# lnkloveating/MediQuery-RAG

Measured on AMD Instinct MI355X. Metric: queries/s (embed+top-k, k=5, b=256) over 1M×768 corpus; p50 single-query ms, higher is better.
Workload: dtype f32 (exact 3-way bf16 split, fp32 accumulate; exact fp32 top-k)

## Files before the change

### include/mq.h

```cpp
#ifndef MQ_H
#define MQ_H

#include <stdint.h>

#ifdef __cplusplus
extern "C" {
#endif

#define MQ_OK 0
#define MQ_EINVAL -1
#define MQ_ENOMEM -2
#define MQ_EHIP -3
#define MQ_EIO -4
#define MQ_ESTATE -5

#define MQ_DTYPE_F32 0
#define MQ_DTYPE_BF16 1
#define MQ_DTYPE_F32X6 2
#define MQ_DTYPE_F32_SCREEN 3

#define MQ_GELU_ERF 0
#define MQ_GELU_TANH 1
#define MQ_POOL_CLS 0
#define MQ_POOL_MEAN 1

#define MQ_MAX_K 64

typedef struct mq_index mq_index;
typedef struct mq_encoder mq_encoder;

const char* mq_last_error(void);
const char* mq_version(void);
const char* mq_build_source_hash(void);
int mq_device_count(void);

int mq_index_create(int device, int dim, int64_t capacity, int dtype, mq_index** out);
int mq_index_destroy(mq_index* ix);
int mq_index_size(const mq_index* ix, int64_t* n_rows);
int mq_index_dim(const mq_index* ix, int* dim);
int mq_index_add(mq_index* ix, const float* rows, int64_t n, int rows_on_device, void* stream);
int mq_index_reset(mq_index* ix);
int mq_index_search(mq_index* ix, const float* queries, int64_t nq, int k,
                    float* out_scores, int64_t* out_ids, int io_on_device, void* stream);
int mq_index_select(mq_index* src, const int64_t* rows, int64_t n, mq_index* dst);
int mq_index_get(mq_index* ix, int64_t row0, int64_t n, float* out, int out_on_device, void* stream);
int mq_index_set_precision(mq_index* ix, int dtype);
int mq_index_set_stream_threshold(mq_index* ix, int max_queries);
int mq_index_set_threshold_scan(mq_index* ix, int enabled);
int mq_index_set_int8_screen(mq_index* ix, int enabled);
int mq_index_set_async_screen(mq_index* ix, int enabled);
int mq_index_rescans(const mq_index* ix, int64_t* rescans, int64_t* remerges);
int mq_index_screen_fallbacks(const mq_index* ix, int64_t* to_direct, int64_t* to_split);
int mq_index_screen_skips(const mq_index* ix, int64_t* bf16_skips, int64_t* int8_skips);
int mq_index_data(mq_index* ix, void** device_rows);
int mq_index_set_timing(mq_index* ix, int enabled);
int mq_index_read_timing(mq_index* ix, float* ms, int n);
#define MQ_MASK_SET 0
#define MQ_MASK_AND 1
#define MQ_MASK_OR 2
#define MQ_MASK_CLEAR 3
int mq_mask_eval(const int32_t* codes, int64_t n, const uint8_t* lut, int n_lut, uint32_t* bits, int mode,
                 void* stream);
int mq_mask_eval_bits(const int32_t* codes, int64_t n, const uint64_t* lut_words, int n_lut, uint32_t* bits,
                      int mode, void* stream);
int mq_mask_combine(uint32_t* dst, const uint32_t* src, int64_t n_words, int mode, void* stream);
int mq_index_search_masked(mq_index* ix, const float* query, int k, const uint32_t* bits, float* out_scores,
                           int64_t* out_ids, int io_on_device, void* stream);
int mq_index_search_masked_batch(mq_index* ix, const float* queries, int64_t nq, int k, const uint32_t* bits,
                                 float* out_scores, int64_t* out_ids, int io_on_device, void* stream);
int mq_index_masked_gathers(const mq_index* ix, int64_t* count);
#define MQ_CONTAINS_MAX_BYTES 256
#define MQ_CONTAINS_SPAN_BYTES 16384
int mq_mask_contains(const uint8_t* text, int64_t text_bytes, const int64_t* offsets, int64_t n,
                     const uint8_t* pattern, int pattern_len, int negate, uint32_t* bits, int mode,
                     uint32_t* scratch, void* stream);

#define MQ_MMR_SCORE(fmul, fsub, lambda, s, red) \
  fsub(fmul((lambda), (s)), fmul(fsub(1.0f, (lambda)), (red)))
int mq_index_mmr_select(mq_index* ix, const float* cand_scores, const int64_t* cand_ids, int64_t nq,
                        int fetch_k, int k, float lambda, float* out_scores, int64_t* out_ids,
                        int io_on_device, void* stream);
int mq_index_search_mmr(mq_index* ix, const float* queries, int64_t nq, int k, int fetch_k,
                        float lambda, const uint32_t* bits, float* out_scores, int64_t* out_ids,
                        int io_on_device, void* stream);

int mq_index_save(mq_index* ix, const char* path);
int mq_index_load(mq_index* ix, const char* path);
int mq_index_save_rows(mq_index* ix, const char* path, int64_t row0, int64_t n);
int mq_index_load_append(mq_index* ix, const char* path);

int mq_topk_merge_host(const float* scores, const int64_t* ids, int n_lists, int64_t nq,
                       int k_in, int k_out, float* out_scores, int64_t* out_ids);
int mq_topk_merge_device(const float* scores, const int64_t* ids, int n_lists, int64_t nq,
                         int k_in, int k_out, float* out_scores, int64_t* out_ids, void* stream);

typedef struct mq_bert_config {
  int vocab_size;
  int hidden;
  int layers;
  int heads;
  int ffn;
  int max_positions;
  int type_vocab;
  float ln_eps;
  int gelu;
  int pooling;
} mq_bert_config;

int mq_encoder_create(int device, const mq_bert_config* cfg, mq_encoder** out);
int mq_encoder_destroy(mq_encoder* enc);
int64_t mq_encoder_weight_count(const mq_bert_config* cfg);
int mq_encoder_load_weights(mq_encoder* enc, const float* blob, int64_t n_floats);
int mq_encoder_set_precision(mq_encoder* enc, int dtype);
#define MQ_ENC_STAGES 8
int mq_encoder_set_graphs(mq_encoder* enc, int enabled);
#define MQ_ENC_OPT_ROWS_MAX 0
#define MQ_ENC_OPT_ROWS_SPLITS 1
#define MQ_ENC_OPT_SPLITK_MAX 2
#define MQ_ENC_OPT_LN_ROWS_PER_WAVE 3
#define MQ_ENC_OPT_FUSE_ATTN_OPROJ 4
#define MQ_ENC_OPT_FUSED_LN 5
#define MQ_ENC_OPT_SPLITK_TILES 6
#define MQ_ENC_OPT_LN_ON_LOAD 7
#define MQ_ENC_OPT_RESIDENT_LAYERS 8
#define MQ_ENC_OPT_X6_PRESPLIT 9
#define MQ_ENC_OPT_ROWS_PLANES 10
#define MQ_ENC_OPT_LN_FOLD 11
int mq_encoder_set_option(mq_encoder* enc, int option, int value);
int mq_encoder_get_option(const mq_encoder* enc, int option, int* value);
int mq_encoder_set_timing(mq_encoder* enc, int enabled);
int mq_encoder_read_timing(mq_encoder* enc, float* ms, int n);
int mq_encoder_embed(mq_encoder* enc, const int32_t* ids, const int32_t* mask, int B, int L,
                     float* out, int io_on_device, void* stream);

typedef struct mq_tokenizer mq_tokenizer;
int mq_tokenizer_create_wordpiece(const char* vocab_path, int lower_case, int max_length,
                                  mq_tokenizer** out);
int mq_tokenizer_create_wordpiece_tokens(const char* const* tokens, int n_tokens, int lower_case,
                                         int max_length, mq_tokenizer** out);
int mq_tokenizer_create_char(int vocab_size, int max_length, mq_tokenizer** out);
int mq_tokenizer_destroy(mq_tokenizer* tok);
int mq_tokenizer_encode_batch(mq_tokenizer* tok, const char* const* texts, int n, int pad_to,
                              int32_t* ids, int32_t* mask, int* out_len);

int mq_debug_gemm_f32(const float* A, const float* W, const float* bias, const float* resid,
                      float* out, int M, int N, int K, int epi, int tile, void* stream);
int64_t mq_debug_w3_bytes(int N, int K);
int mq_debug_split_w3(const float* W, int N, int K, void* w3, void* stream);
int mq_debug_gemm_x6p(const float* A, const void* W3, const float* bias, const float* resid,
                      float* out, int M, int N, int K, int epi, int tile, void* stream);
int mq_debug_gemm_x6p_ln(const float* A, const void* W3, const float* bias, const float* resid,
                         float* out, int M, int N, int K, int epi, int tile, const float* stats_in,
                         float* stats_out, const float* g, const float* b, const float* s_fold,
                         float eps, void* stream);
int mq_debug_ln_fold_weight(const float* W, const float* bias, const float* g, const float* b, int N,
                            int K, float* Wg, float* s_out, float* c_out, void* stream);
int mq_debug_attention(const float* qkv, const int* mask, int B, int L, int H, int heads, float scale,
                       int variant, float* ctx, void* stream);
int mq_debug_attn_oproj(const float* qkv, const int* mask, int B, int L, int H, int heads, float scale,
                        const float* Wo, const float* bo, const float* resid, int cls_only, int hg, int qf,
                        int acc, float* out, void* stream);

int mq_debug_int8_screen(mq_index* ix, const float* query, int kc, float* out_scores, int64_t* out_ids,
                         float* stats);

#ifdef __cplusplus
}
#endif
#endif
```

### mediquery-rag_amd/csrc/encoder.hip

```cpp
#include <algorithm>
#include <cmath>
#include <cstdlib>
#include <cstring>
#include <memory>
#include <vector>

#include "common.hpp"
#include "gemm_epi.hpp"
#include "gemm_f32.hpp"
#include "gemm_x6p.hpp"

namespace mq {


struct LnArgs {
  float* stats_out;
  const float* stats_in;
  const float* g;
  const float* b;
  float* xout;
  int ldx;
  int nt;
  float eps;
};

__device__ __forceinline__ float wave_sum(float v) {
#pragma unroll
  for (int off = 32; off > 0; off >>= 1) v += __shfl_xor(v, off);
  return v;
}

#ifndef MQ_LN_DIAG
#define MQ_LN_DIAG 0
#endif
#if MQ_LN_DIAG != 0 && !defined(MQ_MEASUREMENT_BUILD)
#error "MQ_LN_DIAG computes wrong results: only a measurement build (-DMQ_MEASUREMENT_BUILD) may set it"
#endif

template <class T, class Coords>
struct LnInHooks {
  static constexpr int A_LOADS = T::BM * T::F4_PER_ROW / T::THREADS;
  static_assert(T::A_SLOTS && T::THREADS % T::F4_PER_ROW == 0, "A slots: fixed row chunk per thread");
  const LnArgs& ln;
  Coords& coords;
  float2* st;
  int M, nk, S;
  float inv_k;
  FastDiv nkd;
  float2 part[kLnMaxParts];
  floatx4 gg[T::PF], bb[T::PF];
  float2 mr[A_LOADS];
  template <class DC>
  __device__ __forceinline__ void issue(int s, DC) {
    if constexpr (MQ_LN_DIAG == 1) return;
    constexpr int d = DC::value;
    const int sc = s < S ? s : S - 1;
    const int i = nkd.div(sc), kt = sc - i * nk;
    const int k = kt * T::BK + (threadIdx.x % T::F4_PER_ROW) * 4;
    gg[d] = *reinterpret_cast<const floatx4*>(ln.g + k);
    bb[d] = *reinterpret_cast<const floatx4*>(ln.b + k);
    int m0;
    int64_t n0;
    coords(i, m0, n0);
    const float2* src = reinterpret_cast<const float2*>(ln.stats_in) +
                        (int64_t)min(m0 + (int)threadIdx.x % T::BM, M - 1) * kLnMaxParts;
#pragma unroll
    for (int t = 0; t < kLnMaxParts; ++t) part[t] = src[t];
  }
  __device__ __forceinline__ void prepare(int s) {
    if constexpr (MQ_LN_DIAG == 1) return;
    if (s >= S || nkd.mod(s) != 0) return;
#pragma unroll
    for (int t = 0; t < kLnMaxParts; ++t) asm volatile("" : "+v"(part[t].x), "+v"(part[t].y));
    float mean = 0.f;
#pragma unroll
    for (int t = 0; t < kLnMaxParts; ++t) mean += part[t].x;
    mean *= 1.0f / (float)kLnMaxParts;
    float m2 = 0.f;
#pragma unroll
    for (int t = 0; t < kLnMaxParts; ++t) {
      const float dm = part[t].x - mean;
      m2 += part[t].y + (float)kLnPartW * dm * dm;
    }
    const float rstd = 1.0f / sqrtf(m2 * inv_k + ln.eps);
    if (threadIdx.x < T::BM) st[(nkd.div(s) & 1) * T::BM + threadIdx.x] = make_float2(mean, rstd);
  }
  __device__ __forceinline__ void stage_in(int s) {
    if constexpr (MQ_LN_DIAG == 1) return;
    const float2* ms = st + (nkd.div(s < S ? s : S - 1) & 1) * T::BM;
#pragma unroll
    for (int a = 0; a < A_LOADS; ++a) mr[a] = ms[((int)threadIdx.x + a * T::THREADS) / T::F4_PER_ROW];
  }
  template <class DC>
  __device__ __forceinline__ void xform(Stager<T>& sg, int s, DC) {
    if constexpr (MQ_LN_DIAG != 0) return;
    constexpr int d = DC::value;
#pragma unroll
    for (int a = 0; a < A_LOADS; ++a) sg.r[a] = (sg.r[a] - mr[a].x) * mr[a].y * gg[d] + bb[d];
    const int sc = s < S ? s : S - 1;
    const int i = nkd.div(sc), kt = sc - i * nk;
    int m0;
    int64_t n0;
    coords(i, m0, n0);
    if (n0 == 0 && s < S) {
      const int ch = threadIdx.x % T::F4_PER_ROW;
#pragma unroll
      for (int a = 0; a < A_LOADS; ++a) {
        const int r = min(m0 + ((int)threadIdx.x + a * T::THREADS) / T::F4_PER_ROW, M - 1);
        *reinterpret_cast<floatx4*>(ln.xout + (int64_t)r * ln.ldx + kt * T::BK + ch * 4) = sg.r[a];
      }
    }
  }
};

template <class T, int EPI, bool LN_IN = false>
__global__ __launch_bounds__(T::THREADS, T::WG_PER_CU) void gemm_nt_kernel(const float* __restrict__ A, int lda,
                                                         const float* __restrict__ W,
                                                         const float* __restrict__ bias,
                                                         const float* __restrict__ resid, int ldr,
                                                         float* __restrict__ out, int ldo, int M,
                                                         int N, int K, LnArgs ln, int rx, LnFold lf) {
  __shared__ __attribute__((aligned(16))) float lds[2 * T::STAGE_FLOATS];
  __shared__ float2 ln_st[LN_IN ? 2 * T::BM : 1];
  const int lane = threadIdx.x & 63, wave = __builtin_amdgcn_readfirstlane(threadIdx.x >> 6);
  const int wm = wave / T::WAVES_N, wn = wave % T::WAVES_N;
  const int tiles_n = (N + T::BN - 1) / T::BN, tiles_m = (M + T::BM - 1) / T::BM;
  const int G = gridDim.x, per_xcd = G >> 3;
  const int xslot = (blockIdx.x & 7) * per_xcd + (blockIdx.x >> 3);
  Region rg{0, tiles_m, 0, tiles_n};
  int loc = xslot, wstep = G;
  if (rx > 0) {
    rg = region_of(rx, blockIdx.x & 7, tiles_m, tiles_n);
    loc = blockIdx.x >> 3;
    wstep = per_xcd;
  }
  const int rtiles = rg.rm * rg.rn;
  const int n_tiles = loc < rtiles ? (rtiles - loc + wstep - 1) / wstep : 0;
  const FastDiv tnd(rg.rn);
  auto coords = [&](int i, int& m0, int64_t& n0) {
    const int t = i * wstep + loc;
    const int tr = tnd.div(t);
    m0 = (rg.m_lo + tr) * T::BM;
    n0 = (int64_t)(rg.n_lo + t - tr * rg.rn) * T::BN;
  };
  auto epi = [&](int i, floatx16(&acc)[T::TM][T::TN], float*) {
    int m0;
    int64_t n0l;
    coords(i, m0, n0l);
    const int n0 = (int)n0l;
    if constexpr (T::M16) {
      static_assert(EPI != EPI_RESID_STATS, "no LayerNorm partials on the 16x16x32 tiles");
      floatx4 a4[2 * T::TM][2 * T::TN];
#pragma unroll
      for (int m = 0; m < 2 * T::TM; ++m)
#pragma unroll
        for (int n = 0; n < 2 * T::TN; ++n)
#pragma unroll
          for (int e = 0; e < 4; ++e) a4[m][n][e] = acc[m >> 1][n >> 1][4 * (2 * (m & 1) + (n & 1)) + e];
      store_wave_tile16<EPI, 2 * T::TM, 2 * T::TN>(a4, m0 + wm * T::WM, n0 + wn * T::WN, M, N, bias, resid, ldr, out,
                                                   ldo, lane, lf);
      return;
    }
    static_assert(T::M16 || EPI < EPI_RESID_LN_STATS, "the LayerNorm-fold epilogues are on the 16x16 store");
    if constexpr (EPI == EPI_RESID_STATS) {
      static_assert(T::WN == kLnPartW, "stats partials are per kLnPartW-column wave tile");
      const int wr0 = m0 + wm * T::WM, wc0 = n0 + wn * T::WN;
      const int part = wc0 / T::WN;
      float bv[T::TN];
#pragma unroll
      for (int tn = 0; tn < T::TN; ++tn) bv[tn] = bias[wc0 + tn * 32 + (lane & 31)];
      float rv[T::TM][T::TN][16];
      const bool full = m0 + T::BM <= M;
      const __amdgpu_buffer_rsrc_t ro = __builtin_amdgcn_make_buffer_rsrc(
          (void*)(out + (int64_t)wr0 * ldo + wc0), (short)0, 0x7fffffff, 0x00020000);
      const int ol = (4 * (lane >> 5) * ldo + (lane & 31)) * 4;
      if (full) {
        const __amdgpu_buffer_rsrc_t rr = __builtin_amdgcn_make_buffer_rsrc(
            (void*)(resid + (int64_t)wr0 * ldr + wc0), (short)0, 0x7fffffff, 0x00020000);
        const int rl = (4 * (lane >> 5) * ldr + (lane & 31)) * 4;
#pragma unroll
        for (int tm = 0; tm < T::TM; ++tm)
#pragma unroll
          for (int tn = 0; tn < T::TN; ++tn)
#pragma unroll
            for (int e = 0; e < 16; ++e)
              rv[tm][tn][e] = __uint_as_float(__builtin_amdgcn_raw_buffer_load_b32(
                  rr, rl, (acc_row(tm, e, 0) * ldr + tn * 32) * 4, 0));
      } else {
#pragma unroll
        for (int tm = 0; tm < T::TM; ++tm)
#pragma unroll
          for (int tn = 0; tn < T::TN; ++tn)
#pragma unroll
            for (int e = 0; e < 16; ++e) {
              const int row = min(wr0 + acc_row(tm, e, lane), M - 1);
              rv[tm][tn][e] = resid[(int64_t)row * ldr + wc0 + tn * 32 + (lane & 31)];
            }
      }
#pragma unroll
      for (int tm = 0; tm < T::TM; ++tm)
#pragma unroll
        for (int e = 0; e < 16; ++e) {
          const int row = wr0 + acc_row(tm, e, lane);
          float v[T::TN], sum = 0.f;
#pragma unroll
          for (int tn = 0; tn < T::TN; ++tn) {
            v[tn] = acc[tm][tn][e] + bv[tn] + rv[tm][tn][e];
            sum += v[tn];
          }
          if (full) {
#pragma unroll
            for (int tn = 0; tn < T::TN; ++tn)
              __builtin_amdgcn_raw_buffer_store_b32(__float_as_uint(v[tn]), ro, ol, (acc_row(tm, e, 0) * ldo + tn * 32) * 4, 0);
          } else if (row < M) {
#pragma unroll
            for (int tn = 0; tn < T::TN; ++tn) out[(int64_t)row * ldo + wc0 + tn * 32 + (lane & 31)] = v[tn];
          }
#pragma unroll
          for (int off = 16; off > 0; off >>= 1) sum += __shfl_xor(sum, off);
          const float mean = sum * (1.0f / T::WN);
          float m2 = 0.f;
#pragma unroll
          for (int tn = 0; tn < T::TN; ++tn) m2 += (v[tn] - mean) * (v[tn] - mean);
#pragma unroll
          for (int off = 16; off > 0; off >>= 1) m2 += __shfl_xor(m2, off);
          if ((lane & 31) == 0 && row < M)
            reinterpret_cast<float2*>(ln.stats_out)[(int64_t)row * ln.nt + part] = make_float2(mean, m2);
        }
      return;
    }
    if (m0 + T::BM <= M && n0 + T::BN <= N) {
      const int wr0 = m0 + wm * T::WM, wc0 = n0 + wn * T::WN;
      float bv[T::TN];
#pragma unroll
      for (int tn = 0; tn < T::TN; ++tn) bv[tn] = bias[wc0 + tn * 32 + (lane & 31)];
      float rv[T::TM][T::TN][16];
      if constexpr (EPI == EPI_RESID) {
        const __amdgpu_buffer_rsrc_t rr = __builtin_amdgcn_make_buffer_rsrc(
            (void*)(resid + (int64_t)wr0 * ldr + wc0), (short)0, 0x7fffffff, 0x00020000);
        const int rl = (4 * (lane >> 5) * ldr + (lane & 31)) * 4;
#pragma unroll
        for (int tm = 0; tm < T::TM; ++tm)
#pragma unroll
          for (int tn = 0; tn < T::TN; ++tn)
#pragma unroll
            for (int e = 0; e < 16; ++e)
              rv[tm][tn][e] = __uint_as_float(__builtin_amdgcn_raw_buffer_load_b32(
                  rr, rl, (acc_row(tm, e, 0) * ldr + tn * 32) * 4, 0));
      }
      const __amdgpu_buffer_rsrc_t ro = __builtin_amdgcn_make_buffer_rsrc(
          (void*)(out + (int64_t)wr0 * ldo + wc0), (short)0, 0x7fffffff, 0x00020000);
      const int ol = (4 * (lane >> 5) * ldo + (lane & 31)) * 4;
#pragma unroll
      for (int tm = 0; tm < T::TM; ++tm)
#pragma unroll
        for (int tn = 0; tn < T::TN; ++tn)
#pragma unroll
          for (int e = 0; e < 16; ++e) {
            float v = acc[tm][tn][e] + bv[tn];
            if (EPI == EPI_GELU_ERF) v = gelu_erf(v);
            if (EPI == EPI_GELU_TANH) v = gelu_tanh(v);
            if (EPI == EPI_RESID) v += rv[tm][tn][e];
            __builtin_amdgcn_raw_buffer_store_b32(__float_as_uint(v), ro, ol, (acc_row(tm, e, 0) * ldo + tn * 32) * 4, 0);
          }
      return;
    }
#pragma unroll
    for (int tn = 0; tn < T::TN; ++tn) {
      const int col = n0 + wn * T::WN + tn * 32 + (lane & 31);
      if (col >= N) continue;
      const float b = bias[col];
#pragma unroll
      for (int tm = 0; tm < T::TM; ++tm)
#pragma unroll
        for (int e = 0; e < 16; ++e) {
          const int row = m0 + wm * T::WM + acc_row(tm, e, lane);
          if (row >= M) continue;
          float v = acc[tm][tn][e] + b;
          if (EPI == EPI_GELU_ERF) v = gelu_erf(v);
          if (EPI == EPI_GELU_TANH) v = gelu_tanh(v);
          if (EPI == EPI_RESID) v += resid[(int64_t)row * ldr + col];
          out[(int64_t)row * ldo + col] = v;
        }
    }
  };
  if constexpr (LN_IN) {
    LnInHooks<T, decltype(coords)> hk{ln, coords, ln_st, M, K / T::BK, n_tiles * (K / T::BK), 1.0f / (float)K,
                                      FastDiv(K / T::BK)};
    walk_tiles_hooked<T>(lds, n_tiles, TileOperands{A, lda, M, W, K, N, K}, coords, epi, hk);
  } else {
    walk_tiles<T>(lds, n_tiles, TileOperands{A, lda, M, W, K, N, K}, coords, epi);
  }
}

template <class T>
__global__ __launch_bounds__(T::THREADS, 1) void gemm_resid_ln_kernel(
    const float* __restrict__ A, int lda, const float* __restrict__ W, const float* __restrict__ bias,
    const float* resid, const float* __restrict__ lng, const float* __restrict__ lnb, float eps, float* out,
    int M, int K) {
  constexpr int H = T::BN;
  static_assert(T::WAVES_M == 1 && T::TM == 1 && T::BM == 32, "32-row full-width tiles");
  __shared__ __attribute__((aligned(16))) float lds[2 * T::STAGE_FLOATS];
  __shared__ float red[2][T::WAVES_N][32];
  const int lane = threadIdx.x & 63, wave = threadIdx.x >> 6;
  const int total = (M + 31) / 32;
  const int n_tiles = blockIdx.x < total ? (total - blockIdx.x + gridDim.x - 1) / gridDim.x : 0;
  auto coords = [&](int i, int& m0, int64_t& n0) {
    m0 = (blockIdx.x + i * gridDim.x) * 32;
    n0 = 0;
  };
  float bv[T::TN], gv[T::TN], ev[T::TN];
#pragma unroll
  for (int tn = 0; tn < T::TN; ++tn) {
    const int col = wave * T::WN + tn * 32 + (lane & 31);
    bv[tn] = bias[col];
    gv[tn] = lng[col];
    ev[tn] = lnb[col];
  }
  auto epi = [&](int i, floatx16(&acc)[T::TM][T::TN], float*) {
    const int m0 = (blockIdx.x + i * gridDim.x) * 32;
#pragma unroll
    for (int tn = 0; tn < T::TN; ++tn) {
      const int col = wave * T::WN + tn * 32 + (lane & 31);
#pragma unroll
      for (int e = 0; e < 16; ++e) {
        const int row = min(m0 + acc_row(0, e, lane), M - 1);
        acc[0][tn][e] = acc[0][tn][e] + bv[tn] + resid[(int64_t)row * H + col];
      }
    }
    auto row_reduce = [&](int pass, auto&& val) {
      float p[16];
#pragma unroll
      for (int e = 0; e < 16; ++e) {
        float t = 0.f;
#pragma unroll
        for (int tn = 0; tn < T::TN; ++tn) t += val(tn, e);
        p[e] = t;
      }
#pragma unroll
      for (int off = 1; off < 32; off <<= 1)
#pragma unroll
        for (int e = 0; e < 16; ++e) p[e] += __shfl_xor(p[e], off);
      if ((lane & 31) == 0)
#pragma unroll
        for (int e = 0; e < 16; ++e) red[pass][wave][acc_row(0, e, lane)] = p[e];
    };
    row_reduce(0, [&](int tn, int e) { return acc[0][tn][e]; });
    __syncthreads();
    float mean[16];
#pragma unroll
    for (int e = 0; e < 16; ++e) {
      const int rr = acc_row(0, e, lane);
      float t = 0.f;
#pragma unroll
      for (int w = 0; w < T::WAVES_N; ++w) t += red[0][w][rr];
      mean[e] = t * (1.0f / H);
    }
    row_reduce(1, [&](int tn, int e) {
      const float d = acc[0][tn][e] - mean[e];
      return d * d;
    });
    __syncthreads();
#pragma unroll
    for (int e = 0; e < 16; ++e) {
      const int rr = acc_row(0, e, lane);
      float t = 0.f;
#pragma unroll
      for (int w = 0; w < T::WAVES_N; ++w) t += red[1][w][rr];
      const float rstd = 1.0f / sqrtf(t * (1.0f / H) + eps);
      const int row = m0 + rr;
      if (row < M) {
#pragma unroll
        for (int tn = 0; tn < T::TN; ++tn) {
          const int col = wave * T::WN + tn * 32 + (lane & 31);
          out[(int64_t)row * H + col] = (acc[0][tn][e] - mean[e]) * rstd * gv[tn] + ev[tn];
        }
      }
    }
  };
  walk_tiles<T>(lds, n_tiles, TileOperands{A, lda, M, W, K, H, K}, coords, epi);
}

template <class T>
__global__ __launch_bounds__(256, 2) void gemm_splitk_kernel(const float* __restrict__ A, int lda,
                                                             const float* __restrict__ W, int M,
                                                             int N, int K, int S,
                                                             float* __restrict__ slab) {
  __shared__ __attribute__((aligned(16))) float lds[2 * T::STAGE_FLOATS];
  const int lane = threadIdx.x & 63, wave = threadIdx.x >> 6;
  const int wm = wave / T::WAVES_N, wn = wave % T::WAVES_N;
  const int tiles_n = (N + T::BN - 1) / T::BN;
  const int tile = blockIdx.x / S, sidx = blockIdx.x % S;
  const int Kc = K / S;
  const int m0 = (tile / tiles_n) * T::BM;
  const int n0 = (tile % tiles_n) * T::BN;
  auto coords = [&](int, int& mm0, int64_t& nn0) {
    mm0 = m0;
    nn0 = n0;
  };
  float* dst = slab + (int64_t)sidx * M * N;
  auto epi = [&](int, floatx16(&acc)[T::TM][T::TN], float*) {
#pragma unroll
    for (int tn = 0; tn < T::TN; ++tn) {
      const int col = n0 + wn * T::WN + tn * 32 + (lane & 31);
      if (col >= N) continue;
#pragma unroll
      for (int tm = 0; tm < T::TM; ++tm)
#pragma unroll
        for (int e = 0; e < 16; ++e) {
          const int row = m0 + wm * T::WM + acc_row(tm, e, lane);
          if (row < M) dst[(int64_t)row * N + col] = acc[tm][tn][e];
        }
    }
  };
  walk_tiles<T>(lds, 1, TileOperands{A + (int64_t)sidx * Kc, lda, M, W + (int64_t)sidx * Kc, K, N, Kc},
                coords, epi);
}

__device__ __forceinline__ floatx4 sum_slabs(const float* __restrict__ p, int64_t plane, int S) {
  floatx4 v = {-0.f, -0.f, -0.f, -0.f};
  int s = 0;
  for (; s + 8 <= S; s += 8) {
    floatx4 t[8];
#pragma unroll
    for (int u = 0; u < 8; ++u) t[u] = *reinterpret_cast<const floatx4*>(p + (s + u) * plane);
#pragma unroll
    for (int u = 0; u < 8; ++u) v += t[u];
  }
  if (s + 4 <= S) {
    floatx4 t[4];
#pragma unroll
    for (int u = 0; u < 4; ++u) t[u] = *reinterpret_cast<const floatx4*>(p + (s + u) * plane);
#pragma unroll
    for (int u = 0; u < 4; ++u) v += t[u];
    s += 4;
  }
  for (; s < S; ++s) v += *reinterpret_cast<const floatx4*>(p + s * plane);
  return v;
}

template <int EPI>
__global__ __launch_bounds__(256) void splitk_reduce_kernel(const float* __restrict__ slab, int S,
                                                            int M, int N,
                                                            const float* __restrict__ bias,
                                                            const float* __restrict__ resid, int ldr,
                                                            float* __restrict__ out, int ldo) {
  const int64_t i4 = (int64_t)blockIdx.x * 256 + threadIdx.x;
  const int64_t n4 = N / 4;
  if (i4 >= (int64_t)M * n4) return;
  const int row = (int)(i4 / n4), c = (int)(i4 % n4) * 4;
  const int64_t plane = (int64_t)M * N;
  floatx4 v = sum_slabs(slab + (int64_t)row * N + c, plane, S);
  v += *reinterpret_cast<const floatx4*>(bias + c);
#pragma unroll
  for (int j = 0; j < 4; ++j) {
    if (EPI == EPI_GELU_ERF) v[j] = gelu_erf(v[j]);
    if (EPI == EPI_GELU_TANH) v[j] = gelu_tanh(v[j]);
  }
  if (EPI == EPI_RESID) v += *reinterpret_cast<const floatx4*>(resid + (int64_t)row * ldr + c);
  *reinterpret_cast<floatx4*>(out + (int64_t)row * ldo + c) = v;
}

template <int VPL>
__device__ __forceinline__ void ln_row_store(floatx4 (&x)[VPL], const float* __restrict__ g,
                                             const float* __restrict__ b, float eps,
                                             float* __restrict__ dst, int lane) {
  constexpr int H = VPL * 256;
  float s = 0.f;
#pragma unroll
  for (int i = 0; i < VPL; ++i) s += x[i].x + x[i].y + x[i].z + x[i].w;
  const float mean = wave_sum(s) * (1.0f / H);
  float v = 0.f;
#pragma unroll
  for (int i = 0; i < VPL; ++i) {
    x[i] -= mean;
    v += x[i].x * x[i].x + x[i].y * x[i].y + x[i].z * x[i].z + x[i].w * x[i].w;
  }
  const float rstd = 1.0f / sqrtf(wave_sum(v) * (1.0f / H) + eps);
#pragma unroll
  for (int i = 0; i < VPL; ++i) {
    const int c = (i * 64 + lane) * 4;
    const floatx4 gg = *reinterpret_cast<const floatx4*>(g + c);
    const floatx4 bb = *reinterpret_cast<const floatx4*>(b + c);
    *reinterpret_cast<floatx4*>(dst + c) = x[i] * rstd * gg + bb;
  }
}

template <int VPL>
__global__ __launch_bounds__(256) void splitk_reduce_ln_kernel(
    const float* __restrict__ slab, int S, int M, const float* __restrict__ bias,
    const float* resid, int ldr, const float* __restrict__ g, const float* __restrict__ b,
    float eps, float* dst) {
  constexpr int H = VPL * 256;
  __shared__ float part[4];
  const int t = threadIdx.x, lane = t & 63, wave = t >> 6;
  const int row = blockIdx.x;
  const int64_t plane = (int64_t)M * H;
  float x[VPL];
#pragma unroll
  for (int i = 0; i < VPL; ++i) {
    const int c = t + 256 * i;
    const float* p = slab + (int64_t)row * H + c;
    float v = -0.f;
    int sl = 0;
    for (; sl + 8 <= S; sl += 8) {
      float u[8];
#pragma unroll
      for (int j = 0; j < 8; ++j) u[j] = p[(sl + j) * plane];
#pragma unroll
      for (int j = 0; j < 8; ++j) v += u[j];
    }
    if (sl + 4 <= S) {
      float u[4];
#pragma unroll
      for (int j = 0; j < 4; ++j) u[j] = p[(sl + j) * plane];
#pragma unroll
      for (int j = 0; j < 4; ++j) v += u[j];
      sl += 4;
    }
    for (; sl < S; ++sl) v += p[sl * plane];
    x[i] = v + bias[c] + resid[(int64_t)row * ldr + c];
  }
  auto block_sum = [&](float v) {
    v = wave_sum(v);
    if (lane == 0) part[wave] = v;
    __syncthreads();
    const float r = part[0] + part[1] + part[2] + part[3];
    __syncthreads();
    return r;
  };
  float sum = 0.f;
#pragma unroll
  for (int i = 0; i < VPL; ++i) sum += x[i];
  const float mean = block_sum(sum) * (1.0f / H);
  float var = 0.f;
#pragma unroll
  for (int i = 0; i < VPL; ++i) {
    x[i] -= mean;
    var += x[i] * x[i];
  }
  const float rstd = 1.0f / sqrtf(block_sum(var) * (1.0f / H) + eps);
#pragma unroll
  for (int i = 0; i < VPL; ++i) {
    const int c = t + 256 * i;
    dst[(int64_t)row * H + c] = x[i] * rstd * g[c] + b[c];
  }
}

template <int VPL>
__device__ __forceinline__ void ln_row_stats(const floatx4 (&x)[VPL], float eps, float& mean,
                                             float& rstd) {
  constexpr int H = VPL * 256;
  float s = 0.f;
#pragma unroll
  for (int i = 0; i < VPL; ++i) s += x[i].x + x[i].y + x[i].z + x[i].w;
  mean = wave_sum(s) * (1.0f / H);
  float v = 0.f;
#pragma unroll
  for (int i = 0; i < VPL; ++i) {
    const floatx4 d = x[i] - mean;
    v += d.x * d.x + d.y * d.y + d.z * d.z + d.w * d.w;
  }
  rstd = 1.0f / sqrtf(wave_sum(v) * (1.0f / H) + eps);
}

__device__ __forceinline__ float dpp_add(float v, int ctrl_id) {
  int t;
  switch (ctrl_id) {
    case 0: t = __builtin_amdgcn_update_dpp(0, __float_as_int(v), 0xB1, 0xF, 0xF, false); break;
    case 1: t = __builtin_amdgcn_update_dpp(0, __float_as_int(v), 0x4E, 0xF, 0xF, false); break;
    case 2: t = __builtin_amdgcn_update_dpp(0, __float_as_int(v), 0x141, 0xF, 0xF, false); break;
    default: t = __builtin_amdgcn_update_dpp(0, __float_as_int(v), 0x140, 0xF, 0xF, false); break;
  }
  return v + __int_as_float(t);
}
__device__ __forceinline__ float wave_sum_fast(float v) {
  v = dpp_add(v, 0);
  v = dpp_add(v, 1);
  v = dpp_add(v, 2);
  v = dpp_add(v, 3);
  v += __shfl_xor(v, 16);
  v += __shfl_xor(v, 32);
  return v;
}

template <int VPL>
__device__ __forceinline__ void ln_row_stats_fast(const floatx4 (&x)[VPL], float eps, float& mean,
                                                  float& rstd) {
  constexpr int H = VPL * 256;
  float s = 0.f;
#pragma unroll
  for (int i = 0; i < VPL; ++i) s += x[i].x + x[i].y + x[i].z + x[i].w;
  mean = wave_sum_fast(s) * (1.0f / H);
  float v = 0.f;
#pragma unroll
  for (int i = 0; i < VPL; ++i) {
    const floatx4 d = x[i] - mean;
    v += d.x * d.x + d.y * d.y + d.z * d.z + d.w * d.w;
  }
  rstd = 1.0f / sqrtf(wave_sum_fast(v) * (1.0f / H) + eps);
}

#ifndef MQ_ROWS_DBG
#define MQ_ROWS_DBG 0
#endif
#if MQ_ROWS_DBG != 0 && !defined(MQ_MEASUREMENT_BUILD)
#error "MQ_ROWS_DBG computes wrong results: only a measurement build (-DMQ_MEASUREMENT_BUILD) may set it"
#endif
#if defined(MQ_KTRACE) && !defined(MQ_MEASUREMENT_BUILD)
#error "MQ_KTRACE is a measurement build option (-DMQ_MEASUREMENT_BUILD)"
#endif
#ifdef MQ_KTRACE
constexpr int kTraceSlots = 8, kTraceWgs = 1024, kTraceRegions = 4;
__device__ long long mq_ktrace[kTraceRegions * kTraceWgs * kTraceSlots];
#define KTRACE_R(region, slot)                                                                 \
  do {                                                                                        \
    if (threadIdx.x == 0) {                                                                   \
      const int wg_ = blockIdx.x + gridDim.x * (blockIdx.y + gridDim.y * blockIdx.z);           \
      if (wg_ < kTraceWgs) mq_ktrace[((region) * kTraceWgs + wg_) * kTraceSlots + (slot)] = wall_clock64(); \
    }                                                                                         \
  } while (0)
#else
#define KTRACE_R(region, slot) \
  do {                         \
  } while (0)
#endif
#if defined(MQ_ROWS_REPEAT) && !defined(MQ_MEASUREMENT_BUILD)
#error "MQ_ROWS_REPEAT is a measurement build option (-DMQ_MEASUREMENT_BUILD)"
#endif
#ifdef MQ_ROWS_REPEAT
#define ROWS_REP for (int rep_ = 0; rep_ < 2; ++rep_)
#else
#define ROWS_REP
#endif
__device__ __forceinline__ floatx4 load_w(__amdgpu_buffer_rsrc_t w, int byte_off, int nt) {
  return __builtin_bit_cast(floatx4, nt ? __builtin_amdgcn_raw_buffer_load_b128(w, byte_off, 0, 2)
                                        : __builtin_amdgcn_raw_buffer_load_b128(w, byte_off, 0, 0));
}
__device__ __forceinline__ __amdgpu_buffer_rsrc_t w_rsrc(const float* W) {
  return __builtin_amdgcn_make_buffer_rsrc((void*)W, (short)0, 0x7fffffff, 0x00020000);
}
enum RowsFlags { FL_A = 1, FL_O = 2, FL_OT = 4, FL_ACC = 8 };
__device__ __forceinline__ int64_t frag16_offset(int64_t row, int col, int cols) {
  return ((row >> 4) * (cols >> 4) + (col >> 4)) * 256 + ((row & 15) + 16 * ((col & 15) >> 2)) * 4 + (col & 3);
}
__global__ __launch_bounds__(256) void frag16_image_kernel(const float* __restrict__ W, int R, int C,
                                                           floatx4* __restrict__ img) {
  const int64_t idx = (int64_t)blockIdx.x * 256 + threadIdx.x;
  if (idx >= (int64_t)R * C / 4) return;
  const int lane = (int)(idx & 63);
  const int64_t blk = idx >> 6;
  const int cbs = C >> 4;
  const int64_t rb = blk / cbs;
  const int cb = (int)(blk - rb * cbs);
  img[idx] = *reinterpret_cast<const floatx4*>(W + (rb * 16 + (lane & 15)) * C + cb * 16 + 4 * (lane >> 4));
}

constexpr int kRT = 16;
constexpr int kRWaves = 16;
constexpr int kRowsMax = 256;
constexpr int kRowsDefault = 64;

template <int EPI, bool LN_IN, int VPL, int NB, int S_IN, int RT, int FL = 0>
__global__ __launch_bounds__(1024) void rows_gemm_kernel(
    const float* __restrict__ A, int lda, int64_t a_plane, int M, const float* __restrict__ lng,
    const float* __restrict__ lnb, float eps, float* __restrict__ ln_out,
    const float* __restrict__ W, int ldw, const float* __restrict__ bias,
    const float* __restrict__ resid, int ldr, float* __restrict__ out, int ldo, int64_t o_plane,
    const int* __restrict__ ids, int L, int vocab, const float* __restrict__ pos,
    const float* __restrict__ typ, int nt_w, float* __restrict__ zbuf, int64_t zn) {
  static_assert(!(LN_IN && (FL & FL_A)), "a LayerNorm input is read row-major");
  static_assert(!((FL & FL_ACC) && (FL & FL_O)), "accumulated output is row-major");
  if (zbuf) {
    const int64_t nwg = (int64_t)gridDim.x * gridDim.y * gridDim.z;
    const int64_t wg = blockIdx.x + (int64_t)gridDim.x * (blockIdx.y + (int64_t)gridDim.y * blockIdx.z);
    for (int64_t i = wg * 1024 + threadIdx.x; i < zn / 4; i += nwg * 1024)
      reinterpret_cast<floatx4*>(zbuf)[i] = floatx4{0.f, 0.f, 0.f, 0.f};
  }
  constexpr int K = NB * 256;
  constexpr int CH = RT == 1 ? (NB <= 12 ? NB : 8) : (NB <= 6 ? NB : 4);
  static_assert(NB % CH == 0, "the load batch must divide NB");
  static_assert(!LN_IN || NB == VPL, "LayerNorm input needs K == H");
  static_assert(RT >= 1 && RT * kRT * kRT <= 1024, "one epilogue thread per output element");
  constexpr int AS = K + 4;
  __shared__ __attribute__((aligned(16))) float arows[LN_IN ? RT * kRT * AS : 4];
  __shared__ float part[kRWaves][RT][kRT * kRT];
  const int lane = threadIdx.x & 63, wave = threadIdx.x >> 6;
  const int c = lane & 15, kq = lane >> 4;
  const int n0 = blockIdx.x * kRT, r0 = blockIdx.y * kRT * RT;
  const int kb0 = wave * (K / kRWaves);
  const int ks = blockIdx.z;
  const __amdgpu_buffer_rsrc_t wr = w_rsrc(W);
  const int kblk0 = (ks * K + kb0) >> 4;
  const int wo4 = (((n0 >> 4) * (ldw >> 4) + kblk0) * 64 + lane) * 16;

  KTRACE_R(EPI == EPI_BIAS ? 0 : EPI == EPI_RESID ? 2 : 1, 0);
  floatx4 wv[CH], av[RT][CH];
#pragma unroll
  for (int j = 0; j < CH; ++j)
    wv[j] = (MQ_ROWS_DBG & 1) ? floatx4{1e-3f, 1e-3f, 1e-3f, 1e-3f} : load_w(wr, wo4 + 1024 * j, nt_w);
  const int et = threadIdx.x, ert = et / (kRT * kRT), ep = et % (kRT * kRT);
  const bool vt = (FL & FL_OT) && n0 >= 2 * (ldo / 3);
  const int ee = !(FL & FL_O) ? ep
                 : vt ? ((4 * (ep >> 6) + (ep & 3)) * kRT + ((ep >> 2) & 15))
                      : (((ep >> 2) & 15) * kRT + 4 * (ep >> 6) + (ep & 3));
  const int erow = r0 + ert * kRT + ee / kRT, ecol = n0 + ee % kRT;
  float ebias = 0.f, eres = 0.f;
  if (ert < RT && ks == 0 && erow < M) {
    ebias = bias[ecol];
    if (EPI == EPI_RESID) eres = resid[(int64_t)erow * ldr + ecol];
  }
  floatx4 lgv[LN_IN ? VPL : 1], lbv[LN_IN ? VPL : 1];
  if (LN_IN) {
#pragma unroll
    for (int i = 0; i < VPL; ++i) {
      lgv[i] = *reinterpret_cast<const floatx4*>(lng + (i * 64 + lane) * 4);
      lbv[i] = *reinterpret_cast<const floatx4*>(lnb + (i * 64 + lane) * 4);
    }
  }
  if (LN_IN) {
    floatx4 x[RT][VPL];
#pragma unroll
    for (int rt = 0; rt < RT; ++rt) {
      const int rr = min(r0 + rt * kRT + wave, M - 1);
      const float* src = A + (int64_t)rr * lda;
      if constexpr (MQ_ROWS_DBG & 2) {
#pragma unroll
        for (int i = 0; i < VPL; ++i) x[rt][i] = floatx4{0.1f * lane, 0.2f, 0.3f, 0.4f * wave};
      } else if constexpr (S_IN == 0) {
        int id = ids[rr];
        id = id < 0 ? 0 : (id >= vocab ? vocab - 1 : id);
#pragma unroll
        for (int i = 0; i < VPL; ++i) {
          const int cc = (i * 64 + lane) * 4;
          x[rt][i] = *reinterpret_cast<const floatx4*>(A + (int64_t)id * K + cc) +
                     *reinterpret_cast<const floatx4*>(pos + (int64_t)(rr % L) * K + cc) +
                     *reinterpret_cast<const floatx4*>(typ + cc);
        }
      } else {
        floatx4 p[S_IN][VPL];
#pragma unroll
        for (int z = 0; z < S_IN; ++z)
#pragma unroll
          for (int i = 0; i < VPL; ++i)
            p[z][i] = *reinterpret_cast<const floatx4*>(src + z * a_plane + (i * 64 + lane) * 4);
#pragma unroll
        for (int i = 0; i < VPL; ++i) {
          x[rt][i] = p[0][i];
#pragma unroll
          for (int z = 1; z < S_IN; ++z) x[rt][i] += p[z][i];
        }
      }
    }
#pragma unroll
    for (int rt = 0; rt < RT; ++rt) {
      float mu, rs;
      ln_row_stats_fast<VPL>(x[rt], eps, mu, rs);
#pragma unroll
      for (int i = 0; i < VPL; ++i) {
        const int cc = (i * 64 + lane) * 4;
        x[rt][i] = (x[rt][i] - mu) * rs * lgv[i] + lbv[i];
        *reinterpret_cast<floatx4*>(&arows[(rt * kRT + wave) * AS + cc]) = x[rt][i];
      }
    }
    KTRACE_R(EPI == EPI_BIAS ? 0 : EPI == EPI_RESID ? 2 : 1, 1);
    asm volatile("s_waitcnt lgkmcnt(0)" ::: "memory");
    __builtin_amdgcn_s_barrier();
    KTRACE_R(EPI == EPI_BIAS ? 0 : EPI == EPI_RESID ? 2 : 1, 2);
    if (ln_out && ert < RT) {
      const int rr = ert * kRT + ee / kRT, cc = ee % kRT;
      if (r0 + rr < M)
        for (int c0 = blockIdx.x * kRT; c0 < K; c0 += gridDim.x * kRT)
          ln_out[(int64_t)(r0 + rr) * K + c0 + cc] = arows[rr * AS + c0 + cc];
    }
  }

  floatx4 acc[RT];
#pragma unroll
  for (int rt = 0; rt < RT; ++rt) acc[rt] = floatx4{0.f, 0.f, 0.f, 0.f};
#pragma unroll
  for (int b = 0; b < NB; b += CH) {
    if (b > 0) {
#pragma unroll
      for (int j = 0; j < CH; ++j) wv[j] = load_w(wr, wo4 + 1024 * (b + j), nt_w);
    }
#pragma unroll
    for (int rt = 0; rt < RT; ++rt) {
      const float* arow = A + (int64_t)min(r0 + rt * kRT + c, M - 1) * lda + ks * K + kb0 + 4 * kq;
      const floatx4* afr = reinterpret_cast<const floatx4*>(A) +
                           ((int64_t)((r0 >> 4) + rt) * (lda >> 4) + kblk0) * 64 + lane;
#pragma unroll
      for (int j = 0; j < CH; ++j) {
        if (LN_IN)
          av[rt][j] = *reinterpret_cast<const floatx4*>(&arows[(rt * kRT + c) * AS + kb0 + 16 * (b + j) + 4 * kq]);
        else if (MQ_ROWS_DBG & 2)
          av[rt][j] = floatx4{0.1f, 0.2f, 0.3f, 0.4f};
        else if (FL & FL_A)
          av[rt][j] = afr[(b + j) * 64];
        else
          av[rt][j] = *reinterpret_cast<const floatx4*>(arow + 16 * (b + j));
      }
    }
#pragma unroll
    for (int j = 0; j < CH; ++j) {
#pragma unroll
      for (int t = 0; t < 4; ++t) {
#pragma unroll
        for (int rt = 0; rt < RT; ++rt) {
          if (MQ_ROWS_DBG & 4)
            acc[rt][t] += av[rt][j][t] * wv[j][t];
          else
            acc[rt] = __builtin_amdgcn_mfma_f32_16x16x4f32(av[rt][j][t], wv[j][t], acc[rt], 0, 0, 0);
        }
      }
    }
  }
  KTRACE_R(EPI == EPI_BIAS ? 0 : EPI == EPI_RESID ? 2 : 1, 3);
#pragma unroll
  for (int rt = 0; rt < RT; ++rt)
#pragma unroll
    for (int j = 0; j < 4; ++j) part[wave][rt][(4 * kq + j) * kRT + c] = acc[rt][j];
  __syncthreads();
  KTRACE_R(EPI == EPI_BIAS ? 0 : EPI == EPI_RESID ? 2 : 1, 4);
  if (ert >= RT) return;
  float v = part[0][ert][ee];
#pragma unroll
  for (int w = 1; w < kRWaves; ++w) v += part[w][ert][ee];
  if (erow >= M) return;
  if (ks == 0) {
    v += ebias;
    if (EPI == EPI_GELU_ERF) v = gelu_erf(v);
    if (EPI == EPI_GELU_TANH) v = gelu_tanh(v);
    if (EPI == EPI_RESID) v += eres;
  }
  if (FL & FL_O)
    out[ks * o_plane + (((int64_t)((r0 >> 4) + ert) * (ldo >> 4) + blockIdx.x) << 8) + ep] = v;
  else if (FL & FL_ACC)
    (void)atomicAdd(out + (int64_t)erow * ldo + ecol, v);
  else
    out[ks * o_plane + (int64_t)erow * ldo + ecol] = v;
  KTRACE_R(EPI == EPI_BIAS ? 0 : EPI == EPI_RESID ? 2 : 1, 5);
}

template <int VPL>
__global__ __launch_bounds__(256) void embed_ln_kernel(
    const int* __restrict__ ids, int M, int L, int vocab, const float* __restrict__ word,
    const float* __restrict__ pos, const float* __restrict__ typ, const float* __restrict__ g,
    const float* __restrict__ b, float eps, float* __restrict__ out) {
  constexpr int H = VPL * 256;
  const int lane = threadIdx.x & 63;
  const int row = blockIdx.x * 4 + (threadIdx.x >> 6);
  if (row >= M) return;
  int id = ids[row];
  id = id < 0 ? 0 : (id >= vocab ? vocab - 1 : id);
  const int p = row % L;
  floatx4 x[VPL];
#pragma unroll
  for (int i = 0; i < VPL; ++i) {
    const int c = (i * 64 + lane) * 4;
    x[i] = *reinterpret_cast<const floatx4*>(word + (int64_t)id * H + c) +
           *reinterpret_cast<const floatx4*>(pos + (int64_t)p * H + c) +
           *reinterpret_cast<const floatx4*>(typ + c);
  }
  ln_row_store<VPL>(x, g, b, eps, out + (int64_t)row * H, lane);
}

template <int VPL, int RPW>
__global__ __launch_bounds__(256) void ln_kernel(const float* __restrict__ src, int M,
                                                 const float* __restrict__ g,
                                                 const float* __restrict__ b, float eps,
                                                 float* __restrict__ dst) {
  constexpr int H = VPL * 256;
  const int lane = threadIdx.x & 63;
  const int row0 = (blockIdx.x * 4 + (threadIdx.x >> 6)) * RPW;
  if (row0 >= M) return;
  floatx4 x[RPW][VPL];
#pragma unroll
  for (int r = 0; r < RPW; ++r)
#pragma unroll
    for (int i = 0; i < VPL; ++i)
      x[r][i] = *reinterpret_cast<const floatx4*>(src + (int64_t)min(row0 + r, M - 1) * H + (i * 64 + lane) * 4);
  float s[RPW], v[RPW];
#pragma unroll
  for (int r = 0; r < RPW; ++r) {
    s[r] = 0.f;
#pragma unroll
    for (int i = 0; i < VPL; ++i) s[r] += x[r][i].x + x[r][i].y + x[r][i].z + x[r][i].w;
  }
#pragma unroll
  for (int off = 32; off > 0; off >>= 1)
#pragma unroll
    for (int r = 0; r < RPW; ++r) s[r] += __shfl_xor(s[r], off);
#pragma unroll
  for (int r = 0; r < RPW; ++r) {
    const float mean = s[r] * (1.0f / H);
    v[r] = 0.f;
#pragma unroll
    for (int i = 0; i < VPL; ++i) {
      x[r][i] -= mean;
      v[r] += x[r][i].x * x[r][i].x + x[r][i].y * x[r][i].y + x[r][i].z * x[r][i].z + x[r][i].w * x[r][i].w;
    }
  }
#pragma unroll
  for (int off = 32; off > 0; off >>= 1)
#pragma unroll
    for (int r = 0; r < RPW; ++r) v[r] += __shfl_xor(v[r], off);
#pragma unroll
  for (int r = 0; r < RPW; ++r) {
    if (row0 + r >= M) break;
    const float rstd = 1.0f / sqrtf(v[r] * (1.0f / H) + eps);
#pragma unroll
    for (int i = 0; i < VPL; ++i) {
      const int c = (i * 64 + lane) * 4;
      const floatx4 gg = *reinterpret_cast<const floatx4*>(g + c);
      const floatx4 bb = *reinterpret_cast<const floatx4*>(b + c);
      *reinterpret_cast<floatx4*>(dst + (int64_t)(row0 + r) * H + c) = x[r][i] * rstd * gg + bb;
    }
  }
}

template <int VPL>
__global__ __launch_bounds__(256) void ln_rows_inplace_kernel(float* x, int rows, int64_t stride,
                                                              const float* __restrict__ g,
                                                              const float* __restrict__ b, float eps) {
  const int lane = threadIdx.x & 63;
  const int row = blockIdx.x * 4 + (threadIdx.x >> 6);
  if (row >= rows) return;
  float* xr = x + (int64_t)row * stride;
  floatx4 v[VPL];
#pragma unroll
  for (int i = 0; i < VPL; ++i) v[i] = *reinterpret_cast<const floatx4*>(xr + (i * 64 + lane) * 4);
  ln_row_store<VPL>(v, g, b, eps, xr, lane);
}

constexpr int kDh = 64;

template <int NS, int HB = 1>
__global__ __launch_bounds__(64 * NS * HB, NS == 1 && HB == 1 ? 3 : 1) void attention_kernel(const float* __restrict__ qkv,
                                                            const int* __restrict__ mask, int L,
                                                            int H, int heads, int q_tiles,
                                                            float scale, float* __restrict__ ctx) {
  constexpr int kSt = kDh + 4;
  static_assert(HB == 1 || NS == 1, "heads per block or key splits");
  __shared__ __attribute__((aligned(16))) float tiles[NS * HB][32 * kSt];
  __shared__ float wmax[NS > 1 ? NS : 1][32], wsum[NS > 1 ? NS : 1][32];
  const int wv = NS > 1 ? __builtin_amdgcn_readfirstlane(threadIdx.x >> 6) : 0;
  const int hw = HB > 1 ? __builtin_amdgcn_readfirstlane(threadIdx.x >> 6) : 0;
  float* tile = tiles[NS > 1 ? wv : hw];
  float(*obuf)[kDh + 1] = reinterpret_cast<float(*)[kDh + 1]>(tile);
  const int lane = threadIdx.x & 63, r = lane & 31, hh = lane >> 5;
  const int hgroups = heads / HB;
  const int qt = blockIdx.x % q_tiles, h = ((blockIdx.x / q_tiles) % hgroups) * HB + hw;
  const int bseq = blockIdx.x / (q_tiles * hgroups);
  const int q0 = qt * 32;
  const int64_t row0 = (int64_t)bseq * L;
  const int ld = 3 * H;
  auto stage = [&](int row_base, int col) {
#pragma unroll
    for (int i = 0; i < 8; ++i) {
      const int rr = 4 * i + (lane >> 4);
      const float* src = qkv + (row0 + min(row_base + rr, L - 1)) * ld + col + (lane & 15) * 4;
      *reinterpret_cast<floatx4*>(&tile[rr * kSt + (lane & 15) * 4]) = *reinterpret_cast<const floatx4*>(src);
    }
  };

  float qf[32];
  stage(q0, h * kDh);
#pragma unroll
  for (int i = 0; i < 8; ++i) {
    const floatx4 v = *reinterpret_cast<const floatx4*>(&tile[r * kSt + hh * 32 + 4 * i]) * scale;
    qf[4 * i] = v.x;
    qf[4 * i + 1] = v.y;
    qf[4 * i + 2] = v.z;
    qf[4 * i + 3] = v.w;
  }
  float m_run = -INFINITY, l_run = 0.f;
  floatx16 o0, o1;
#pragma unroll
  for (int e = 0; e < 16; ++e) o0[e] = o1[e] = 0.f;

  for (int k0 = wv * 32; k0 < L; k0 += 32 * NS) {
    const int kr = min(k0 + r, L - 1);
    const bool kvalid = (k0 + r < L) && mask[row0 + kr] != 0;
    const unsigned long long kbits = __ballot(kvalid);
    float kf[32];
    stage(k0, H + h * kDh);
#pragma unroll
    for (int i = 0; i < 8; ++i) {
      const floatx4 v = *reinterpret_cast<const floatx4*>(&tile[r * kSt + hh * 32 + 4 * i]);
      kf[4 * i] = v.x;
      kf[4 * i + 1] = v.y;
      kf[4 * i + 2] = v.z;
      kf[4 * i + 3] = v.w;
    }
    floatx16 st;
#pragma unroll
    for (int e = 0; e < 16; ++e) st[e] = 0.f;
#pragma unroll
    for (int sidx = 0; sidx < 32; ++sidx) st = __builtin_amdgcn_mfma_f32_32x32x2f32(kf[sidx], qf[sidx], st, 0, 0, 0);

    float tmax = -INFINITY;
#pragma unroll
    for (int e = 0; e < 16; ++e) {
      const int key = (e & 3) + 8 * (e >> 2) + 4 * hh;
      st[e] = ((kbits >> key) & 1ull) ? st[e] : -INFINITY;
      tmax = fmaxf(tmax, st[e]);
    }
    tmax = fmaxf(tmax, __shfl_xor(tmax, 32));
    const float m_new = fmaxf(m_run, tmax);
    const float alpha = (m_new == -INFINITY) ? 1.f : expf(m_run - m_new);
    float psum = 0.f;
#pragma unroll
    for (int e = 0; e < 16; ++e) {
      st[e] = (st[e] == -INFINITY) ? 0.f : expf(st[e] - m_new);
      psum += st[e];
    }
    psum += __shfl_xor(psum, 32);
    l_run = l_run * alpha + psum;
    m_run = m_new;
    o0 *= alpha;
    o1 *= alpha;
    const float* vbase = qkv + row0 * ld + 2 * H + h * kDh + r;
#pragma unroll
    for (int sidx = 0; sidx < 16; ++sidx) {
      const int key = min(k0 + (sidx & 3) + 8 * (sidx >> 2) + 4 * hh, L - 1);
      const float v0 = vbase[(int64_t)key * ld];
      const float v1 = vbase[(int64_t)key * ld + 32];
      o0 = __builtin_amdgcn_mfma_f32_32x32x2f32(v0, st[sidx], o0, 0, 0, 0);
      o1 = __builtin_amdgcn_mfma_f32_32x32x2f32(v1, st[sidx], o1, 0, 0, 0);
    }
  }
  const int nrows = min(32, L - q0);
  if constexpr (NS == 1) {
    const float inv = l_run > 0.f ? 1.0f / l_run : 0.f;
#pragma unroll
    for (int e = 0; e < 16; ++e) {
      const int d = (e & 3) + 8 * (e >> 2) + 4 * hh;
      obuf[r][d] = o0[e] * inv;
      obuf[r][d + 32] = o1[e] * inv;
    }
    __syncthreads();
    for (int q = 0; q < nrows; ++q) ctx[(row0 + q0 + q) * H + h * kDh + lane] = obuf[q][lane];
  } else {
    if (hh == 0) wmax[wv][r] = m_run;
    __syncthreads();
    float m = -INFINITY;
#pragma unroll
    for (int w = 0; w < NS; ++w) m = fmaxf(m, wmax[w][r]);
    const float sc = m_run == -INFINITY ? 0.f : expf(m_run - m);
    if (hh == 0) wsum[wv][r] = l_run * sc;
#pragma unroll
    for (int e = 0; e < 16; ++e) {
      const int d = (e & 3) + 8 * (e >> 2) + 4 * hh;
      obuf[r][d] = o0[e] * sc;
      obuf[r][d + 32] = o1[e] * sc;
    }
    __syncthreads();
    for (int i = threadIdx.x; i < 32 * kDh; i += 64 * NS) {
      const int q = i / kDh, d = i % kDh;
      if (q >= nrows) break;
      float o = 0.f, l = 0.f;
#pragma unroll
      for (int w = 0; w < NS; ++w) {
        o += reinterpret_cast<const float(*)[kDh + 1]>(tiles[w])[q][d];
        l += wsum[w][q];
      }
      ctx[(row0 + q0 + q) * H + h * kDh + d] = l > 0.f ? o * (1.0f / l) : 0.f;
    }
  }
}

void launch_attention(int B, int L, int heads, int qt, int H, float scale, const float* qkv,
                      const int* mask, float* ctx, hipStream_t s) {
  const int triples = B * heads * qt, key_tiles = (L + 31) / 32;
  const dim3 grid(triples);
  if (key_tiles == 1 && heads == 12 && triples >= 12 * 256)
    hipLaunchKernelGGL((attention_kernel<1, 12>), dim3(B * qt), dim3(768), 0, s, qkv, mask, L, H, heads, qt, scale,
                       ctx);
  else if (key_tiles >= 8 && triples <= 256)
    hipLaunchKernelGGL(attention_kernel<8>, grid, dim3(512), 0, s, qkv, mask, L, H, heads, qt, scale, ctx);
  else if (key_tiles >= 4 && triples <= 512)
    hipLaunchKernelGGL(attention_kernel<4>, grid, dim3(256), 0, s, qkv, mask, L, H, heads, qt, scale, ctx);
  else if (key_tiles >= 2 && triples <= 1024)
    hipLaunchKernelGGL(attention_kernel<2>, grid, dim3(128), 0, s, qkv, mask, L, H, heads, qt, scale, ctx);
  else
    hipLaunchKernelGGL(attention_kernel<1>, grid, dim3(64), 0, s, qkv, mask, L, H, heads, qt, scale, ctx);
}

__global__ __launch_bounds__(512) void attention_rows_kernel(const float* __restrict__ qkv,
                                                             const int* __restrict__ mask, int L,
                                                             int H, int heads, int q_tiles,
                                                             float scale, float* __restrict__ ctx) {
  __shared__ float smax[2][4][16], ssum[2][4][16];
  __shared__ float opart[2][4][16][kDh + 1];
  const int lane = threadIdx.x & 63, w = threadIdx.x >> 6;
  const int kw = w >> 1, qh = w & 1;
  const int c = lane & 15, g = lane >> 4;
  const int qt = blockIdx.x % q_tiles, h = (blockIdx.x / q_tiles) % heads;
  const int bseq = blockIdx.x / (q_tiles * heads);
  const int64_t row0 = (int64_t)bseq * L;
  const int ld = 3 * H;
  const int q = qt * 32 + qh * 16 + c;
  const int key = kw * 16 + c;

  floatx4 qf[4], kf[4];
  {
    const float* qs = qkv + (row0 + min(q, L - 1)) * ld + h * kDh + 4 * g;
    const float* ks = qkv + (row0 + min(key, L - 1)) * ld + H + h * kDh + 4 * g;
#pragma unroll
    for (int s = 0; s < 4; ++s) {
      qf[s] = *reinterpret_cast<const floatx4*>(qs + 16 * s) * scale;
      kf[s] = *reinterpret_cast<const floatx4*>(ks + 16 * s);
    }
  }
  float vf[4][4];
  {
    const float* vs = qkv + row0 * ld + 2 * H + h * kDh + c;
#pragma unroll
    for (int t = 0; t < 4; ++t) {
      const int kk = min(kw * 16 + 4 * g + t, L - 1);
#pragma unroll
      for (int db = 0; db < 4; ++db) vf[db][t] = vs[(int64_t)kk * ld + 16 * db];
    }
  }
  const bool kvalid = key < L && mask[row0 + min(key, L - 1)] != 0;
  const unsigned kbits = (unsigned)(__ballot(kvalid) & 0xFFFFull);

  floatx4 s0 = {0.f, 0.f, 0.f, 0.f}, s1 = {0.f, 0.f, 0.f, 0.f};
#pragma unroll
  for (int s = 0; s < 2; ++s)
#pragma unroll
    for (int t = 0; t < 4; ++t) {
      s0 = __builtin_amdgcn_mfma_f32_16x16x4f32(kf[s][t], qf[s][t], s0, 0, 0, 0);
      s1 = __builtin_amdgcn_mfma_f32_16x16x4f32(kf[s + 2][t], qf[s + 2][t], s1, 0, 0, 0);
    }
  floatx4 st = s0 + s1;
  float mx = -INFINITY;
#pragma unroll
  for (int j = 0; j < 4; ++j) {
    st[j] = ((kbits >> (4 * g + j)) & 1u) ? st[j] : -INFINITY;
    mx = fmaxf(mx, st[j]);
  }
  mx = fmaxf(mx, __shfl_xor(mx, 16));
  mx = fmaxf(mx, __shfl_xor(mx, 32));
  if (g == 0) smax[qh][kw][c] = mx;
  __syncthreads();
  const float m = fmaxf(fmaxf(smax[qh][0][c], smax[qh][1][c]), fmaxf(smax[qh][2][c], smax[qh][3][c]));
  float ls = 0.f;
#pragma unroll
  for (int j = 0; j < 4; ++j) {
    st[j] = (st[j] == -INFINITY) ? 0.f : expf(st[j] - m);
    ls += st[j];
  }
  ls += __shfl_xor(ls, 16);
  ls += __shfl_xor(ls, 32);
  if (g == 0) ssum[qh][kw][c] = ls;
  floatx4 o[4];
#pragma unroll
  for (int db = 0; db < 4; ++db) {
    o[db] = floatx4{0.f, 0.f, 0.f, 0.f};
#pragma unroll
    for (int t = 0; t < 4; ++t) o[db] = __builtin_amdgcn_mfma_f32_16x16x4f32(vf[db][t], st[t], o[db], 0, 0, 0);
  }
#pragma unroll
  for (int db = 0; db < 4; ++db)
#pragma unroll
    for (int j = 0; j < 4; ++j) opart[qh][kw][c][16 * db + 4 * g + j] = o[db][j];
  __syncthreads();
#pragma unroll
  for (int e = 0; e < 4; ++e) {
    const int idx = e * 512 + (int)threadIdx.x;
    const int q32 = idx >> 6, d = idx & 63;
    const int qq = q32 >> 4, qc = q32 & 15;
    const float v = ((opart[qq][0][qc][d] + opart[qq][1][qc][d]) + opart[qq][2][qc][d]) + opart[qq][3][qc][d];
    const float l = ((ssum[qq][0][qc] + ssum[qq][1][qc]) + ssum[qq][2][qc]) + ssum[qq][3][qc];
    const int qrow = qt * 32 + q32;
    if (qrow < L) ctx[(row0 + qrow) * H + h * kDh + d] = v * (l > 0.f ? 1.0f / l : 0.f);
  }
}

constexpr int kOpCols = 32;

template <int HG, int NKB, bool QF = false, bool ACC = false>
__global__ __launch_bounds__(512) void attn_oproj_rows_kernel(
    const float* __restrict__ qkv, const int* __restrict__ mask, int L, int H, int rps, int qtiles,
    float scale, const float* __restrict__ Wo, const float* __restrict__ bo,
    const float* __restrict__ resid, int ldr, float* __restrict__ out, int64_t o_plane, int nt_w) {
  constexpr int KG = HG * kDh;
  constexpr int CS = KG + 4;
  constexpr int KQ = KG / 4;
  constexpr int NJ = KQ / 16;
  __shared__ __attribute__((aligned(16))) float ctx[16 * CS];
  __shared__ float part[8][256];
  const int lane = threadIdx.x & 63, w = threadIdx.x >> 6;
  const int c = lane & 15, g = lane >> 4;
  const int b = blockIdx.y / qtiles, q0 = (blockIdx.y % qtiles) * 16;
  const int grp = blockIdx.z, h0 = grp * HG;
  const int n0 = blockIdx.x * kOpCols;
  const int64_t srow0 = (int64_t)b * L;
  const int ld = 3 * H;

  KTRACE_R(3, 0);
  const int cb = w & 1, kqr = w >> 1;
  floatx4 wv[NJ];
  {
    const __amdgpu_buffer_rsrc_t wr = w_rsrc(Wo);
    const int wo4 = ((((n0 >> 4) + cb) * (H >> 4) + ((h0 * kDh + kqr * KQ) >> 4)) * 64 + lane) * 16;
#pragma unroll
    for (int j = 0; j < NJ; ++j) wv[j] = load_w(wr, wo4 + 1024 * j, nt_w);
  }
  const int et = threadIdx.x, ecb = et >> 8, erow_t = (et & 255) >> 4, ecol = n0 + ecb * 16 + (et & 15);
  const int qrow = q0 + erow_t;
  const int64_t orow = (int64_t)b * rps + qrow;
  float ebias = 0.f, eres = 0.f;
  if (grp == 0 && qrow < rps) {
    ebias = bo[ecol];
    eres = resid[orow * ldr + ecol];
  }

  if (w < HG) {
    const int h = h0 + w;
    const int qpos = rps == 1 ? 0 : min(q0 + c, L - 1);
    floatx4 qf[4], kf[NKB][4];
    float vf[NKB][4][4];
    if constexpr (QF) {
      const floatx4* f4 = reinterpret_cast<const floatx4*>(qkv);
      const int cbs = ld >> 4;
      const int64_t rb0 = srow0 >> 4;
      auto blk = [&](int64_t rb, int cb) { return f4 + (rb * cbs + cb) * 64 + lane; };
#pragma unroll
      for (int sI = 0; sI < 4; ++sI) qf[sI] = *blk(rb0 + (q0 >> 4), ((h * kDh) >> 4) + sI);
#pragma unroll
      for (int kb = 0; kb < NKB; ++kb)
#pragma unroll
        for (int sI = 0; sI < 4; ++sI) kf[kb][sI] = *blk(rb0 + kb, ((H + h * kDh) >> 4) + sI);
#pragma unroll
      for (int kb = 0; kb < NKB; ++kb)
#pragma unroll
        for (int db = 0; db < 4; ++db) {
          const floatx4 v = *blk(rb0 + kb, ((2 * H + h * kDh) >> 4) + db);
#pragma unroll
          for (int t = 0; t < 4; ++t) vf[kb][db][t] = v[t];
        }
    } else {
      const float* qs = qkv + (srow0 + qpos) * ld + h * kDh + 4 * g;
#pragma unroll
      for (int sI = 0; sI < 4; ++sI) qf[sI] = *reinterpret_cast<const floatx4*>(qs + 16 * sI);
#pragma unroll
      for (int kb = 0; kb < NKB; ++kb) {
        const float* ks = qkv + (srow0 + min(kb * 16 + c, L - 1)) * ld + H + h * kDh + 4 * g;
#pragma unroll
        for (int sI = 0; sI < 4; ++sI) kf[kb][sI] = *reinterpret_cast<const floatx4*>(ks + 16 * sI);
      }
      const float* vs = qkv + srow0 * ld + 2 * H + h * kDh + c;
#pragma unroll
      for (int kb = 0; kb < NKB; ++kb)
#pragma unroll
        for (int t = 0; t < 4; ++t) {
          const int64_t kk = min(kb * 16 + 4 * g + t, L - 1);
#pragma unroll
          for (int db = 0; db < 4; ++db) vf[kb][db][t] = vs[kk * ld + 16 * db];
        }
    }
    const bool kval = lane < L && mask[srow0 + min(lane, L - 1)] != 0;
    const unsigned long long kbits = __ballot(kval);
#pragma unroll
    for (int sI = 0; sI < 4; ++sI) qf[sI] *= scale;
    KTRACE_R(3, 1);
    floatx4 st[NKB];
#pragma unroll
    for (int kb = 0; kb < NKB; ++kb) {
      floatx4 a0 = {0.f, 0.f, 0.f, 0.f}, a1 = {0.f, 0.f, 0.f, 0.f};
#pragma unroll
      for (int t = 0; t < 4; ++t) {
        a0 = __builtin_amdgcn_mfma_f32_16x16x4f32(kf[kb][0][t], qf[0][t], a0, 0, 0, 0);
        a1 = __builtin_amdgcn_mfma_f32_16x16x4f32(kf[kb][2][t], qf[2][t], a1, 0, 0, 0);
      }
#pragma unroll
      for (int t = 0; t < 4; ++t) {
        a0 = __builtin_amdgcn_mfma_f32_16x16x4f32(kf[kb][1][t], qf[1][t], a0, 0, 0, 0);
        a1 = __builtin_amdgcn_mfma_f32_16x16x4f32(kf[kb][3][t], qf[3][t], a1, 0, 0, 0);
      }
      st[kb] = a0 + a1;
    }
    float mx = -INFINITY;
#pragma unroll
    for (int kb = 0; kb < NKB; ++kb)
#pragma unroll
      for (int j = 0; j < 4; ++j) {
        const int key = kb * 16 + 4 * g + j;
        st[kb][j] = ((kbits >> key) & 1ull) ? st[kb][j] : -INFINITY;
        mx = fmaxf(mx, st[kb][j]);
      }
    mx = fmaxf(mx, __shfl_xor(mx, 16));
    mx = fmaxf(mx, __shfl_xor(mx, 32));
    float ls = 0.f;
#pragma unroll
    for (int kb = 0; kb < NKB; ++kb)
#pragma unroll
      for (int j = 0; j < 4; ++j) {
        st[kb][j] = (st[kb][j] == -INFINITY) ? 0.f : expf(st[kb][j] - mx);
        ls += st[kb][j];
      }
    ls += __shfl_xor(ls, 16);
    ls += __shfl_xor(ls, 32);
    const float inv = ls > 0.f ? 1.0f / ls : 0.f;
    floatx4 o[4];
#pragma unroll
    for (int db = 0; db < 4; ++db) {
      o[db] = floatx4{0.f, 0.f, 0.f, 0.f};
#pragma unroll
      for (int kb = 0; kb < NKB; ++kb)
#pragma unroll
        for (int t = 0; t < 4; ++t) o[db] = __builtin_amdgcn_mfma_f32_16x16x4f32(vf[kb][db][t], st[kb][t], o[db], 0, 0, 0);
    }
#pragma unroll
    for (int db = 0; db < 4; ++db)
#pragma unroll
      for (int j = 0; j < 4; ++j) ctx[c * CS + w * kDh + 16 * db + 4 * g + j] = o[db][j] * inv;
    KTRACE_R(3, 2);
  }
  __syncthreads();
  KTRACE_R(3, 3);
  floatx4 acc2[2] = {{0.f, 0.f, 0.f, 0.f}, {0.f, 0.f, 0.f, 0.f}};
#pragma unroll
  for (int j = 0; j < NJ; ++j) {
    const floatx4 av = *reinterpret_cast<const floatx4*>(&ctx[c * CS + kqr * KQ + 16 * j + 4 * g]);
#pragma unroll
    for (int t = 0; t < 4; ++t) acc2[j & 1] = __builtin_amdgcn_mfma_f32_16x16x4f32(av[t], wv[j][t], acc2[j & 1], 0, 0, 0);
  }
  const floatx4 acc = acc2[0] + acc2[1];
  KTRACE_R(3, 4);
#pragma unroll
  for (int j = 0; j < 4; ++j) part[w][(4 * g + j) * 16 + c] = acc[j];
  __syncthreads();
  KTRACE_R(3, 5);
  const int e = et & 255;
  float v = part[ecb][e];
#pragma unroll
  for (int q = 1; q < 4; ++q) v += part[ecb + 2 * q][e];
  if (qrow >= rps) return;
  if (grp == 0) v = (v + ebias) + eres;
  if (ACC)
    (void)atomicAdd(out + orow * H + ecol, v);
  else
    out[grp * o_plane + orow * H + ecol] = v;
  KTRACE_R(3, 6);
}

template <int VPL>
__global__ __launch_bounds__(256) void pool_kernel(const float* __restrict__ hs,
                                                   const int* __restrict__ mask, int B, int L,
                                                   int pooling, float* __restrict__ out) {
  constexpr int H = VPL * 256;
  const int lane = threadIdx.x & 63;
  const int b = blockIdx.x * 4 + (threadIdx.x >> 6);
  if (b >= B) return;
  floatx4 x[VPL];
  if (pooling == MQ_POOL_MEAN) {
    float cnt = 0.f;
#pragma unroll
    for (int i = 0; i < VPL; ++i) x[i] = floatx4{0.f, 0.f, 0.f, 0.f};
    for (int r = 0; r < L; ++r) {
      if (!mask[(int64_t)b * L + r]) continue;
      cnt += 1.f;
#pragma unroll
      for (int i = 0; i < VPL; ++i)
        x[i] += *reinterpret_cast<const floatx4*>(hs + ((int64_t)b * L + r) * H + (i * 64 + lane) * 4);
    }
    const float inv = 1.0f / fmaxf(cnt, 1.f);
#pragma unroll
    for (int i = 0; i < VPL; ++i) x[i] *= inv;
  } else {
#pragma unroll
    for (int i = 0; i < VPL; ++i)
      x[i] = *reinterpret_cast<const floatx4*>(hs + (int64_t)b * L * H + (i * 64 + lane) * 4);
  }
  float ss = 0.f;
#pragma unroll
  for (int i = 0; i < VPL; ++i) ss += x[i].x * x[i].x + x[i].y * x[i].y + x[i].z * x[i].z + x[i].w * x[i].w;
  const float inv = 1.0f / fmaxf(sqrtf(wave_sum(ss)), 1e-12f);
#pragma unroll
  for (int i = 0; i < VPL; ++i)
    *reinterpret_cast<floatx4*>(out + (int64_t)b * H + (i * 64 + lane) * 4) = x[i] * inv;
}

template <int VPL>
__global__ __launch_bounds__(256) void ln_pool_kernel(const float* __restrict__ hs, int planes,
                                                      int64_t plane, const int* __restrict__ mask,
                                                      int B, int L, int rows, int pooling,
                                                      const float* __restrict__ g,
                                                      const float* __restrict__ be, float eps,
                                                      float* __restrict__ out) {
  constexpr int H = VPL * 256;
  const int lane = threadIdx.x & 63;
  const int b = blockIdx.x * 4 + (threadIdx.x >> 6);
  if (b >= B) return;
  auto ln_row = [&](const float* src, floatx4 (&x)[VPL]) {
#pragma unroll
    for (int i = 0; i < VPL; ++i) x[i] = *reinterpret_cast<const floatx4*>(src + (i * 64 + lane) * 4);
    for (int z = 1; z < planes; ++z)
#pragma unroll
      for (int i = 0; i < VPL; ++i) x[i] += *reinterpret_cast<const floatx4*>(src + z * plane + (i * 64 + lane) * 4);
    float mu, rs;
    ln_row_stats<VPL>(x, eps, mu, rs);
#pragma unroll
    for (int i = 0; i < VPL; ++i) {
      const int c = (i * 64 + lane) * 4;
      x[i] = (x[i] - mu) * rs * *reinterpret_cast<const floatx4*>(g + c) +
             *reinterpret_cast<const floatx4*>(be + c);
    }
  };
  floatx4 x[VPL];
  if (pooling == MQ_POOL_MEAN) {
    float cnt = 0.f;
#pragma unroll
    for (int i = 0; i < VPL; ++i) x[i] = floatx4{0.f, 0.f, 0.f, 0.f};
    for (int r = 0; r < L; ++r) {
      if (!mask[(int64_t)b * L + r]) continue;
      cnt += 1.f;
      floatx4 y[VPL];
      ln_row(hs + ((int64_t)b * rows + r) * H, y);
#pragma unroll
      for (int i = 0; i < VPL; ++i) x[i] += y[i];
    }
    const float inv = 1.0f / fmaxf(cnt, 1.f);
#pragma unroll
    for (int i = 0; i < VPL; ++i) x[i] *= inv;
  } else {
    ln_row(hs + (int64_t)b * rows * H, x);
  }
  float ss = 0.f;
#pragma unroll
  for (int i = 0; i < VPL; ++i) ss += x[i].x * x[i].x + x[i].y * x[i].y + x[i].z * x[i].z + x[i].w * x[i].w;
  const float inv = 1.0f / fmaxf(sqrtf(wave_sum(ss)), 1e-12f);
#pragma unroll
  for (int i = 0; i < VPL; ++i)
    *reinterpret_cast<floatx4*>(out + (int64_t)b * H + (i * 64 + lane) * 4) = x[i] * inv;
}

}

using namespace mq;

namespace {

struct Buf {
  float* p = nullptr;
  size_t n = 0;
  int ensure(size_t need) {
    if (need <= n) return MQ_OK;
    if (p) (void)hipFree(p);
    p = nullptr;
    n = 0;
    if (hipMalloc((void**)&p, need * sizeof(float)) != hipSuccess)
      MQ_FAIL(MQ_ENOMEM, "hipMalloc(%zu floats) failed", need);
    n = need;
    return MQ_OK;
  }
  void release() {
    if (p) (void)hipFree(p);
    p = nullptr;
    n = 0;
  }
};

struct LayerW {
  const float *wqkv, *bqkv, *wo, *bo, *ln1g, *ln1b, *w1, *b1, *w2, *b2, *ln2g, *ln2b;
  const unsigned char *wqkv3 = nullptr, *wo3 = nullptr, *w13 = nullptr, *w23 = nullptr;
  const float *wqkvf = nullptr, *wof = nullptr, *w1f = nullptr, *w2f = nullptr;
  const unsigned char *w1g3 = nullptr, *wqkvg3 = nullptr;
  const float *w1gf = nullptr, *wqkvgf = nullptr;
  const float *w1s = nullptr, *w1c = nullptr, *wqkvs = nullptr, *wqkvc = nullptr;
};

int64_t weight_count(const mq_bert_config& c) {
  const int64_t H = c.hidden, F = c.ffn;
  const int64_t per_layer = 3 * H * H + 3 * H + H * H + H + 2 * H + F * H + F + H * F + H + 2 * H;
  return ((int64_t)c.vocab_size + c.max_positions + c.type_vocab) * H + 2 * H + c.layers * per_layer;
}

}


namespace {

struct GemmArgs {
  float* slab;
  size_t slab_floats;
  const float* A;
  int lda;
  const float* W;
  const float* bias;
  const float* resid;
  int ldr;
  float* out;
  int ldo;
  int M, N, K;
  int nt = 0;
  const void* W3 = nullptr;
  LnFold lf{};
};

template <class T, int EPI, bool LN_IN = false>
void launch_gemm_t(const GemmArgs& g, int num_cus, hipStream_t s, const LnArgs& ln = LnArgs{}) {
  const int tiles = ((g.M + T::BM - 1) / T::BM) * ((g.N + T::BN - 1) / T::BN);
  const int grid = (std::min(tiles, T::WG_PER_CU * num_cus) + 7) / 8 * 8;
  const int tiles_m = (g.M + T::BM - 1) / T::BM, tiles_n = (g.N + T::BN - 1) / T::BN;
  const int rx = region_pick_rx(tiles_m, tiles_n, (double)T::BM * g.K * 4, (double)T::BN * g.K * 4, grid);
  hipLaunchKernelGGL((gemm_nt_kernel<T, EPI, LN_IN>), dim3(grid), dim3(T::THREADS), 0, s, g.A, g.lda, g.W,
                     g.bias, g.resid, g.ldr, g.out, g.ldo, g.M, g.N, g.K, ln, rx, g.lf);
}

using GemmBig = F32Tile<2, 2, 2, 2>;
using GemmT96 = F32Tile<4, 1, 1, 3>;
using GemmMid = F32Tile<2, 2, 2, 1>;
using GemmSmall = F32Tile<1, 4, 1, 1>;

using X6Big = F32Tile<2, 2, 2, 2, true, 2, false, 0, false, true>;
using X6T96 = F32Tile<4, 1, 1, 3, true, 2, false, 0, false, true>;
using X6Mid = F32Tile<2, 2, 2, 1, true, 2, false, 0, false, true>;
using X6W192 = F32Tile<4, 2, 1, 3, true, 2, false, 0, false, true>;

template <int EPI>
void launch_gemm_tile(const GemmArgs& g, int tile, int num_cus, hipStream_t s) {
  switch (tile) {
    case 0: launch_gemm_t<GemmBig, EPI>(g, num_cus, s); return;
    case 1: launch_gemm_t<GemmT96, EPI>(g, num_cus, s); return;
    case 2: launch_gemm_t<GemmMid, EPI>(g, num_cus, s); return;
    case 5: launch_gemm_t<X6Big, EPI>(g, num_cus, s); return;
    case 6: launch_gemm_t<X6T96, EPI>(g, num_cus, s); return;
    case 7: launch_gemm_t<X6Mid, EPI>(g, num_cus, s); return;
    case 8: launch_gemm_t<F32Tile<4, 2, 1, 3>, EPI>(g, num_cus, s); return;
    case 9: launch_gemm_t<X6W192, EPI>(g, num_cus, s); return;
    default: launch_gemm_t<GemmSmall, EPI>(g, num_cus, s); return;
  }
}

int splitk_factor(const GemmArgs& g, int num_cus, int cap = 16, int tiles_max = 0) {
  if (!g.slab || g.N % 4 != 0) return 0;
  const int64_t tiles = (int64_t)((g.M + 31) / 32) * ((g.N + 127) / 128);
  const int64_t slots = 2 * (int64_t)num_cus;
  if (tiles > (tiles_max > 0 ? tiles_max : num_cus) || g.M > 256) return 0;
  const int slices = g.K / kBK;
  int best = 1;
  for (int s = 1; s <= slices && s <= cap; ++s)
    if (slices % s == 0 && tiles * s <= slots && (size_t)s * g.M * g.N <= g.slab_floats) best = s;
  return best >= 2 ? best : 0;
}

void launch_splitk_gemm(const GemmArgs& g, int S, hipStream_t s) {
  auto go = [&](auto tile) {
    using T = decltype(tile);
    const int tiles = ((g.M + T::BM - 1) / T::BM) * ((g.N + T::BN - 1) / T::BN);
    hipLaunchKernelGGL((gemm_splitk_kernel<T>), dim3(tiles * S), dim3(256), 0, s, g.A, g.lda, g.W, g.M, g.N, g.K,
                       S, g.slab);
  };
  if (g.nt)
    go(F32Tile<1, 4, 1, 1, false, 2, false, 0, true>{});
  else
    go(F32Tile<1, 4, 1, 1>{});
}

template <int EPI>
void launch_splitk(const GemmArgs& g, int S, hipStream_t s) {
  launch_splitk_gemm(g, S, s);
  const int64_t n4 = (int64_t)g.M * g.N / 4;
  hipLaunchKernelGGL((splitk_reduce_kernel<EPI>), dim3((unsigned)((n4 + 255) / 256)), dim3(256), 0,
                     s, g.slab, S, g.M, g.N, g.bias, g.resid, g.ldr, g.out, g.ldo);
}

int x6_tile_pick(const GemmArgs& g, int num_cus) {
  const int bns[3] = {128, 96, 64};
  const double effs[3] = {1.0, 0.96, 0.9};
  const int64_t slots = 2 * (int64_t)num_cus;
  int best = 0;
  double best_cost = 1e300;
  for (int i = 0; i < 3; ++i) {
    const int64_t tiles = (int64_t)((g.M + 127) / 128) * ((g.N + bns[i] - 1) / bns[i]);
    const double cost = (double)((tiles + slots - 1) / slots) * 128 * bns[i] / effs[i];
    if (cost < best_cost) {
      best_cost = cost;
      best = i;
    }
  }
  return best;
}

template <int EPI>
void launch_gemm_fold(const GemmArgs& g, int num_cus, hipStream_t s) {
  if (g.W3) {
    X6pArgs a{g.A, g.lda, g.W3, g.bias, g.resid, g.ldr, g.out, g.ldo, g.M, g.N, g.K};
    a.lf = g.lf;
    launch_gemm_x6p(a, EPI, -1, num_cus, s);
    return;
  }
  if constexpr (EPI == EPI_RESID_LN_STATS) {
    launch_gemm_t<X6T96, EPI>(g, num_cus, s);
  } else {
    switch (x6_tile_pick(g, num_cus)) {
      case 0: launch_gemm_t<X6Big, EPI>(g, num_cus, s); return;
      case 1: launch_gemm_t<X6T96, EPI>(g, num_cus, s); return;
      default: launch_gemm_t<X6Mid, EPI>(g, num_cus, s); return;
    }
  }
}

template <int EPI>
void launch_gemm(const GemmArgs& g, int num_cus, hipStream_t s, bool x6 = false, int splitk_cap = 16,
                 int splitk_tiles = 0) {
  const int S = splitk_factor(g, num_cus, splitk_cap, splitk_tiles);
  if (S) {
    launch_splitk<EPI>(g, S, s);
    return;
  }
  if (x6 && (int64_t)((g.M + 127) / 128) * ((g.N + 191) / 192) < num_cus) x6 = false;
  if (x6 && g.W3) {
    launch_gemm_x6p(X6pArgs{g.A, g.lda, g.W3, g.bias, g.resid, g.ldr, g.out, g.ldo, g.M, g.N, g.K}, EPI, -1, num_cus,
                    s);
    return;
  }
  if (x6) {
    launch_gemm_tile<EPI>(g, 5 + x6_tile_pick(g, num_cus), num_cus, s);
    return;
  }
  struct Cand {
    int bm, bn;
    double eff;
  };
  const Cand cands[4] = {{128, 128, 1.0}, {128, 96, 0.96}, {128, 64, 0.9}, {32, 128, 0.55}};
  const int64_t slots = 2 * (int64_t)num_cus;
  int best = 0;
  double best_cost = 1e300;
  for (int i = 0; i < 4; ++i) {
    const int64_t tiles = (int64_t)((g.M + cands[i].bm - 1) / cands[i].bm) * ((g.N + cands[i].bn - 1) / cands[i].bn);
    const int64_t rounds = (tiles + slots - 1) / slots;
    const double cost = (double)rounds * cands[i].bm * cands[i].bn / cands[i].eff;
    if (cost < best_cost) {
      best_cost = cost;
      best = i;
    }
  }
  launch_gemm_tile<EPI>(g, best, num_cus, s);
}

void launch_gemm_stats(const GemmArgs& g, const LnArgs& ln, int num_cus, hipStream_t s) {
  launch_gemm_t<GemmT96, EPI_RESID_STATS>(g, num_cus, s, ln);
}

template <int EPI>
void launch_gemm_ln_in(const GemmArgs& g, const LnArgs& ln, int num_cus, hipStream_t s) {
  const int64_t slots = 2 * (int64_t)num_cus;
  auto cost = [&](int bn, double eff) {
    const int64_t tiles = (int64_t)((g.M + 127) / 128) * ((g.N + bn - 1) / bn);
    return (double)((tiles + slots - 1) / slots) * 128 * bn / eff;
  };
  if (cost(128, 1.0) <= cost(96, 0.96))
    launch_gemm_t<GemmBig, EPI, true>(g, num_cus, s, ln);
  else
    launch_gemm_t<GemmT96, EPI, true>(g, num_cus, s, ln);
}

#ifndef MQ_LN_FOLD_DEFAULT
#define MQ_LN_FOLD_DEFAULT 1
#endif
constexpr bool kLnFoldDefault = MQ_LN_FOLD_DEFAULT != 0;

enum Stage { ST_EMBED = 0, ST_QKV, ST_ATTN, ST_OPROJ, ST_LN, ST_FFN_UP, ST_FFN_DOWN, ST_POOL, ST_N };


}

struct mq_encoder {
  int device = 0;
  PinBuf pin;
  mq_bert_config cfg{};
  int precision = MQ_DTYPE_F32;
  bool loaded = false;
  Buf weights;
  const float *word = nullptr, *pos = nullptr, *typ = nullptr, *eg = nullptr, *eb = nullptr;
  std::vector<LayerW> layers;
  Buf x, y, qkv, ctx, ffn, io_out, slab;
  Buf w3;
  Buf wfrag;
  int* io_ids = nullptr;
  int* io_mask = nullptr;
  size_t io_tokens = 0;
  Timeline tl;
  int num_cus = 256;
  struct Graph {
    int B = 0, L = 0, precision = 0;
    std::vector<const void*> bufs;
    hipGraphExec_t exec = nullptr;
    uint64_t last_use = 0;
  };
  std::vector<Graph> graphs;
  bool fuse_attn_oproj = true;
  int rows_max = kRowsDefault;
  int rows_splits = 0;
  int splitk_max = 16;
  int splitk_tiles = 0;
  int ln_rows_per_wave = 4;
  bool fused_ln = false;
  int resident_layers = 8;
  bool ln_on_load = false;
  Buf lnst;
  bool x6_presplit = true;
  bool ln_fold = kLnFoldDefault;
  Buf wfold3, wfoldf, sfold;
  bool rows_planes = false;
  bool use_graphs = false;
  uint64_t graph_clock = 0;
  hipStream_t cap_stream = nullptr;
  std::mutex mu;
};

namespace {

int build_w3(mq_encoder* e) {
  if (e->precision != MQ_DTYPE_F32X6 || !e->loaded || e->layers.empty() || e->layers[0].wqkv3) return MQ_OK;
  const mq_bert_config& c = e->cfg;
  const int H = c.hidden, F = c.ffn;
  const size_t per = w3_bytes(3 * H, H) + w3_bytes(H, H) + w3_bytes(F, H) + w3_bytes(H, F);
  DeviceGuard dg(e->device);
  int rc = e->w3.ensure((per * e->layers.size() + 3) / 4);
  if (rc) return rc;
  unsigned char* p = reinterpret_cast<unsigned char*>(e->w3.p);
  for (LayerW& w : e->layers) {
    auto one = [&](const float* W, int n, int k, const unsigned char*& dst) {
      launch_split_w3(W, n, k, p, nullptr);
      dst = p;
      p += w3_bytes(n, k);
    };
    one(w.wqkv, 3 * H, H, w.wqkv3);
    one(w.wo, H, H, w.wo3);
    one(w.w1, F, H, w.w13);
    one(w.w2, H, F, w.w23);
  }
  MQ_HIP(hipGetLastError());
  MQ_HIP(hipStreamSynchronize(nullptr));
  return MQ_OK;
}

int build_fold(mq_encoder* e) {
  const mq_bert_config& c = e->cfg;
  const int H = c.hidden, F = c.ffn;
  if (!e->ln_fold || e->precision != MQ_DTYPE_F32X6 || !e->loaded || e->layers.empty() ||
      H != kLnPartW * kLnMaxParts || F % 32 != 0)
    return MQ_OK;
  const bool img = e->x6_presplit;
  if (img ? e->layers[0].w1g3 != nullptr : e->layers[0].w1gf != nullptr) return MQ_OK;
  const size_t nl = e->layers.size();
  DeviceGuard dg(e->device);
  int rc = e->sfold.ensure(nl * 2 * ((size_t)F + 3 * H));
  if (rc) return rc;
  Buf tmp;
  if (img) {
    rc = e->wfold3.ensure((nl * w3_bytes(F, H) + (nl - 1) * w3_bytes(3 * H, H) + 3) / 4);
    if (!rc) rc = tmp.ensure((size_t)std::max(F, 3 * H) * H);
  } else {
    rc = e->wfoldf.ensure((nl * (size_t)F + (nl - 1) * (size_t)3 * H) * H);
  }
  if (rc) return rc;
  unsigned char* p3 = reinterpret_cast<unsigned char*>(e->wfold3.p);
  float* pf = e->wfoldf.p;
  float* ps = e->sfold.p;
  const LayerW* prev = nullptr;
  for (LayerW& w : e->layers) {
    auto one = [&](const float* W, const float* bias, const float* g, const float* b, int n, const unsigned char*& d3,
                   const float*& df, const float*& ds, const float*& dc) {
      float* wg = img ? tmp.p : pf;
      launch_ln_fold_weight(W, bias, g, b, n, H, wg, ps, ps + n, nullptr);
      ds = ps;
      dc = ps + n;
      ps += 2 * n;
      if (img) {
        launch_split_w3(wg, n, H, p3, nullptr);
        d3 = p3;
        p3 += w3_bytes(n, H);
      } else {
        df = pf;
        pf += (size_t)n * H;
      }
    };
    one(w.w1, w.b1, w.ln1g, w.ln1b, F, w.w1g3, w.w1gf, w.w1s, w.w1c);
    if (prev) one(w.wqkv, w.bqkv, prev->ln2g, prev->ln2b, 3 * H, w.wqkvg3, w.wqkvgf, w.wqkvs, w.wqkvc);
    prev = &w;
  }
  const hipError_t e1 = hipGetLastError(), e2 = hipStreamSynchronize(nullptr);
  tmp.release();
  MQ_HIP(e1);
  MQ_HIP(e2);
  return MQ_OK;
}

int build_frag16(mq_encoder* e) {
  const mq_bert_config& c = e->cfg;
  const int64_t H = c.hidden, F = c.ffn;
  const int64_t per = 3 * H * H + H * H + F * H + H * F;
  DeviceGuard dg(e->device);
  int rc = e->wfrag.ensure((size_t)(per * (int64_t)e->layers.size()));
  if (rc) return rc;
  float* p = e->wfrag.p;
  for (LayerW& w : e->layers) {
    auto one = [&](const float* W, int64_t r, int64_t k, const float*& dst) {
      const int64_t n4 = r * k / 4;
      hipLaunchKernelGGL(frag16_image_kernel, dim3((unsigned)((n4 + 255) / 256)), dim3(256), 0, nullptr, W, (int)r,
                         (int)k, reinterpret_cast<floatx4*>(p));
      dst = p;
      p += r * k;
    };
    one(w.wqkv, 3 * H, H, w.wqkvf);
    one(w.wo, H, H, w.wof);
    one(w.w1, F, H, w.w1f);
    one(w.w2, H, F, w.w2f);
  }
  MQ_HIP(hipGetLastError());
  MQ_HIP(hipStreamSynchronize(nullptr));
  return MQ_OK;
}

template <int EPI>
void gemm(mq_encoder* e, const GemmArgs& g, int stage, hipStream_t s) {
  e->tl.mark(s, stage);
  GemmArgs a = g;
  if (!e->x6_presplit) a.W3 = nullptr;
  launch_gemm<EPI>(a, e->num_cus, s, e->precision == MQ_DTYPE_F32X6, e->splitk_max, e->splitk_tiles);
}

template <int VPL>
void gemm_resid_ln(mq_encoder* e, const GemmArgs& g, const float* lng, const float* lnb, float* x,
                   int stage, hipStream_t s) {
  const int H = VPL * 256;
  const unsigned rb = (unsigned)((g.M + 3) / 4);
  const int S = splitk_factor(g, e->num_cus, e->splitk_max, e->splitk_tiles);
  if constexpr (VPL <= 3) {
    if (!S && e->fused_ln && e->precision == MQ_DTYPE_F32 && g.ldr == H && g.N == H && g.resid == x) {
      using T = F32Tile<1, 8, 1, VPL, false, 2, false, 16>;
      e->tl.mark(s, stage);
      const int tiles = (g.M + 31) / 32;
      hipLaunchKernelGGL((gemm_resid_ln_kernel<T>), dim3(std::min(tiles, e->num_cus)), dim3(T::THREADS), 0, s,
                         g.A, g.lda, g.W, g.bias, g.resid, lng, lnb, e->cfg.ln_eps, x, g.M, g.K);
      return;
    }
  }
  if (S && g.ldr == H && g.N == H) {
    e->tl.mark(s, stage);
    launch_splitk_gemm(g, S, s);
    e->tl.mark(s, ST_LN);
    hipLaunchKernelGGL((splitk_reduce_ln_kernel<VPL>), dim3((unsigned)g.M), dim3(256), 0, s, g.slab, S,
                       g.M, g.bias, g.resid, g.ldr, lng, lnb, e->cfg.ln_eps, x);
    return;
  }
  gemm<EPI_RESID>(e, g, stage, s);
  e->tl.mark(s, ST_LN);
  const int rpw = e->ln_rows_per_wave;
  if (rpw == 4)
    hipLaunchKernelGGL((ln_kernel<VPL, 4>), dim3((unsigned)((g.M + 15) / 16)), dim3(256), 0, s, g.out, g.M, lng,
                       lnb, e->cfg.ln_eps, x);
  else if (rpw == 1)
    hipLaunchKernelGGL((ln_kernel<VPL, 1>), dim3(rb), dim3(256), 0, s, g.out, g.M, lng, lnb, e->cfg.ln_eps, x);
  else
    hipLaunchKernelGGL((ln_kernel<VPL, 2>), dim3((unsigned)((g.M + 7) / 8)), dim3(256), 0, s, g.out, g.M, lng,
                       lnb, e->cfg.ln_eps, x);
}

template <int VPL>
int forward_vpl(mq_encoder* e, const int* ids, const int* mask, int B, int L, float* out,
                hipStream_t s) {
  const mq_bert_config& c = e->cfg;
  const int M = B * L, H = c.hidden, F = c.ffn;
  const unsigned row_blocks = (unsigned)((M + 3) / 4);
  const float scale = 1.0f / sqrtf((float)(H / c.heads));
  const int q_tiles = (L + 31) / 32;
  e->tl.mark(s, ST_EMBED);
  hipLaunchKernelGGL((embed_ln_kernel<VPL>), dim3(row_blocks), dim3(256), 0, s, ids, M, L,
                     c.vocab_size, e->word, e->pos, e->typ, e->eg, e->eb, c.ln_eps, e->x.p);
  const int nt = H / kLnPartW;
  const bool lnl = e->ln_on_load && !e->fused_ln && e->precision == MQ_DTYPE_F32 && M > 256 &&
                   H == kLnPartW * kLnMaxParts && e->lnst.n >= (size_t)4 * M * nt;
  float* st1 = e->lnst.p;
  float* st2 = lnl ? e->lnst.p + (size_t)2 * M * nt : nullptr;
  bool y_pending = false;
  const LayerW* prev = nullptr;
  const LayerW w0 = e->layers.empty() ? LayerW{} : e->layers[0];
  const bool fold = e->ln_fold && e->precision == MQ_DTYPE_F32X6 && M > 256 && H == kLnPartW * kLnMaxParts &&
                    F % 32 == 0 && (int64_t)((M + 127) / 128) * ((H + 191) / 192) >= e->num_cus &&
                    e->lnst.n >= (size_t)4 * M * nt && (e->x6_presplit ? w0.w1g3 != nullptr : w0.w1gf != nullptr);
  float* fst1 = e->lnst.p;
  float* fst2 = e->lnst.p + (size_t)2 * M * nt;
  bool raw = false;
  auto fold_gemm = [&](auto epi, GemmArgs g, int stage) {
    e->tl.mark(s, stage);
    if (!e->x6_presplit) g.W3 = nullptr;
    g.lf.eps = c.ln_eps;
    launch_gemm_fold<decltype(epi)::value>(g, e->num_cus, s);
  };
  auto ln_args = [&](const float* stats, const float* g, const float* b) {
    LnArgs a{};
    a.stats_in = stats;
    a.g = g;
    a.b = b;
    a.xout = e->x.p;
    a.ldx = H;
    a.nt = nt;
    a.eps = c.ln_eps;
    return a;
  };
  auto stats_out = [&](float* stats) {
    LnArgs a{};
    a.stats_out = stats;
    a.nt = nt;
    return a;
  };
  for (size_t li = 0; li < e->layers.size(); ++li) {
    const LayerW& w = e->layers[li];
    const bool cls_only = c.pooling == MQ_POOL_CLS && li + 1 == e->layers.size();
    const int rows = cls_only ? B : M;
    const int stride = cls_only ? L * H : H;
    const float* qkv_in = y_pending ? e->y.p : e->x.p;
    const int lnt = M <= 256 && (int)li >= e->resident_layers ? 1 : 0;
    const bool fold_layer = fold && !(cls_only && L > 1);
    auto qkv_fold = [&](GemmArgs g, int row0) {
      g.W = w.wqkvgf ? w.wqkvgf + (int64_t)row0 * H : nullptr;
      g.W3 = w.wqkvg3 ? w.wqkvg3 + w3_row_offset(row0, H) : nullptr;
      g.bias = w.wqkvc + row0;
      g.lf.s = w.wqkvs + row0;
      g.lf.stats_in = fst2;
      fold_gemm(IC<EPI_BIAS_LNFOLD>{}, g, ST_QKV);
    };
    auto qkv_gemm = [&](GemmArgs g) {
      g.nt = lnt;
      if (raw) {
        qkv_fold(g, (int)(g.W - w.wqkv) / H);
      } else if (y_pending) {
        e->tl.mark(s, ST_QKV);
        launch_gemm_ln_in<EPI_BIAS>(g, ln_args(st2, prev->ln2g, prev->ln2b), e->num_cus, s);
      } else {
        gemm<EPI_BIAS>(e, g, ST_QKV, s);
      }
    };
    if (cls_only && L > 1) {
      GemmArgs kv{e->slab.p, e->slab.n, qkv_in, H, w.wqkv + (int64_t)H * H, w.bqkv + H, nullptr, 0, e->qkv.p + H,
                  3 * H, M, 2 * H, H};
      if (w.wqkv3) kv.W3 = w.wqkv3 + w3_row_offset(H, H);
      qkv_gemm(kv);
      if (raw) {
        e->tl.mark(s, ST_LN);
        hipLaunchKernelGGL((ln_rows_inplace_kernel<VPL>), dim3((unsigned)((B + 3) / 4)), dim3(256), 0, s, e->x.p, B,
                           (int64_t)L * H, prev->ln2g, prev->ln2b, c.ln_eps);
      }
      GemmArgs q{e->slab.p, e->slab.n, e->x.p, L * H, w.wqkv, w.bqkv, nullptr, 0, e->qkv.p, L * 3 * H, B, H, H, lnt};
      q.W3 = w.wqkv3;
      gemm<EPI_BIAS>(e, q, ST_QKV, s);
    } else {
      GemmArgs qkv{e->slab.p, e->slab.n, qkv_in, H, w.wqkv, w.bqkv, nullptr, 0, e->qkv.p, 3 * H, M, 3 * H, H};
      qkv.W3 = w.wqkv3;
      qkv_gemm(qkv);
    }
    y_pending = false;
    const bool resid_raw = raw && fold_layer;
    raw = false;
    e->tl.mark(s, ST_ATTN);
    const int qt = cls_only ? 1 : q_tiles;
    launch_attention(B, L, c.heads, qt, H, scale, e->qkv.p, mask, e->ctx.p, s);
    const bool lnl_layer = lnl && !cls_only;
    GemmArgs oproj{e->slab.p, e->slab.n, e->ctx.p, stride, w.wo, w.bo, e->x.p, stride, e->y.p, H, rows, H, H, lnt};
    oproj.W3 = w.wo3;
    if (fold_layer) {
      oproj.lf.stats_out = fst1;
      if (resid_raw) {
        oproj.lf.stats_in = fst2;
        oproj.lf.g = prev->ln2g;
        oproj.lf.b = prev->ln2b;
      }
      fold_gemm(IC<EPI_RESID_LN_STATS>{}, oproj, ST_OPROJ);
    } else if (lnl_layer) {
      e->tl.mark(s, ST_OPROJ);
      launch_gemm_stats(oproj, stats_out(st1), e->num_cus, s);
    } else {
      gemm_resid_ln<VPL>(e, oproj, w.ln1g, w.ln1b, e->x.p, ST_OPROJ, s);
    }
    GemmArgs up{e->slab.p, e->slab.n, lnl_layer ? e->y.p : e->x.p, H, w.w1, w.b1, nullptr, 0, e->ffn.p, F,
                rows, F, H, lnt};
    up.W3 = w.w13;
    if (fold_layer) {
      up.A = e->y.p;
      up.W = w.w1gf;
      up.W3 = w.w1g3;
      up.bias = w.w1c;
      up.lf.s = w.w1s;
      up.lf.stats_in = fst1;
      if (c.gelu == MQ_GELU_TANH)
        fold_gemm(IC<EPI_GELU_TANH_LNFOLD>{}, up, ST_FFN_UP);
      else
        fold_gemm(IC<EPI_GELU_ERF_LNFOLD>{}, up, ST_FFN_UP);
    } else if (lnl_layer) {
      e->tl.mark(s, ST_FFN_UP);
      if (c.gelu == MQ_GELU_TANH)
        launch_gemm_ln_in<EPI_GELU_TANH>(up, ln_args(st1, w.ln1g, w.ln1b), e->num_cus, s);
      else
        launch_gemm_ln_in<EPI_GELU_ERF>(up, ln_args(st1, w.ln1g, w.ln1b), e->num_cus, s);
    } else if (c.gelu == MQ_GELU_TANH) {
      gemm<EPI_GELU_TANH>(e, up, ST_FFN_UP, s);
    } else {
      gemm<EPI_GELU_ERF>(e, up, ST_FFN_UP, s);
    }
    GemmArgs down{e->slab.p, e->slab.n, e->ffn.p, F, w.w2, w.b2, e->x.p, H, e->y.p, H, rows, H, F, lnt};
    down.W3 = w.w23;
    if (fold_layer) {
      const bool last = li + 1 == e->layers.size();
      down.resid = e->y.p;
      down.lf.stats_in = fst1;
      down.lf.g = w.ln1g;
      down.lf.b = w.ln1b;
      down.lf.stats_out = fst2;
      down.out = last ? e->ctx.p : e->x.p;
      fold_gemm(IC<EPI_RESID_LN_STATS>{}, down, ST_FFN_DOWN);
      if (last) {
        e->tl.mark(s, ST_LN);
        hipLaunchKernelGGL((ln_kernel<VPL, 4>), dim3((unsigned)((M + 15) / 16)), dim3(256), 0, s, e->ctx.p, M, w.ln2g,
                           w.ln2b, c.ln_eps, e->x.p);
      } else {
        raw = true;
      }
    } else if (lnl_layer && li + 1 < e->layers.size()) {
      e->tl.mark(s, ST_FFN_DOWN);
      launch_gemm_stats(down, stats_out(st2), e->num_cus, s);
      y_pending = true;
    } else {
      gemm_resid_ln<VPL>(e, down, w.ln2g, w.ln2b, e->x.p, ST_FFN_DOWN, s);
    }
    prev = &w;
  }
  e->tl.mark(s, ST_POOL);
  const bool pruned = c.pooling == MQ_POOL_CLS;
  hipLaunchKernelGGL((pool_kernel<VPL>), dim3((B + 3) / 4), dim3(256), 0, s, e->x.p, mask, B,
                     pruned ? 1 : L, c.pooling, out);
  e->tl.close(s);
  MQ_HIP(hipGetLastError());
  return MQ_OK;
}

struct RowsArgs {
  const float* A;
  int lda;
  int64_t a_plane;
  const float* W;
  int ldw;
  const float* bias;
  const float* resid;
  int ldr;
  float* out;
  int ldo;
  int64_t o_plane;
  int M, N, K;
  int splits;
  const int* ids = nullptr;
  int L = 1, vocab = 0;
  const float* pos = nullptr;
  const float* typ = nullptr;
  int nt_w = 0;
  float* zbuf = nullptr;
  int64_t zn = 0;
};

template <int EPI, bool LN_IN, int VPL, int NB, int S_IN, int RT, int FL>
void launch_rows_rt(const RowsArgs& g, const float* lng, const float* lnb, float eps, float* ln_out,
                    hipStream_t s) {
  hipLaunchKernelGGL((rows_gemm_kernel<EPI, LN_IN, VPL, NB, S_IN, RT, FL>),
                     dim3(g.N / kRT, (g.M + kRT * RT - 1) / (kRT * RT), g.splits), dim3(64 * kRWaves), 0, s,
                     g.A, g.lda, g.a_plane, g.M, lng, lnb, eps, ln_out, g.W, g.ldw, g.bias, g.resid, g.ldr,
                     g.out, g.ldo, g.o_plane, g.ids, g.L, g.vocab, g.pos, g.typ, g.nt_w, g.zbuf, g.zn);
}

template <int EPI, bool LN_IN, int VPL, int NB, int S_IN, int FL = 0>
void launch_rows_nb(const RowsArgs& g, const float* lng, const float* lnb, float eps, float* ln_out,
                    hipStream_t s) {
  constexpr bool two_fit = LN_IN && (size_t)(2 * kRT * (NB * 256 + 4) + kRWaves * 2 * kRT * kRT) * 4 <= 160 * 1024;
  if constexpr (two_fit) {
    if (g.M > kRT) {
      launch_rows_rt<EPI, LN_IN, VPL, NB, S_IN, 2, FL>(g, lng, lnb, eps, ln_out, s);
      return;
    }
  }
  launch_rows_rt<EPI, LN_IN, VPL, NB, S_IN, 1, FL>(g, lng, lnb, eps, ln_out, s);
}

bool rows_nb_ok(int nb) { return nb >= 1 && (nb <= 4 || nb == 6 || nb == 8 || nb == 12 || nb == 16); }

int rows_splits(int K, int forced = 0) {
  const int nb = K / 256;
  if (forced >= 1 && forced <= 4 && nb % forced == 0 && rows_nb_ok(nb / forced)) return forced;
  for (int sp = 1; sp <= 4; ++sp)
    if (nb % sp == 0 && nb / sp <= 6 && rows_nb_ok(nb / sp)) return sp;
  return 1;
}

template <int EPI, int NB, int FL>
void launch_rows_plain(const RowsArgs& g, hipStream_t s) {
  launch_rows_nb<EPI, false, 1, NB, 1, FL>(g, nullptr, nullptr, 0.f, nullptr, s);
}

template <int EPI, int FL = 0>
void launch_rows(const RowsArgs& g, hipStream_t s) {
  switch (g.K / g.splits / 256) {
    case 1: launch_rows_plain<EPI, 1, FL>(g, s); return;
    case 2: launch_rows_plain<EPI, 2, FL>(g, s); return;
    case 3: launch_rows_plain<EPI, 3, FL>(g, s); return;
    case 4: launch_rows_plain<EPI, 4, FL>(g, s); return;
    case 6: launch_rows_plain<EPI, 6, FL>(g, s); return;
    case 8: launch_rows_plain<EPI, 8, FL>(g, s); return;
    case 12: launch_rows_plain<EPI, 12, FL>(g, s); return;
    default: launch_rows_plain<EPI, 16, FL>(g, s); return;
  }
}

template <int EPI, int VPL, int FL = 0>
void launch_rows_ln(const RowsArgs& g, int s_in, const float* lng, const float* lnb, float eps,
                    float* ln_out, hipStream_t s) {
  switch (s_in) {
    case 0: launch_rows_nb<EPI, true, VPL, VPL, 0, FL>(g, lng, lnb, eps, ln_out, s); return;
    case 1: launch_rows_nb<EPI, true, VPL, VPL, 1, FL>(g, lng, lnb, eps, ln_out, s); return;
    case 2: launch_rows_nb<EPI, true, VPL, VPL, 2, FL>(g, lng, lnb, eps, ln_out, s); return;
    case 3: launch_rows_nb<EPI, true, VPL, VPL, 3, FL>(g, lng, lnb, eps, ln_out, s); return;
    default: launch_rows_nb<EPI, true, VPL, VPL, 4, FL>(g, lng, lnb, eps, ln_out, s); return;
  }
}

template <int HG, bool QF, bool ACC>
void launch_attn_oproj_hg(int nkb, dim3 grid, hipStream_t s, const float* qkv, const int* mask, int L, int H,
                          int rps, int qtiles, float scale, const float* wo, const float* bo, const float* resid,
                          int ldr, float* out, int64_t o_plane, int nt_w) {
  auto go = [&](auto kern) {
    hipLaunchKernelGGL(kern, grid, dim3(512), 0, s, qkv, mask, L, H, rps, qtiles, scale, wo, bo, resid, ldr, out,
                       o_plane, nt_w);
  };
  switch (nkb) {
    case 1: go(attn_oproj_rows_kernel<HG, 1, QF, ACC>); break;
    case 2: go(attn_oproj_rows_kernel<HG, 2, QF, ACC>); break;
    case 3: go(attn_oproj_rows_kernel<HG, 3, QF, ACC>); break;
    default: go(attn_oproj_rows_kernel<HG, 4, QF, ACC>); break;
  }
}

void launch_attn_oproj(int hg, bool qf, bool acc, int nkb, dim3 grid, hipStream_t s, const float* qkv,
                       const int* mask, int L, int H, int rps, int qtiles, float scale, const float* wo,
                       const float* bo, const float* resid, int ldr, float* out, int64_t o_plane, int nt_w) {
  auto go = [&](auto hgc, auto qfc, auto accc) {
    launch_attn_oproj_hg<decltype(hgc)::value, decltype(qfc)::value, decltype(accc)::value>(
        nkb, grid, s, qkv, mask, L, H, rps, qtiles, scale, wo, bo, resid, ldr, out, o_plane, nt_w);
  };
  if (hg == 6) {
    if (qf && acc) go(IC<6>{}, std::true_type{}, std::true_type{});
    else if (qf) go(IC<6>{}, std::true_type{}, std::false_type{});
    else if (acc) go(IC<6>{}, std::false_type{}, std::true_type{});
    else go(IC<6>{}, std::false_type{}, std::false_type{});
  } else {
    if (qf && acc) go(IC<4>{}, std::true_type{}, std::true_type{});
    else if (qf) go(IC<4>{}, std::true_type{}, std::false_type{});
    else if (acc) go(IC<4>{}, std::false_type{}, std::true_type{});
    else go(IC<4>{}, std::false_type{}, std::false_type{});
  }
}

int oproj_heads_per_plane(const mq_encoder* e, int L) {
  const mq_bert_config& c = e->cfg;
  if (!e->fuse_attn_oproj || L > 64 || c.hidden != c.heads * kDh || c.hidden % kOpCols) return 0;
  return c.heads % 6 == 0 ? 6 : c.heads % 4 == 0 ? 4 : 0;
}

template <int VPL>
int forward_rows(mq_encoder* e, const int* ids, const int* mask, int B, int L, float* out,
                 hipStream_t s) {
  const mq_bert_config& c = e->cfg;
  const int M = B * L, H = c.hidden, F = c.ffn;
  const float eps = c.ln_eps;
  const float scale = 1.0f / sqrtf((float)(H / c.heads));
  const int q_tiles = (L + 31) / 32;
  const int dsplit = rows_splits(F, e->rows_splits);
  const int hg = oproj_heads_per_plane(e, L);
  const bool qf = hg != 0 && L % 16 == 0 && (3 * H) % 48 == 0;
  const bool dacc = dsplit == 2 && !e->rows_planes;
  const bool yacc = hg != 0 && c.heads / hg == 2 && !e->rows_planes;
  int prev_rows = M;
  for (size_t li = 0; li < e->layers.size(); ++li) {
    const LayerW& w = e->layers[li];
    const bool cls_only = c.pooling == MQ_POOL_CLS && li + 1 == e->layers.size();
    const int rows = cls_only ? B : M;
    const int stride = cls_only ? L * H : H;
    const int nt = (int)li >= e->resident_layers ? 1 : 0;
    e->tl.mark(s, ST_QKV);
    RowsArgs qkv{e->slab.p, H, (int64_t)prev_rows * H, w.wqkvf, H, w.bqkv, nullptr, 0, e->qkv.p, 3 * H, 0, M, 3 * H, H, 1};
    qkv.nt_w = nt;
    if (li == 0) {
      qkv.A = e->word;
      qkv.a_plane = 0;
      qkv.ids = ids;
      qkv.L = L;
      qkv.vocab = c.vocab_size;
      qkv.pos = e->pos;
      qkv.typ = e->typ;
    }
    const LayerW* pl = li ? &e->layers[li - 1] : nullptr;
    const float* lg = pl ? pl->ln2g : e->eg;
    const float* lb = pl ? pl->ln2b : e->eb;
    const int s_in = pl ? (dacc ? 1 : dsplit) : 0;
    if (yacc) {
      qkv.zbuf = e->y.p;
      qkv.zn = (int64_t)rows * H;
    }
    if (qf)
      ROWS_REP launch_rows_ln<EPI_BIAS, VPL, FL_O | FL_OT>(qkv, s_in, lg, lb, eps, e->x.p, s);
    else
      ROWS_REP launch_rows_ln<EPI_BIAS, VPL>(qkv, s_in, lg, lb, eps, e->x.p, s);
    const int qt = cls_only ? 1 : q_tiles;
    int y_planes = 1;
    if (hg) {
      e->tl.mark(s, ST_OPROJ);
      const int rps = cls_only ? 1 : L, qtiles = (rps + 15) / 16;
      y_planes = c.heads / hg;
      const dim3 grid(H / kOpCols, B * qtiles, y_planes);
      if (yacc) y_planes = 1;
      ROWS_REP launch_attn_oproj(hg, qf, yacc, (L + 15) / 16, grid, s, e->qkv.p, mask, L, H, rps, qtiles, scale, w.wof, w.bo, e->x.p,
                                 stride, e->y.p, (int64_t)rows * H, nt);
    } else {
      e->tl.mark(s, ST_ATTN);
      if (L <= 64)
        hipLaunchKernelGGL(attention_rows_kernel, dim3(B * c.heads * qt), dim3(512), 0, s, e->qkv.p, mask, L,
                           H, c.heads, qt, scale, e->ctx.p);
      else
        launch_attention(B, L, c.heads, qt, H, scale, e->qkv.p, mask, e->ctx.p, s);
      e->tl.mark(s, ST_OPROJ);
      RowsArgs oproj{e->ctx.p, stride, 0, w.wof, H, w.bo, e->x.p, stride, e->y.p, H, 0, rows, H, H, 1};
      oproj.nt_w = nt;
      launch_rows<EPI_RESID>(oproj, s);
    }
    e->tl.mark(s, ST_FFN_UP);
    RowsArgs up{e->y.p, H, (int64_t)rows * H, w.w1f, H, w.b1, nullptr, 0, e->ffn.p, F, 0, rows, F, H, 1};
    up.nt_w = nt;
    if (dacc) {
      up.zbuf = e->slab.p;
      up.zn = (int64_t)rows * H;
    }
    if (c.gelu == MQ_GELU_TANH)
      ROWS_REP launch_rows_ln<EPI_GELU_TANH, VPL, FL_O>(up, y_planes, w.ln1g, w.ln1b, eps, e->x.p, s);
    else
      ROWS_REP launch_rows_ln<EPI_GELU_ERF, VPL, FL_O>(up, y_planes, w.ln1g, w.ln1b, eps, e->x.p, s);
    e->tl.mark(s, ST_FFN_DOWN);
    RowsArgs down{e->ffn.p, F, 0, w.w2f, F, w.b2, e->x.p, H, e->slab.p, H, (int64_t)rows * H, rows, H, F, dsplit};
    down.nt_w = nt;
    if (dacc)
      ROWS_REP launch_rows<EPI_RESID, FL_A | FL_ACC>(down, s);
    else
      ROWS_REP launch_rows<EPI_RESID, FL_A>(down, s);
    prev_rows = rows;
  }
  e->tl.mark(s, ST_POOL);
  const LayerW& last = e->layers.back();
  const int pool_rows = c.pooling == MQ_POOL_CLS ? 1 : L;
  hipLaunchKernelGGL((ln_pool_kernel<VPL>), dim3((unsigned)((B + 3) / 4)), dim3(256), 0, s, e->slab.p, dacc ? 1 : dsplit,
                     (int64_t)prev_rows * H, mask, B, L, pool_rows, c.pooling, last.ln2g, last.ln2b, eps, out);
  e->tl.close(s);
  MQ_HIP(hipGetLastError());
  return MQ_OK;
}

bool use_rows_path(const mq_encoder* e, int B, int L) {
  const mq_bert_config& c = e->cfg;
  const int sp = rows_splits(c.ffn, e->rows_splits);
  return (int64_t)B * L <= e->rows_max && !e->layers.empty() && c.ffn % 256 == 0 &&
         rows_nb_ok(c.ffn / 256 / sp) && (size_t)sp * B * L * c.hidden <= e->slab.n &&
         e->layers[0].wqkvf != nullptr;
}

}

namespace {

int forward(mq_encoder* e, const int* ids, const int* mask, int B, int L, float* out,
            hipStream_t s) {
  const bool rows = use_rows_path(e, B, L);
  switch (e->cfg.hidden) {
    case 256: return rows ? forward_rows<1>(e, ids, mask, B, L, out, s) : forward_vpl<1>(e, ids, mask, B, L, out, s);
    case 512: return rows ? forward_rows<2>(e, ids, mask, B, L, out, s) : forward_vpl<2>(e, ids, mask, B, L, out, s);
    case 768: return rows ? forward_rows<3>(e, ids, mask, B, L, out, s) : forward_vpl<3>(e, ids, mask, B, L, out, s);
    default: return rows ? forward_rows<4>(e, ids, mask, B, L, out, s) : forward_vpl<4>(e, ids, mask, B, L, out, s);
  }
}

constexpr size_t kMaxGraphs = 6;

int launch_graph(mq_encoder* e, int B, int L, hipStream_t s) {
  const std::vector<const void*> bufs = {e->weights.p, e->x.p,   e->y.p,      e->qkv.p,
                                         e->ctx.p,     e->ffn.p, e->slab.p,   e->io_out.p,
                                         e->io_ids,    e->io_mask,  e->w3.p,   e->wfrag.p};
  mq_encoder::Graph* hit = nullptr;
  for (auto& g : e->graphs)
    if (g.B == B && g.L == L && g.precision == e->precision && g.bufs == bufs) hit = &g;
  if (!hit) {
    if (!e->cap_stream) MQ_HIP(hipStreamCreateWithFlags(&e->cap_stream, hipStreamNonBlocking));
    for (size_t i = 0; i < e->graphs.size();) {
      if (e->graphs[i].bufs != bufs) {
        (void)hipGraphExecDestroy(e->graphs[i].exec);
        e->graphs.erase(e->graphs.begin() + i);
      } else {
        ++i;
      }
    }
    if (e->graphs.size() >= kMaxGraphs) {
      auto lru = std::min_element(e->graphs.begin(), e->graphs.end(),
                                  [](const auto& a, const auto& b) { return a.last_use < b.last_use; });
      (void)hipGraphExecDestroy(lru->exec);
      e->graphs.erase(lru);
    }
    hipGraph_t graph = nullptr;
    MQ_HIP(hipStreamBeginCapture(e->cap_stream, hipStreamCaptureModeThreadLocal));
    const int rc = forward(e, e->io_ids, e->io_mask, B, L, e->io_out.p, e->cap_stream);
    const hipError_t end = hipStreamEndCapture(e->cap_stream, &graph);
    if (rc) {
      if (graph) (void)hipGraphDestroy(graph);
      return rc;
    }
    if (end != hipSuccess) MQ_FAIL(MQ_EHIP, "graph capture failed: %s", hipGetErrorString(end));
    mq_encoder::Graph g;
    g.B = B;
    g.L = L;
    g.precision = e->precision;
    g.bufs = bufs;
    const hipError_t inst = hipGraphInstantiate(&g.exec, graph, nullptr, nullptr, 0);
    (void)hipGraphDestroy(graph);
    if (inst != hipSuccess) MQ_FAIL(MQ_EHIP, "graph instantiate failed: %s", hipGetErrorString(inst));
    e->graphs.push_back(g);
    hit = &e->graphs.back();
  }
  hit->last_use = ++e->graph_clock;
  MQ_HIP(hipGraphLaunch(hit->exec, s));
  return MQ_OK;
}

__global__ __launch_bounds__(256) void frag16_qkv_image_kernel(const float* __restrict__ qkv, int rows, int H,
                                                               float* __restrict__ img) {
  const int ld = 3 * H;
  const int64_t idx = (int64_t)blockIdx.x * 256 + threadIdx.x;
  if (idx >= (int64_t)rows * ld) return;
  const int64_t row = idx / ld;
  const int col = (int)(idx - row * ld);
  const bool vt = col >= 2 * H;
  const int64_t irow = vt ? ((row & ~(int64_t)15) | (col & 15)) : row;
  const int icol = vt ? ((col & ~15) | (int)(row & 15)) : col;
  img[frag16_offset(irow, icol, ld)] = qkv[idx];
}

}

extern "C" {

int64_t mq_encoder_weight_count(const mq_bert_config* cfg) {
  if (!cfg) return -1;
  return weight_count(*cfg);
}

int mq_encoder_create(int device, const mq_bert_config* cfg, mq_encoder** out) {
  clear_error();
  MQ_CHECK_ARG(out && cfg, "NULL argument");
  *out = nullptr;
  const mq_bert_config& c = *cfg;
  MQ_CHECK_ARG(c.hidden == 256 || c.hidden == 512 || c.hidden == 768 || c.hidden == 1024,
               "hidden must be 256/512/768/1024 (got %d)", c.hidden);
  MQ_CHECK_ARG(c.heads > 0 && c.hidden / c.heads == kDh && c.hidden % c.heads == 0,
               "head dim must be %d (hidden %d, heads %d)", kDh, c.hidden, c.heads);
  MQ_CHECK_ARG(c.ffn > 0 && c.ffn % kBK == 0, "ffn must be a positive multiple of %d", kBK);
  MQ_CHECK_ARG(c.layers >= 1 && c.vocab_size > 0 && c.max_positions > 0 && c.type_vocab > 0,
               "bad config");
  MQ_CHECK_ARG(c.gelu == MQ_GELU_ERF || c.gelu == MQ_GELU_TANH, "bad gelu variant");
  MQ_CHECK_ARG(c.pooling == MQ_POOL_CLS || c.pooling == MQ_POOL_MEAN, "bad pooling");
  DeviceGuard dg(device);
  if (!dg.ok) MQ_FAIL(MQ_EHIP, "hipSetDevice(%d) failed", device);
  auto e = std::make_unique<mq_encoder>();
  e->device = device;
  e->cfg = c;
  int cus = 0;
  if (hipDeviceGetAttribute(&cus, hipDeviceAttributeMultiprocessorCount, device) == hipSuccess &&
      cus > 0)
    e->num_cus = cus;
  *out = e.release();
  return MQ_OK;
}

int mq_encoder_destroy(mq_encoder* e) {
  clear_error();
  if (!e) return MQ_OK;
  {
    DeviceGuard dg(e->device);
    for (Buf* b : {&e->weights, &e->x, &e->y, &e->qkv, &e->ctx, &e->ffn, &e->io_out, &e->slab, &e->w3, &e->wfrag,
                   &e->lnst})
      b->release();
    if (e->io_ids) (void)hipFree(e->io_ids);
    if (e->io_mask) (void)hipFree(e->io_mask);
    e->pin.release();
    for (auto& g : e->graphs) (void)hipGraphExecDestroy(g.exec);
    if (e->cap_stream) (void)hipStreamDestroy(e->cap_stream);
  }
  delete e;
  return MQ_OK;
}

int mq_encoder_load_weights(mq_encoder* e, const float* blob, int64_t n_floats) {
  clear_error();
  MQ_CHECK_ARG(e && blob, "NULL argument");
  const mq_bert_config& c = e->cfg;
  const int64_t need = weight_count(c);
  MQ_CHECK_ARG(n_floats == need, "weight blob has %lld floats, config needs %lld",
               (long long)n_floats, (long long)need);
  std::lock_guard<std::mutex> lk(e->mu);
  DeviceGuard dg(e->device);
  int rc = e->weights.ensure((size_t)need);
  if (rc) return rc;
  MQ_HIP(hipMemcpy(e->weights.p, blob, (size_t)need * 4, hipMemcpyHostToDevice));
  const int64_t H = c.hidden, F = c.ffn;
  const float* p = e->weights.p;
  auto take = [&](int64_t n) {
    const float* r = p;
    p += n;
    return r;
  };
  e->word = take((int64_t)c.vocab_size * H);
  e->pos = take((int64_t)c.max_positions * H);
  e->typ = take((int64_t)c.type_vocab * H);
  e->eg = take(H);
  e->eb = take(H);
  e->layers.clear();
  for (int l = 0; l < c.layers; ++l) {
    LayerW w;
    w.wqkv = take(3 * H * H);
    w.bqkv = take(3 * H);
    w.wo = take(H * H);
    w.bo = take(H);
    w.ln1g = take(H);
    w.ln1b = take(H);
    w.w1 = take(F * H);
    w.b1 = take(F);
    w.w2 = take(H * F);
    w.b2 = take(H);
    w.ln2g = take(H);
    w.ln2b = take(H);
    e->layers.push_back(w);
  }
  e->loaded = true;
  if (H % 16 == 0 && F % 16 == 0) {
    rc = build_frag16(e);
    if (rc) return rc;
  }
  return build_w3(e);
}

int mq_encoder_set_precision(mq_encoder* e, int dtype) {
  clear_error();
  MQ_CHECK_ARG(e, "NULL encoder");
  MQ_CHECK_ARG(dtype == MQ_DTYPE_F32 || dtype == MQ_DTYPE_F32X6,
               "encoder precision must be MQ_DTYPE_F32 or MQ_DTYPE_F32X6 (got %d)", dtype);
  std::lock_guard<std::mutex> lk(e->mu);
  e->precision = dtype;
  return build_w3(e);
}

int mq_debug_gemm_f32(const float* A, const float* W, const float* bias, const float* resid,
                      float* out, int M, int N, int K, int epi, int tile, void* stream) {
  clear_error();
  MQ_CHECK_ARG(A && W && bias && out && (epi != EPI_RESID || resid), "NULL buffer");
  MQ_CHECK_ARG(M > 0 && N > 0 && K > 0 && K % kBK == 0, "bad shape M=%d N=%d K=%d", M, N, K);
  MQ_CHECK_ARG(epi >= 0 && epi <= 3 && tile >= 0 && tile <= 9, "bad epi/tile");
  int dev = 0, cus = 256;
  (void)hipGetDevice(&dev);
  (void)hipDeviceGetAttribute(&cus, hipDeviceAttributeMultiprocessorCount, dev);
  GemmArgs g{nullptr, 0, A, K, W, bias, resid, N, out, N, M, N, K};
  hipStream_t s = (hipStream_t)stream;
  if (tile == 4) {
    MQ_CHECK_ARG(N % 4 == 0, "split-K needs N %% 4 == 0");
    const int slices = K / kBK;
    int S = 1;
    for (int c = 2; c <= slices && c <= 64; ++c)
      if (slices % c == 0) S = c;
    float* slab = nullptr;
    if (hipMalloc((void**)&slab, (size_t)S * M * N * 4) != hipSuccess)
      MQ_FAIL(MQ_ENOMEM, "slab allocation failed");
    g.slab = slab;
    g.slab_floats = (size_t)S * M * N;
    switch (epi) {
      case EPI_BIAS: launch_splitk<EPI_BIAS>(g, S, s); break;
      case EPI_GELU_ERF: launch_splitk<EPI_GELU_ERF>(g, S, s); break;
      case EPI_GELU_TANH: launch_splitk<EPI_GELU_TANH>(g, S, s); break;
      default: launch_splitk<EPI_RESID>(g, S, s); break;
    }
    const hipError_t err = hipStreamSynchronize(s);
    (void)hipFree(slab);
    if (err != hipSuccess) MQ_FAIL(MQ_EHIP, "split-K GEMM failed: %s", hipGetErrorString(err));
    return MQ_OK;
  }
  switch (epi) {
    case EPI_BIAS: launch_gemm_tile<EPI_BIAS>(g, tile, cus, s); break;
    case EPI_GELU_ERF: launch_gemm_tile<EPI_GELU_ERF>(g, tile, cus, s); break;
    case EPI_GELU_TANH: launch_gemm_tile<EPI_GELU_TANH>(g, tile, cus, s); break;
    default: launch_gemm_tile<EPI_RESID>(g, tile, cus, s); break;
  }
  MQ_HIP(hipGetLastError());
  return MQ_OK;
}

int mq_debug_attention(const float* qkv, const int* mask, int B, int L, int H, int heads, float scale,
                       int variant, float* ctx, void* stream) {
  clear_error();
  MQ_CHECK_ARG(qkv && mask && ctx, "NULL buffer");
  MQ_CHECK_ARG(B > 0 && L > 0 && heads > 0 && H == heads * kDh, "bad shape B=%d L=%d H=%d heads=%d", B, L, H, heads);
  hipStream_t s = (hipStream_t)stream;
  const int qt = (L + 31) / 32;
  const dim3 grid(B * heads * qt);
  switch (variant) {
    case -1: launch_attention(B, L, heads, qt, H, scale, qkv, mask, ctx, s); break;
    case 1: hipLaunchKernelGGL(attention_kernel<1>, grid, dim3(64), 0, s, qkv, mask, L, H, heads, qt, scale, ctx); break;
    case 2: hipLaunchKernelGGL(attention_kernel<2>, grid, dim3(128), 0, s, qkv, mask, L, H, heads, qt, scale, ctx); break;
    case 4: hipLaunchKernelGGL(attention_kernel<4>, grid, dim3(256), 0, s, qkv, mask, L, H, heads, qt, scale, ctx); break;
    case 8: hipLaunchKernelGGL(attention_kernel<8>, grid, dim3(512), 0, s, qkv, mask, L, H, heads, qt, scale, ctx); break;
    case 12:
      MQ_CHECK_ARG(heads == 12 && L <= 32, "variant 12 needs heads == 12 and L <= 32 (heads %d, L %d)", heads, L);
      hipLaunchKernelGGL((attention_kernel<1, 12>), dim3(B * qt), dim3(768), 0, s, qkv, mask, L, H, heads, qt, scale,
                         ctx);
      break;
    case 16:
      MQ_CHECK_ARG(L <= 64, "variant 16 (attention_rows_kernel) needs L <= 64 (got %d)", L);
      hipLaunchKernelGGL(attention_rows_kernel, grid, dim3(512), 0, s, qkv, mask, L, H, heads, qt, scale, ctx);
      break;
    default: MQ_FAIL(MQ_EINVAL, "bad attention variant %d", variant);
  }
  MQ_HIP(hipGetLastError());
  return MQ_OK;
}

int mq_debug_attn_oproj(const float* qkv, const int* mask, int B, int L, int H, int heads, float scale,
                        const float* Wo, const float* bo, const float* resid, int cls_only, int hg, int qf,
                        int acc, float* out, void* stream) {
  clear_error();
  MQ_CHECK_ARG(qkv && mask && Wo && bo && resid && out, "NULL buffer");
  MQ_CHECK_ARG(B > 0 && L > 0 && heads > 0 && H == heads * kDh, "bad shape B=%d L=%d H=%d heads=%d", B, L, H, heads);
  MQ_CHECK_ARG((hg == 4 || hg == 6) && heads % hg == 0, "hg must be 4 or 6 and divide heads (hg %d, heads %d)", hg,
               heads);
  MQ_CHECK_ARG(L <= 64, "the fused kernel holds L <= 64 keys (got %d)", L);
  MQ_CHECK_ARG(!qf || L % 16 == 0, "qf needs L %% 16 == 0 (got %d)", L);
  const int planes = heads / hg;
  MQ_CHECK_ARG(!acc || planes == 2, "acc needs two head groups (got %d)", planes);
  hipStream_t s = (hipStream_t)stream;
  const int M = B * L, rows = cls_only ? B : M;
  float* scratch = nullptr;
  const size_t wo_floats = (size_t)H * H, qkv_floats = qf ? (size_t)M * 3 * H : 0;
  if (hipMalloc((void**)&scratch, (wo_floats + qkv_floats) * 4) != hipSuccess)
    MQ_FAIL(MQ_ENOMEM, "operand image allocation failed");
  hipLaunchKernelGGL(frag16_image_kernel, dim3((unsigned)((wo_floats / 4 + 255) / 256)), dim3(256), 0, s, Wo, H, H,
                     reinterpret_cast<floatx4*>(scratch));
  const float* qkv_in = qkv;
  if (qf) {
    float* img = scratch + wo_floats;
    hipLaunchKernelGGL(frag16_qkv_image_kernel, dim3((unsigned)((qkv_floats + 255) / 256)), dim3(256), 0, s, qkv, M,
                       H, img);
    qkv_in = img;
  }
  hipError_t err = hipSuccess;
  if (acc) err = hipMemsetAsync(out, 0, (size_t)rows * H * 4, s);
  if (err == hipSuccess) {
    const int rps = cls_only ? 1 : L, qtiles = (rps + 15) / 16;
    const dim3 grid(H / kOpCols, B * qtiles, planes);
    launch_attn_oproj(hg, qf != 0, acc != 0, (L + 15) / 16, grid, s, qkv_in, mask, L, H, rps, qtiles, scale, scratch,
                      bo, resid, cls_only ? L * H : H, out, (int64_t)rows * H, 0);
    err = hipGetLastError();
  }
  const hipError_t serr = hipStreamSynchronize(s);
  (void)hipFree(scratch);
  if (err == hipSuccess) err = serr;
  if (err != hipSuccess) MQ_FAIL(MQ_EHIP, "fused attention + output projection failed: %s", hipGetErrorString(err));
  return MQ_OK;
}

int mq_encoder_set_graphs(mq_encoder* e, int enabled) {
  clear_error();
  MQ_CHECK_ARG(e, "NULL encoder");
  std::lock_guard<std::mutex> lk(e->mu);
  e->use_graphs = enabled != 0;
  return MQ_OK;
}

int mq_encoder_set_option(mq_encoder* e, int option, int value) {
  clear_error();
  MQ_CHECK_ARG(e, "NULL encoder");
  std::lock_guard<std::mutex> lk(e->mu);
  switch (option) {
    case MQ_ENC_OPT_ROWS_MAX:
      MQ_CHECK_ARG(value >= 0 && value <= kRowsMax, "rows_max must be in [0, %d] (got %d)", kRowsMax, value);
      e->rows_max = value;
      break;
    case MQ_ENC_OPT_ROWS_SPLITS:
      MQ_CHECK_ARG(value >= 0 && value <= 4, "rows_splits must be in [0, 4] (got %d)", value);
      e->rows_splits = value;
      break;
    case MQ_ENC_OPT_SPLITK_MAX:
      MQ_CHECK_ARG(value >= 2 && value <= 64, "splitk_max must be in [2, 64] (got %d)", value);
      e->splitk_max = value;
      break;
    case MQ_ENC_OPT_LN_ROWS_PER_WAVE:
      MQ_CHECK_ARG(value == 1 || value == 2 || value == 4, "ln_rows_per_wave must be 1, 2 or 4 (got %d)", value);
      e->ln_rows_per_wave = value;
      break;
    case MQ_ENC_OPT_FUSE_ATTN_OPROJ:
      MQ_CHECK_ARG(value == 0 || value == 1, "fuse_attn_oproj must be 0 or 1 (got %d)", value);
      e->fuse_attn_oproj = value != 0;
      break;
    case MQ_ENC_OPT_FUSED_LN:
      MQ_CHECK_ARG(value == 0 || value == 1, "fused_ln must be 0 or 1 (got %d)", value);
      e->fused_ln = value != 0;
      break;
    case MQ_ENC_OPT_RESIDENT_LAYERS:
      MQ_CHECK_ARG(value >= 0 && value <= 1024, "resident_layers must be in [0, 1024] (got %d)", value);
      e->resident_layers = value;
      break;
    case MQ_ENC_OPT_LN_ON_LOAD:
      MQ_CHECK_ARG(value == 0 || value == 1, "ln_on_load must be 0 or 1 (got %d)", value);
      e->ln_on_load = value != 0;
      break;
    case MQ_ENC_OPT_SPLITK_TILES:
      MQ_CHECK_ARG(value >= 0 && value <= 4096, "splitk_tiles must be in [0, 4096] (got %d)", value);
      e->splitk_tiles = value;
      break;
    case MQ_ENC_OPT_X6_PRESPLIT:
      MQ_CHECK_ARG(value == 0 || value == 1, "x6_presplit must be 0 or 1 (got %d)", value);
      e->x6_presplit = value != 0;
      break;
    case MQ_ENC_OPT_ROWS_PLANES:
      MQ_CHECK_ARG(value == 0 || value == 1, "rows_planes must be 0 or 1 (got %d)", value);
      e->rows_planes = value != 0;
      break;
    case MQ_ENC_OPT_LN_FOLD:
      MQ_CHECK_ARG(value == 0 || value == 1, "ln_fold must be 0 or 1 (got %d)", value);
      e->ln_fold = value != 0;
      break;
    default:
      MQ_FAIL(MQ_EINVAL, "unknown encoder option %d", option);
  }
  for (auto& g : e->graphs) (void)hipGraphExecDestroy(g.exec);
  e->graphs.clear();
  return MQ_OK;
}

int mq_encoder_get_option(const mq_encoder* e, int option, int* value) {
  clear_error();
  MQ_CHECK_ARG(e && value, "NULL argument");
  switch (option) {
    case MQ_ENC_OPT_ROWS_MAX: *value = e->rows_max; break;
    case MQ_ENC_OPT_ROWS_SPLITS: *value = e->rows_splits; break;
    case MQ_ENC_OPT_SPLITK_MAX: *value = e->splitk_max; break;
    case MQ_ENC_OPT_LN_ROWS_PER_WAVE: *value = e->ln_rows_per_wave; break;
    case MQ_ENC_OPT_FUSE_ATTN_OPROJ: *value = e->fuse_attn_oproj ? 1 : 0; break;
    case MQ_ENC_OPT_FUSED_LN: *value = e->fused_ln ? 1 : 0; break;
    case MQ_ENC_OPT_LN_ON_LOAD: *value = e->ln_on_load ? 1 : 0; break;
    case MQ_ENC_OPT_RESIDENT_LAYERS: *value = e->resident_layers; break;
    case MQ_ENC_OPT_SPLITK_TILES: *value = e->splitk_tiles; break;
    case MQ_ENC_OPT_X6_PRESPLIT: *value = e->x6_presplit ? 1 : 0; break;
    case MQ_ENC_OPT_ROWS_PLANES: *value = e->rows_planes ? 1 : 0; break;
    case MQ_ENC_OPT_LN_FOLD: *value = e->ln_fold ? 1 : 0; break;
    default: MQ_FAIL(MQ_EINVAL, "unknown encoder option %d", option);
  }
  return MQ_OK;
}

int mq_encoder_set_timing(mq_encoder* e, int enabled) {
  clear_error();
  MQ_CHECK_ARG(e, "NULL encoder");
  std::lock_guard<std::mutex> lk(e->mu);
  DeviceGuard dg(e->device);
  e->tl.drain();
  e->tl.on = enabled != 0;
  return MQ_OK;
}

int mq_encoder_read_timing(mq_encoder* e, float* ms, int n) {
  clear_error();
  MQ_CHECK_ARG(e && ms && n >= 0, "bad argument");
  std::lock_guard<std::mutex> lk(e->mu);
  DeviceGuard dg(e->device);
  e->tl.read(ms, n);
  return MQ_OK;
}

int mq_encoder_embed(mq_encoder* e, const int32_t* ids, const int32_t* mask, int B, int L,
                     float* out, int io_on_device, void* stream) {
  clear_error();
  MQ_CHECK_ARG(e, "NULL encoder");
  MQ_CHECK_ARG(B >= 0 && L >= 1, "bad shape B=%d L=%d", B, L);
  MQ_CHECK_ARG(L <= e->cfg.max_positions, "L=%d exceeds max_positions %d", L, e->cfg.max_positions);
  if (B == 0) return MQ_OK;
  MQ_CHECK_ARG(ids && mask && out, "NULL buffer");
  MQ_CHECK_ARG((int64_t)B * L < (1ll << 31) / 4096, "batch too large");
  if (!e->loaded) MQ_FAIL(MQ_ESTATE, "encoder weights not loaded");
  std::lock_guard<std::mutex> lk(e->mu);
  DeviceGuard dg(e->device);
  hipStream_t s = (hipStream_t)stream;
  const mq_bert_config& c = e->cfg;
  const size_t M = (size_t)B * L;
  if (e->tl.used > 4096) e->tl.drain();
  int rc = MQ_OK;
  rc = e->slab.ensure((size_t)2 * e->num_cus * 32 * 128);
  if (rc) return rc;
  rc = build_fold(e);
  if (rc) return rc;
  const size_t ln_parts = (e->ln_on_load || e->ln_fold) && M > 256 ? (size_t)4 * M * std::max(1, c.hidden / kLnPartW) : 0;
  for (auto bn : {std::make_pair(&e->x, M * c.hidden), std::make_pair(&e->y, (M <= (size_t)kRowsMax ? 4 : 1) * M * c.hidden),
                  std::make_pair(&e->ctx, M * c.hidden), std::make_pair(&e->qkv, M * 3 * c.hidden),
                  std::make_pair(&e->ffn, (M + 15) / 16 * 16 * c.ffn), std::make_pair(&e->lnst, ln_parts)}) {
    rc = bn.first->ensure(bn.second);
    if (rc) return rc;
  }
  const bool graph = e->use_graphs && !e->tl.on;
  const int* dids = ids;
  const int* dmask = mask;
  float* dout = out;
  if (!io_on_device || graph) {
    if (e->io_tokens < M) {
      if (e->io_ids) (void)hipFree(e->io_ids);
      if (e->io_mask) (void)hipFree(e->io_mask);
      e->io_ids = e->io_mask = nullptr;
      e->io_tokens = 0;
      if (hipMalloc((void**)&e->io_ids, M * 4) != hipSuccess ||
          hipMalloc((void**)&e->io_mask, M * 4) != hipSuccess)
        MQ_FAIL(MQ_ENOMEM, "hipMalloc(io) failed");
      e->io_tokens = M;
    }
    rc = e->io_out.ensure((size_t)B * c.hidden);
    if (rc) return rc;
    const hipMemcpyKind kind = io_on_device ? hipMemcpyDeviceToDevice : hipMemcpyHostToDevice;
    if (!io_on_device && M * 8 + (size_t)B * c.hidden * 4 <= (1u << 20)) {
      rc = e->pin.ensure(M * 8 + (size_t)B * c.hidden * 4);
      if (rc) return rc;
      memcpy(e->pin.as<unsigned char>(), ids, M * 4);
      memcpy(e->pin.as<unsigned char>() + M * 4, mask, M * 4);
      MQ_HIP(hipMemcpyAsync(e->io_ids, e->pin.p, M * 4, kind, s));
      MQ_HIP(hipMemcpyAsync(e->io_mask, e->pin.as<unsigned char>() + M * 4, M * 4, kind, s));
    } else {
      MQ_HIP(hipMemcpyAsync(e->io_ids, ids, M * 4, kind, s));
      MQ_HIP(hipMemcpyAsync(e->io_mask, mask, M * 4, kind, s));
    }
    dids = e->io_ids;
    dmask = e->io_mask;
    dout = e->io_out.p;
  }
  if (graph) {
    rc = launch_graph(e, B, L, s);
  } else {
    rc = forward(e, dids, dmask, B, L, dout, s);
  }
  if (rc) return rc;
  if (io_on_device && dout != out)
    MQ_HIP(hipMemcpyAsync(out, dout, (size_t)B * c.hidden * 4, hipMemcpyDeviceToDevice, s));
  if (!io_on_device) {
    const size_t ob = (size_t)B * c.hidden * 4;
    if (M * 8 + ob <= (1u << 20)) {
      unsigned char* hp = e->pin.as<unsigned char>() + M * 8;
      MQ_HIP(hipMemcpyAsync(hp, dout, ob, hipMemcpyDeviceToHost, s));
      MQ_HIP(hipStreamSynchronize(s));
      memcpy(out, hp, ob);
    } else {
      MQ_HIP(hipMemcpyAsync(out, dout, ob, hipMemcpyDeviceToHost, s));
      MQ_HIP(hipStreamSynchronize(s));
    }
  }
  return MQ_OK;
}

#ifdef MQ_KTRACE
int mq_debug_ktrace_read(long long* out, int n) {
  const int total = kTraceRegions * kTraceWgs * kTraceSlots;
  if (!out || n < total) return MQ_EINVAL;
  if (hipMemcpyFromSymbol(out, HIP_SYMBOL(mq_ktrace), total * sizeof(long long)) != hipSuccess) return MQ_EHIP;
  std::vector<long long> zero(total, 0);
  if (hipMemcpyToSymbol(HIP_SYMBOL(mq_ktrace), zero.data(), total * sizeof(long long)) != hipSuccess) return MQ_EHIP;
  return MQ_OK;
}
#endif

}
```

### mediquery-rag_amd/mediquery_hip/_lib.py

```python
import ctypes
import hashlib
import os

try:
    import torch
except Exception:
    torch = None

LIB_PATH = os.environ.get("MQ_LIB_PATH") or os.path.join(os.path.dirname(os.path.abspath(__file__)),
                                                          "libmqhip.so")

MQ_OK = 0
MQ_DTYPE_F32, MQ_DTYPE_BF16, MQ_DTYPE_F32X6, MQ_DTYPE_F32_SCREEN = 0, 1, 2, 3
MQ_GELU_ERF, MQ_GELU_TANH = 0, 1
MQ_POOL_CLS, MQ_POOL_MEAN = 0, 1
MQ_MAX_K = 64
MQ_MASK_SET, MQ_MASK_AND, MQ_MASK_OR, MQ_MASK_CLEAR = 0, 1, 2, 3
MQ_CONTAINS_MAX_BYTES = 256
MQ_CONTAINS_SPAN_BYTES = 16384
MQ_ENC_OPT_ROWS_MAX, MQ_ENC_OPT_ROWS_SPLITS, MQ_ENC_OPT_SPLITK_MAX = 0, 1, 2
MQ_ENC_OPT_LN_ROWS_PER_WAVE, MQ_ENC_OPT_FUSE_ATTN_OPROJ, MQ_ENC_OPT_FUSED_LN = 3, 4, 5
MQ_ENC_OPT_SPLITK_TILES, MQ_ENC_OPT_LN_ON_LOAD, MQ_ENC_OPT_RESIDENT_LAYERS = 6, 7, 8
MQ_ENC_OPT_X6_PRESPLIT = 9
MQ_ENC_OPT_ROWS_PLANES = 10
MQ_ENC_OPT_LN_FOLD = 11


class MQError(RuntimeError):

    def __init__(self, fn, code, msg):
        super().__init__("%s failed (status %d): %s" % (fn, code, msg))
        self.code = code


class BertConfigC(ctypes.Structure):
    _fields_ = [("vocab_size", ctypes.c_int), ("hidden", ctypes.c_int), ("layers", ctypes.c_int),
                ("heads", ctypes.c_int), ("ffn", ctypes.c_int), ("max_positions", ctypes.c_int),
                ("type_vocab", ctypes.c_int), ("ln_eps", ctypes.c_float), ("gelu", ctypes.c_int),
                ("pooling", ctypes.c_int)]

    @classmethod
    def from_config(cls, cfg):
        return cls(cfg.vocab_size, cfg.hidden, cfg.layers, cfg.heads, cfg.ffn, cfg.max_positions,
                   cfg.type_vocab, cfg.ln_eps, cfg.gelu, cfg.pooling)


_P = ctypes.c_void_p
_I = ctypes.c_int
_I64 = ctypes.c_int64
_PP = ctypes.POINTER(ctypes.c_void_p)

SIGNATURES = {
    "mq_last_error": (ctypes.c_char_p, []),
    "mq_version": (ctypes.c_char_p, []),
    "mq_build_source_hash": (ctypes.c_char_p, []),
    "mq_device_count": (_I, []),
    "mq_index_create": (_I, [_I, _I, _I64, _I, _PP]),
    "mq_index_destroy": (_I, [_P]),
    "mq_index_size": (_I, [_P, ctypes.POINTER(_I64)]),
    "mq_index_dim": (_I, [_P, ctypes.POINTER(_I)]),
    "mq_index_add": (_I, [_P, _P, _I64, _I, _P]),
    "mq_index_reset": (_I, [_P]),
    "mq_index_search": (_I, [_P, _P, _I64, _I, _P, _P, _I, _P]),
    "mq_index_get": (_I, [_P, _I64, _I64, _P, _I, _P]),
    "mq_index_select": (_I, [_P, _P, _I64, _P]),
    "mq_index_data": (_I, [_P, _PP]),
    "mq_index_set_precision": (_I, [_P, _I]),
    "mq_index_set_stream_threshold": (_I, [_P, _I]),
    "mq_index_set_threshold_scan": (_I, [_P, _I]),
    "mq_index_set_int8_screen": (_I, [_P, _I]),
    "mq_index_set_async_screen": (_I, [_P, _I]),
    "mq_index_rescans": (_I, [_P, _P, _P]),
    "mq_index_screen_fallbacks": (_I, [_P, _P, _P]),
    "mq_index_screen_skips": (_I, [_P, _P, _P]),
    "mq_index_set_timing": (_I, [_P, _I]),
    "mq_index_read_timing": (_I, [_P, _P, _I]),
    "mq_index_save": (_I, [_P, ctypes.c_char_p]),
    "mq_index_load": (_I, [_P, ctypes.c_char_p]),
    "mq_index_save_rows": (_I, [_P, ctypes.c_char_p, ctypes.c_int64, ctypes.c_int64]),
    "mq_index_load_append": (_I, [_P, ctypes.c_char_p]),
    "mq_mask_eval": (_I, [_P, _I64, _P, _I, _P, _I, _P]),
    "mq_mask_eval_bits": (_I, [_P, _I64, _P, _I, _P, _I, _P]),
    "mq_mask_combine": (_I, [_P, _P, _I64, _I, _P]),
    "mq_mask_contains": (_I, [_P, _I64, _P, _I64, _P, _I, _I, _P, _I, _P, _P]),
    "mq_index_search_masked": (_I, [_P, _P, _I, _P, _P, _P, _I, _P]),
    "mq_index_search_masked_batch": (_I, [_P, _P, _I64, _I, _P, _P, _P, _I, _P]),
    "mq_index_masked_gathers": (_I, [_P, ctypes.POINTER(_I64)]),
    "mq_index_mmr_select": (_I, [_P, _P, _P, _I64, _I, _I, ctypes.c_float, _P, _P, _I, _P]),
    "mq_index_search_mmr": (_I, [_P, _P, _I64, _I, _I, ctypes.c_float, _P, _P, _P, _I, _P]),
    "mq_topk_merge_host": (_I, [_P, _P, _I, _I64, _I, _I, _P, _P]),
    "mq_topk_merge_device": (_I, [_P, _P, _I, _I64, _I, _I, _P, _P, _P]),
    "mq_encoder_create": (_I, [_I, ctypes.POINTER(BertConfigC), _PP]),
    "mq_encoder_destroy": (_I, [_P]),
    "mq_encoder_weight_count": (_I64, [ctypes.POINTER(BertConfigC)]),
    "mq_encoder_load_weights": (_I, [_P, _P, _I64]),
    "mq_encoder_set_precision": (_I, [_P, _I]),
    "mq_encoder_set_graphs": (_I, [_P, _I]),
    "mq_encoder_set_option": (_I, [_P, _I, _I]),
    "mq_encoder_get_option": (_I, [_P, _I, ctypes.POINTER(ctypes.c_int)]),
    "mq_encoder_set_timing": (_I, [_P, _I]),
    "mq_encoder_read_timing": (_I, [_P, _P, _I]),
    "mq_encoder_embed": (_I, [_P, _P, _P, _I, _I, _P, _I, _P]),
    "mq_tokenizer_create_wordpiece": (_I, [ctypes.c_char_p, _I, _I, _PP]),
    "mq_tokenizer_create_wordpiece_tokens": (_I, [ctypes.POINTER(ctypes.c_char_p), _I, _I, _I, _PP]),
    "mq_tokenizer_create_char": (_I, [_I, _I, _PP]),
    "mq_tokenizer_destroy": (_I, [_P]),
    "mq_tokenizer_encode_batch": (_I, [_P, ctypes.POINTER(ctypes.c_char_p), _I, _I, _P, _P,
                                       ctypes.POINTER(_I)]),
    "mq_debug_gemm_f32": (_I, [_P, _P, _P, _P, _P, _I, _I, _I, _I, _I, _P]),
    "mq_debug_w3_bytes": (_I64, [_I, _I]),
    "mq_debug_split_w3": (_I, [_P, _I, _I, _P, _P]),
    "mq_debug_gemm_x6p": (_I, [_P, _P, _P, _P, _P, _I, _I, _I, _I, _I, _P]),
    "mq_debug_gemm_x6p_ln": (_I, [_P, _P, _P, _P, _P, _I, _I, _I, _I, _I, _P, _P, _P, _P, _P, ctypes.c_float, _P]),
    "mq_debug_ln_fold_weight": (_I, [_P, _P, _P, _P, _I, _I, _P, _P, _P, _P]),
    "mq_debug_attention": (_I, [_P, _P, _I, _I, _I, _I, ctypes.c_float, _I, _P, _P]),
    "mq_debug_attn_oproj": (_I, [_P, _P, _I, _I, _I, _I, ctypes.c_float, _P, _P, _P, _I, _I, _I, _I, _P, _P]),
    "mq_debug_int8_screen":(_I, [_P, _P, _I, _P, _P, _P]),
}

_lib = None


def lib():
    global _lib
    if _lib is None:
        if not os.path.exists(LIB_PATH):
            raise ImportError("libmqhip.so not found at %s - build it with "
                              "`make -C mediquery-rag_amd/csrc` or __graft_entry__.build()" % LIB_PATH)
        h = ctypes.CDLL(LIB_PATH)
        allow_missing = os.environ.get("MQ_LIB_ALLOW_MISSING") == "1"
        for name, (res, args) in SIGNATURES.items():
            if allow_missing and not hasattr(h, name):
                continue
            fn = getattr(h, name)
            fn.restype = res
            fn.argtypes = args
        _lib = h
    return _lib


def check(fn_name, rc):
    if rc != MQ_OK:
        raise MQError(fn_name, rc, lib().mq_last_error().decode("utf-8", "replace"))
    return rc


def call(fn_name, *args):
    return check(fn_name, getattr(lib(), fn_name)(*args))


CSRC = os.path.join(os.path.dirname(os.path.dirname(os.path.abspath(__file__))), "csrc")
_STAMPED_EXT = (".hip", ".cpp", ".hpp", ".inc")


def tree_source_hash(csrc=CSRC):
    names = sorted(f for f in os.listdir(csrc) if f.endswith(_STAMPED_EXT))
    paths = [os.path.join(csrc, f) for f in names]
    paths += [os.path.join(csrc, "Makefile"), os.path.join(csrc, "..", "..", "include", "mq.h")]
    h = hashlib.sha256()
    for p in paths:
        with open(p, "rb") as f:
            h.update(f.read())
    return h.hexdigest()[:16]


def built_source_hash():
    return lib().mq_build_source_hash().decode()


def check_build_fresh():
    if not os.path.isdir(CSRC):
        return
    built, tree = built_source_hash(), tree_source_hash()
    if built != tree:
        raise ImportError("libmqhip.so at %s was built from sources %s, the tree holds %s: "
                          "rebuild with `make -C mediquery-rag_amd/csrc`" % (LIB_PATH, built, tree))


def device_count():
    return lib().mq_device_count()


def ptr(a):
    if a is None:
        return None
    if isinstance(a, int):
        return ctypes.c_void_p(a)
    if hasattr(a, "data_ptr"):
        return ctypes.c_void_p(a.data_ptr())
    return ctypes.c_void_p(a.ctypes.data)


class device_scope:

    def __init__(self, device):
        self._ctx = None
        if device is not None and torch is not None and torch.cuda.is_available():
            self._ctx = torch.cuda.device(int(device))

    def __enter__(self):
        if self._ctx is not None:
            self._ctx.__enter__()
        return self

    def __exit__(self, *exc):
        if self._ctx is not None:
            return self._ctx.__exit__(*exc)
        return False


def stream_handle(stream=None):
    if stream is None:
        if torch is None or not torch.cuda.is_available():
            return None
        stream = torch.cuda.current_stream()
    if isinstance(stream, int):
        return ctypes.c_void_p(stream)
    return ctypes.c_void_p(stream.cuda_stream)
```

### mediquery-rag_amd/mediquery_hip/native.py

```python
import ctypes

import numpy as np

from . import _lib
from .config import BertConfig
from .weights import state_dict_to_blob, synthetic_state_dict


class FlatIndex:

    def __init__(self, dim=768, capacity=0, device=0, dtype=_lib.MQ_DTYPE_F32):
        h = ctypes.c_void_p()
        _lib.call("mq_index_create", device, dim, capacity, dtype, ctypes.byref(h))
        self._h = h
        self.dim = dim
        self.device = device

    def close(self):
        h, self._h = getattr(self, "_h", None), None
        if h:
            try:
                _lib.lib().mq_index_destroy(h)
            except Exception:
                pass

    __del__ = close

    def __len__(self):
        n = ctypes.c_int64()
        _lib.call("mq_index_size", self._h, ctypes.byref(n))
        return n.value

    def add(self, rows):
        rows = np.ascontiguousarray(rows, dtype=np.float32).reshape(-1, self.dim)
        _lib.call("mq_index_add", self._h, _lib.ptr(rows), rows.shape[0], 0, None)

    def add_device(self, rows, stream=None):
        assert rows.is_cuda and rows.dtype.is_floating_point and rows.is_contiguous()
        _lib.call("mq_index_add", self._h, _lib.ptr(rows), rows.shape[0], 1,
                  _lib.stream_handle(stream))

    def reset(self):
        _lib.call("mq_index_reset", self._h)

    def search(self, queries, k):
        q = np.ascontiguousarray(queries, dtype=np.float32).reshape(-1, self.dim)
        scores = np.empty((q.shape[0], k), dtype=np.float32)
        ids = np.empty((q.shape[0], k), dtype=np.int64)
        _lib.call("mq_index_search", self._h, _lib.ptr(q), q.shape[0], k, _lib.ptr(scores),
                  _lib.ptr(ids), 0, None)
        return scores, ids

    def search_device(self, queries, k, out_scores, out_ids, stream=None):
        _lib.call("mq_index_search", self._h, _lib.ptr(queries), queries.shape[0], k,
                  _lib.ptr(out_scores), _lib.ptr(out_ids), 1, _lib.stream_handle(stream))

    def get(self, row0=0, n=None):
        n = len(self) - row0 if n is None else n
        out = np.empty((n, self.dim), dtype=np.float32)
        _lib.call("mq_index_get", self._h, row0, n, _lib.ptr(out), 0, None)
        return out

    def select(self, rows, out=None):
        rows = np.ascontiguousarray(rows, dtype=np.int64).reshape(-1)
        out = FlatIndex(dim=self.dim, device=self.device) if out is None else out
        _lib.call("mq_index_select", self._h, _lib.ptr(rows), rows.size, out._h)
        return out

    def data_ptr(self):
        p = ctypes.c_void_p()
        _lib.call("mq_index_data", self._h, ctypes.byref(p))
        return p.value

    STAGES = ("flat_search_kernel", "merge_kernel")

    def set_precision(self, dtype):
        _lib.call("mq_index_set_precision", self._h, dtype)

    def set_stream_threshold(self, max_queries):
        _lib.call("mq_index_set_stream_threshold", self._h, int(max_queries))

    def set_threshold_scan(self, enabled=True):
        _lib.call("mq_index_set_threshold_scan", self._h, int(bool(enabled)))

    def set_int8_screen(self, enabled=True):
        _lib.call("mq_index_set_int8_screen", self._h, int(bool(enabled)))

    def set_async_screen(self, enabled=True):
        _lib.call("mq_index_set_async_screen", self._h, int(bool(enabled)))

    @property
    def rescans(self):
        n = ctypes.c_int64()
        _lib.call("mq_index_rescans", self._h, ctypes.byref(n), None)
        return n.value

    @property
    def remerges(self):
        n = ctypes.c_int64()
        _lib.call("mq_index_rescans", self._h, None, ctypes.byref(n))
        return n.value

    @property
    def screen_fallbacks(self):
        n = ctypes.c_int64()
        _lib.call("mq_index_screen_fallbacks", self._h, ctypes.byref(n), None)
        return n.value

    @property
    def screen_passdowns(self):
        n = ctypes.c_int64()
        _lib.call("mq_index_screen_fallbacks", self._h, None, ctypes.byref(n))
        return n.value

    @property
    def screen_skips(self):
        n = ctypes.c_int64()
        _lib.call("mq_index_screen_skips", self._h, ctypes.byref(n), None)
        return n.value

    @property
    def int8_skips(self):
        n = ctypes.c_int64()
        _lib.call("mq_index_screen_skips", self._h, None, ctypes.byref(n))
        return n.value

    def set_timing(self, enabled=True):
        _lib.call("mq_index_set_timing", self._h, int(bool(enabled)))

    def read_timing(self):
        ms = np.zeros(len(self.STAGES), dtype=np.float32)
        _lib.call("mq_index_read_timing", self._h, _lib.ptr(ms), len(ms))
        return dict(zip(self.STAGES, ms.tolist()))

    def save(self, path):
        _lib.call("mq_index_save", self._h, str(path).encode())

    def load(self, path):
        _lib.call("mq_index_load", self._h, str(path).encode())

    def _check_bits(self, bits):
        check_mask_words(bits, len(self), self.device)

    def search_masked(self, queries, k, bits):
        q = np.ascontiguousarray(queries, dtype=np.float32).reshape(-1, self.dim)
        self._check_bits(bits)
        scores = np.empty((q.shape[0], k), dtype=np.float32)
        ids = np.empty((q.shape[0], k), dtype=np.int64)
        with _lib.device_scope(self.device):
            _lib.call("mq_index_search_masked_batch", self._h, _lib.ptr(q), q.shape[0], k, _lib.ptr(bits),
                      _lib.ptr(scores), _lib.ptr(ids), 0, _lib.stream_handle(None))
        return scores, ids

    def mmr_select(self, cand_scores, cand_ids, k, lambda_mult=0.5):
        s = np.ascontiguousarray(cand_scores, dtype=np.float32)
        i = np.ascontiguousarray(cand_ids, dtype=np.int64)
        s = s.reshape(1, -1) if s.ndim == 1 else s
        i = i.reshape(s.shape)
        scores = np.empty((s.shape[0], k), dtype=np.float32)
        ids = np.empty((s.shape[0], k), dtype=np.int64)
        with _lib.device_scope(self.device):
            _lib.call("mq_index_mmr_select", self._h, _lib.ptr(s), _lib.ptr(i), s.shape[0], s.shape[1], k,
                      float(lambda_mult), _lib.ptr(scores), _lib.ptr(ids), 0, _lib.stream_handle(None))
        return scores, ids

    def mmr_select_device(self, cand_scores, cand_ids, k, lambda_mult, out_scores, out_ids, stream=None):
        _lib.call("mq_index_mmr_select", self._h, _lib.ptr(cand_scores), _lib.ptr(cand_ids),
                  cand_scores.shape[0], cand_scores.shape[1], k, float(lambda_mult), _lib.ptr(out_scores),
                  _lib.ptr(out_ids), 1, _lib.stream_handle(stream))

    def search_mmr(self, queries, k, fetch_k, lambda_mult=0.5, bits=None):
        q = np.ascontiguousarray(queries, dtype=np.float32).reshape(-1, self.dim)
        if bits is not None:
            self._check_bits(bits)
        scores = np.empty((q.shape[0], k), dtype=np.float32)
        ids = np.empty((q.shape[0], k), dtype=np.int64)
        with _lib.device_scope(self.device):
            _lib.call("mq_index_search_mmr", self._h, _lib.ptr(q), q.shape[0], k, fetch_k, float(lambda_mult),
                      _lib.ptr(bits), _lib.ptr(scores), _lib.ptr(ids), 0, _lib.stream_handle(None))
        return scores, ids

    @property
    def masked_gathers(self):
        n = ctypes.c_int64()
        _lib.call("mq_index_masked_gathers", self._h, ctypes.byref(n))
        return n.value

    def save_rows(self, path, row0, n):
        _lib.call("mq_index_save_rows", self._h, str(path).encode(), int(row0), int(n))

    def load_append(self, path):
        _lib.call("mq_index_load_append", self._h, str(path).encode())


def merge_topk_host(scores, ids, k_out):
    scores = np.ascontiguousarray(scores, dtype=np.float32)
    ids = np.ascontiguousarray(ids, dtype=np.int64)
    n_lists, nq, k_in = scores.shape
    os_ = np.empty((nq, k_out), dtype=np.float32)
    oi = np.empty((nq, k_out), dtype=np.int64)
    _lib.call("mq_topk_merge_host", _lib.ptr(scores), _lib.ptr(ids), n_lists, nq, k_in, k_out,
              _lib.ptr(os_), _lib.ptr(oi))
    return os_, oi


def merge_topk_device(scores, ids, k_out, out_scores, out_ids, stream=None):
    n_lists, nq, k_in = scores.shape
    _lib.call("mq_topk_merge_device", _lib.ptr(scores), _lib.ptr(ids), n_lists, nq, k_in, k_out,
              _lib.ptr(out_scores), _lib.ptr(out_ids), _lib.stream_handle(stream))


class Encoder:

    def __init__(self, cfg: BertConfig, weights=None, seed=0, device=0):
        self.cfg = cfg
        self.device = device
        self._ccfg = _lib.BertConfigC.from_config(cfg)
        h = ctypes.c_void_p()
        _lib.call("mq_encoder_create", device, ctypes.byref(self._ccfg), ctypes.byref(h))
        self._h = h
        sd = weights if weights is not None else synthetic_state_dict(cfg, seed)
        blob = state_dict_to_blob(cfg, sd)
        n = _lib.lib().mq_encoder_weight_count(ctypes.byref(self._ccfg))
        if n != blob.size:
            raise ValueError("weight blob %d floats, library expects %d" % (blob.size, n))
        _lib.call("mq_encoder_load_weights", self._h, _lib.ptr(blob), blob.size)

    def close(self):
        h, self._h = getattr(self, "_h", None), None
        if h:
            try:
                _lib.lib().mq_encoder_destroy(h)
            except Exception:
                pass

    __del__ = close

    STAGES = ("embed_ln", "qkv_gemm", "attention", "out_proj_gemm", "layernorm", "ffn_up_gemm",
              "ffn_down_gemm", "pool")

    def set_timing(self, enabled=True):
        _lib.call("mq_encoder_set_timing", self._h, int(bool(enabled)))

    def read_timing(self):
        ms = np.zeros(len(self.STAGES), dtype=np.float32)
        _lib.call("mq_encoder_read_timing", self._h, _lib.ptr(ms), len(ms))
        return dict(zip(self.STAGES, ms.tolist()))

    def set_precision(self, dtype):
        _lib.call("mq_encoder_set_precision", self._h, dtype)

    def set_graphs(self, enabled=True):
        _lib.call("mq_encoder_set_graphs", self._h, int(bool(enabled)))

    OPTIONS = {"rows_max": _lib.MQ_ENC_OPT_ROWS_MAX, "rows_splits": _lib.MQ_ENC_OPT_ROWS_SPLITS,
               "splitk_max": _lib.MQ_ENC_OPT_SPLITK_MAX, "ln_rows_per_wave": _lib.MQ_ENC_OPT_LN_ROWS_PER_WAVE,
               "fuse_attn_oproj": _lib.MQ_ENC_OPT_FUSE_ATTN_OPROJ, "fused_ln": _lib.MQ_ENC_OPT_FUSED_LN,
               "splitk_tiles": _lib.MQ_ENC_OPT_SPLITK_TILES, "ln_on_load": _lib.MQ_ENC_OPT_LN_ON_LOAD,
               "resident_layers": _lib.MQ_ENC_OPT_RESIDENT_LAYERS, "x6_presplit": _lib.MQ_ENC_OPT_X6_PRESPLIT,
               "rows_planes": _lib.MQ_ENC_OPT_ROWS_PLANES, "ln_fold": _lib.MQ_ENC_OPT_LN_FOLD}

    def set_option(self, name, value):
        _lib.call("mq_encoder_set_option", self._h, self.OPTIONS[name], int(value))

    def get_option(self, name):
        v = ctypes.c_int()
        _lib.call("mq_encoder_get_option", self._h, self.OPTIONS[name], ctypes.byref(v))
        return v.value

    def embed(self, ids, mask):
        ids = np.ascontiguousarray(ids, dtype=np.int32)
        mask = np.ascontiguousarray(mask, dtype=np.int32)
        B, L = ids.shape
        out = np.empty((B, self.cfg.hidden), dtype=np.float32)
        _lib.call("mq_encoder_embed", self._h, _lib.ptr(ids), _lib.ptr(mask), B, L, _lib.ptr(out),
                  0, None)
        return out

    def embed_device(self, ids, mask, out, stream=None):
        B, L = ids.shape
        _lib.call("mq_encoder_embed", self._h, _lib.ptr(ids), _lib.ptr(mask), B, L, _lib.ptr(out),
                  1, _lib.stream_handle(stream))


def check_mask_words(bits, n, device=None):
    if not (getattr(bits, "is_cuda", False) and bits.element_size() == 4 and bits.is_contiguous()
            and bits.numel() >= (int(n) + 31) // 32):
        raise ValueError("bits must be a contiguous 32-bit device tensor of >= ceil(n / 32) = %d words"
                         % ((int(n) + 31) // 32))
    if device is not None and bits.device.index != int(device):
        raise ValueError("bits lives on cuda:%s, the index on cuda:%d" % (bits.device.index, int(device)))


def _check_codes(codes, bits):
    import torch
    if not (getattr(codes, "is_cuda", False) and codes.dtype == torch.int32 and codes.is_contiguous()):
        raise ValueError("codes must be a contiguous int32 device tensor")
    check_mask_words(bits, codes.numel(), codes.device.index)


def mask_eval(codes, lut, bits, mode, stream=None):
    import torch
    _check_codes(codes, bits)
    if not (getattr(lut, "is_cuda", False) and lut.dtype == torch.uint8 and lut.is_contiguous()
            and lut.device == codes.device and lut.numel() >= 1):
        raise ValueError("lut must be a non-empty contiguous uint8 tensor on the codes' device")
    with _lib.device_scope(codes.device.index):
        _lib.call("mq_mask_eval", _lib.ptr(codes), codes.numel(), _lib.ptr(lut), lut.numel(), _lib.ptr(bits),
                  mode, _lib.stream_handle(stream))


def mask_eval_bits(codes, lut, bits, mode, stream=None):
    _check_codes(codes, bits)
    lut = np.asarray(lut).astype(bool)
    if not 1 <= lut.size <= 256:
        raise ValueError("a by-value table holds 1..256 entries (got %d)" % lut.size)
    words = np.zeros(4, dtype=np.uint64)
    for i in np.flatnonzero(lut).tolist():
        words[i >> 6] |= np.uint64(1 << (i & 63))
    with _lib.device_scope(codes.device.index):
        _lib.call("mq_mask_eval_bits", _lib.ptr(codes), codes.numel(), _lib.ptr(words), len(lut), _lib.ptr(bits),
                  mode, _lib.stream_handle(stream))


def mask_contains(text, offsets, pattern, bits, mode, negate=False, stream=None, scratch=None):
    import torch
    if not (getattr(text, "is_cuda", False) and text.dtype == torch.uint8 and text.is_contiguous()
            and text.dim() == 1):
        raise ValueError("text must be a contiguous 1-d uint8 device tensor")
    if text.numel() and text.data_ptr() % 16:
        raise ValueError("text must start at a 16-byte aligned address")
    if not (getattr(offsets, "is_cuda", False) and offsets.dtype == torch.int64 and offsets.is_contiguous()
            and offsets.numel() >= 1 and offsets.device == text.device):
        raise ValueError("offsets must be a contiguous int64 tensor of n + 1 elements on the text's device")
    n = offsets.numel() - 1
    check_mask_words(bits, n, text.device.index)
    if not isinstance(pattern, (bytes, bytearray)) or not 1 <= len(pattern) <= _lib.MQ_CONTAINS_MAX_BYTES:
        raise ValueError("pattern must be 1..%d bytes" % _lib.MQ_CONTAINS_MAX_BYTES)
    with _lib.device_scope(text.device.index):
        if scratch is None:
            scratch = torch.empty(max(1, (n + 31) // 32), dtype=torch.int32, device=text.device)
        check_mask_words(scratch, n, text.device.index)
        if scratch.data_ptr() == bits.data_ptr():
            raise ValueError("scratch must not be bits")
        _lib.call("mq_mask_contains", _lib.ptr(text), text.numel(), _lib.ptr(offsets), n, bytes(pattern),
                  len(pattern), int(bool(negate)), _lib.ptr(bits), mode, _lib.ptr(scratch),
                  _lib.stream_handle(stream))


def mask_combine(dst, src, mode, stream=None):
    check_mask_words(dst, 0)
    if src is not None:
        check_mask_words(src, 32 * dst.numel(), dst.device.index)
    with _lib.device_scope(dst.device.index):
        _lib.call("mq_mask_combine", _lib.ptr(dst), _lib.ptr(src), dst.numel(), mode, _lib.stream_handle(stream))
```

Measured before the change: 38260.

## Compute last-layer CLS attention without materializing keys and values

For CLS pooling, the last layer's CLS query is projected through the transposed key weights (u = Wk^T q per head). Scores are then dot products of u with the layernormed hidden rows, and the context is formed by multiplying Wv with the attention-weighted sum of hidden rows. This removes the full K/V projection GEMM over all tokens in the final layer and replaces it with a streaming online-softmax pass plus small per-head GEMMs. The final LayerNorm and L2 normalization are also fused into the split-K reduce, which drops the separate pool launch. In exchange it adds a one-time weight transpose, extra scratch buffers and new kernels.

```diff
diff --git a/include/mq.h b/include/mq.h
--- a/include/mq.h
+++ b/include/mq.h
@@ -126,6 +126,7 @@
 #define MQ_ENC_OPT_X6_PRESPLIT 9
 #define MQ_ENC_OPT_ROWS_PLANES 10
 #define MQ_ENC_OPT_LN_FOLD 11
+#define MQ_ENC_OPT_CLS_KFREE 12
 int mq_encoder_set_option(mq_encoder* enc, int option, int value);
 int mq_encoder_get_option(const mq_encoder* enc, int option, int* value);
 int mq_encoder_set_timing(mq_encoder* enc, int enabled);
@@ -157,6 +158,10 @@
                             int K, float* Wg, float* s_out, float* c_out, void* stream);
 int mq_debug_attention(const float* qkv, const int* mask, int B, int L, int H, int heads, float scale,
                        int variant, float* ctx, void* stream);
+int mq_debug_cls_attention(const float* q, const float* x, const float* stats, const float* ln_g,
+                           const float* ln_b, float eps, const int* mask, int B, int L, int H, int heads,
+                           float scale, const float* Wk, const float* Wv, const float* bv, float* ctx,
+                           void* stream);
 int mq_debug_attn_oproj(const float* qkv, const int* mask, int B, int L, int H, int heads, float scale,
                         const float* Wo, const float* bo, const float* resid, int cls_only, int hg, int qf,
                         int acc, float* out, void* stream);
diff --git a/mediquery-rag_amd/csrc/encoder.hip b/mediquery-rag_amd/csrc/encoder.hip
--- a/mediquery-rag_amd/csrc/encoder.hip
+++ b/mediquery-rag_amd/csrc/encoder.hip
@@ -486,7 +486,7 @@
   }
 }
 
-template <int VPL>
+template <int VPL, bool POOL = false>
 __global__ __launch_bounds__(256) void splitk_reduce_ln_kernel(
     const float* __restrict__ slab, int S, int M, const float* __restrict__ bias,
     const float* resid, int ldr, const float* __restrict__ g, const float* __restrict__ b,
@@ -540,6 +540,19 @@
     var += x[i] * x[i];
   }
   const float rstd = 1.0f / sqrtf(block_sum(var) * (1.0f / H) + eps);
+  if constexpr (POOL) {
+    float ss = 0.f;
+#pragma unroll
+    for (int i = 0; i < VPL; ++i) {
+      const int c = t + 256 * i;
+      x[i] = x[i] * rstd * g[c] + b[c];
+      ss += x[i] * x[i];
+    }
+    const float inv = 1.0f / fmaxf(sqrtf(block_sum(ss)), 1e-12f);
+#pragma unroll
+    for (int i = 0; i < VPL; ++i) dst[(int64_t)row * H + t + 256 * i] = x[i] * inv;
+    return;
+  }
 #pragma unroll
   for (int i = 0; i < VPL; ++i) {
     const int c = t + 256 * i;
@@ -932,6 +945,19 @@
   for (int i = 0; i < VPL; ++i) v[i] = *reinterpret_cast<const floatx4*>(xr + (i * 64 + lane) * 4);
   ln_row_store<VPL>(v, g, b, eps, xr, lane);
 }
+template <int VPL>
+__global__ __launch_bounds__(256) void ln_rows_kernel(const float* __restrict__ x, int rows, int64_t stride,
+                                                      const float* __restrict__ g, const float* __restrict__ b,
+                                                      float eps, float* __restrict__ dst) {
+  const int lane = threadIdx.x & 63;
+  const int row = blockIdx.x * 4 + (threadIdx.x >> 6);
+  if (row >= rows) return;
+  const float* xr = x + (int64_t)row * stride;
+  floatx4 v[VPL];
+#pragma unroll
+  for (int i = 0; i < VPL; ++i) v[i] = *reinterpret_cast<const floatx4*>(xr + (i * 64 + lane) * 4);
+  ln_row_store<VPL>(v, g, b, eps, dst + (int64_t)row * (VPL * 256), lane);
+}
 
 constexpr int kDh = 64;
 
@@ -1439,6 +1465,198 @@
     *reinterpret_cast<floatx4*>(out + (int64_t)b * H + (i * 64 + lane) * 4) = x[i] * inv;
 }
 
+
+__global__ __launch_bounds__(256) void transpose_kernel(const float* __restrict__ W, int R, int C,
+                                                        float* __restrict__ out) {
+  __shared__ float tile[32][33];
+  const int tx = threadIdx.x & 31, ty = threadIdx.x >> 5;
+  const int r0 = blockIdx.y * 32, c0 = blockIdx.x * 32;
+  for (int j = ty; j < 32; j += 8)
+    if (r0 + j < R && c0 + tx < C) tile[j][tx] = W[(int64_t)(r0 + j) * C + c0 + tx];
+  __syncthreads();
+  for (int j = ty; j < 32; j += 8)
+    if (c0 + j < C && r0 + tx < R) out[(int64_t)(c0 + j) * R + r0 + tx] = tile[tx][j];
+}
+
+constexpr int kClsCtxSplits = 4;
+template <class T>
+__global__ __launch_bounds__(256, 2) void gemm_heads_kernel(const float* __restrict__ A, int lda, int a_head,
+                                                            const float* __restrict__ W, int ldw, int w_head,
+                                                            const float* __restrict__ bias,
+                                                            const float* __restrict__ live, int M, int N, int K,
+                                                            float* __restrict__ out, int ldo, int o_head, int S,
+                                                            int64_t o_plane) {
+  __shared__ __attribute__((aligned(16))) float lds[2 * T::STAGE_FLOATS];
+  const int lane = threadIdx.x & 63, wave = threadIdx.x >> 6;
+  const int wm = wave / T::WAVES_N, wn = wave % T::WAVES_N;
+  const int tiles_n = (N + T::BN - 1) / T::BN;
+  const int per_head = ((M + T::BM - 1) / T::BM) * tiles_n;
+  const int sidx = blockIdx.x % S, ht = blockIdx.x / S;
+  const int head = ht / per_head, tile = ht % per_head;
+  const int Kc = K / S;
+  const int m0 = (tile / tiles_n) * T::BM;
+  const int n0 = (tile % tiles_n) * T::BN;
+  auto coords = [&](int, int& mm0, int64_t& nn0) {
+    mm0 = m0;
+    nn0 = n0;
+  };
+  float* dst = out + sidx * o_plane + (int64_t)head * o_head;
+  auto epi = [&](int, floatx16(&acc)[T::TM][T::TN], float*) {
+#pragma unroll
+    for (int tn = 0; tn < T::TN; ++tn) {
+      const int col = n0 + wn * T::WN + tn * 32 + (lane & 31);
+      if (col >= N) continue;
+      const float bv = bias ? bias[head * N + col] : 0.f;
+#pragma unroll
+      for (int tm = 0; tm < T::TM; ++tm)
+#pragma unroll
+        for (int e = 0; e < 16; ++e) {
+          const int row = m0 + wm * T::WM + acc_row(tm, e, lane);
+          if (row < M) dst[(int64_t)row * ldo + col] = bias ? __fmaf_rn(live[row], bv, acc[tm][tn][e]) : acc[tm][tn][e];
+        }
+    }
+  };
+  walk_tiles<T>(lds, 1,
+                TileOperands{A + (int64_t)head * a_head + sidx * Kc, lda, M, W + (int64_t)head * w_head + sidx * Kc, ldw,
+                             N, Kc},
+                coords, epi);
+}
+
+__global__ __launch_bounds__(256) void cls_ctx_reduce_kernel(const float* __restrict__ part, int B, int H,
+                                                             const float* __restrict__ bv,
+                                                             const float* __restrict__ live,
+                                                             float* __restrict__ ctx) {
+  const int64_t i4 = (int64_t)blockIdx.x * 256 + threadIdx.x;
+  const int n4 = H / 4;
+  if (i4 >= (int64_t)B * n4) return;
+  const int row = (int)(i4 / n4), c = (int)(i4 % n4) * 4;
+  floatx4 v = sum_slabs(part + (int64_t)row * H + c, (int64_t)B * H, kClsCtxSplits);
+  const float lv = live[row];
+  const floatx4 b = *reinterpret_cast<const floatx4*>(bv + c);
+#pragma unroll
+  for (int j = 0; j < 4; ++j) v[j] = __fmaf_rn(lv, b[j], v[j]);
+  *reinterpret_cast<floatx4*>(ctx + (int64_t)row * H + c) = v;
+}
+
+constexpr int kClsChunk = 16;
+template <int VPL, bool FOLD>
+__global__ __launch_bounds__(256 * VPL) void cls_pass_kernel(const float* __restrict__ x,
+                                                             const float* __restrict__ stats,
+                                                             const float* __restrict__ g,
+                                                             const float* __restrict__ be, float eps,
+                                                             const float* __restrict__ u,
+                                                             const int* __restrict__ mask, int L, float scale,
+                                                             float* __restrict__ z, float* __restrict__ live) {
+  constexpr int H = VPL * 256, HEADS = H / kDh, CH = kClsChunk;
+  constexpr int TPR = H / CH;
+  static_assert(CH == 16 && (CH * H + CH * HEADS + 2 * HEADS) * 4 <= 64 * 1024, "LDS: one chunk of rows, scores");
+  __shared__ __attribute__((aligned(16))) float xs[CH * H];
+  __shared__ __attribute__((aligned(16))) float ps[CH * HEADS];
+  __shared__ __attribute__((aligned(16))) float alpha_s[HEADS];
+  __shared__ float l_s[HEADS];
+  const int t = threadIdx.x, lane = t & 63, h = t >> 6;
+  const int b = blockIdx.x;
+  const int64_t row0 = (int64_t)b * L;
+  const int lrow = t / TPR, lc4 = t % TPR;
+  floatx4 ur[VPL];
+#pragma unroll
+  for (int i = 0; i < VPL; ++i) {
+    ur[i] = *reinterpret_cast<const floatx4*>(u + ((int64_t)b * HEADS + h) * H + (i * 64 + lane) * 4);
+    if constexpr (FOLD) ur[i] *= *reinterpret_cast<const floatx4*>(g + (i * 64 + lane) * 4);
+  }
+  floatx4 xr[4], sr[kLnMaxParts / 2];
+  int mk = 0;
+  auto fetch = [&](int k0) {
+    const int64_t row = row0 + min(k0 + lrow, L - 1);
+#pragma unroll
+    for (int j = 0; j < 4; ++j) xr[j] = *reinterpret_cast<const floatx4*>(x + row * H + (lc4 + TPR * j) * 4);
+    if constexpr (FOLD) {
+      const floatx4* sp = reinterpret_cast<const floatx4*>(stats + row * (2 * kLnMaxParts));
+#pragma unroll
+      for (int i = 0; i < kLnMaxParts / 2; ++i) sr[i] = sp[i];
+    }
+    mk = lane < CH && k0 + lane < L ? mask[row0 + k0 + lane] : 0;
+  };
+  float zacc[HEADS];
+#pragma unroll
+  for (int hh = 0; hh < HEADS; ++hh) zacc[hh] = 0.f;
+  float m_run = -INFINITY, l_run = 0.f;
+  fetch(0);
+  for (int k0 = 0; k0 < L; k0 += CH) {
+    if constexpr (FOLD) {
+      float mu, rho;
+      ln_merge(sr, eps, mu, rho);
+#pragma unroll
+      for (int j = 0; j < 4; ++j) xr[j] = (xr[j] - mu) * rho;
+    }
+#pragma unroll
+    for (int j = 0; j < 4; ++j) *reinterpret_cast<floatx4*>(xs + lrow * H + (lc4 + TPR * j) * 4) = xr[j];
+    const int live_key = mk;
+    __syncthreads();
+    if (k0 + CH < L) fetch(k0 + CH);
+    float d[CH];
+#pragma unroll
+    for (int k = 0; k < CH; ++k) {
+      float a = 0.f;
+#pragma unroll
+      for (int i = 0; i < VPL; ++i) {
+        const floatx4 v = *reinterpret_cast<const floatx4*>(xs + k * H + (i * 64 + lane) * 4);
+        a = fmaf(v.x, ur[i].x, fmaf(v.y, ur[i].y, fmaf(v.z, ur[i].z, fmaf(v.w, ur[i].w, a))));
+      }
+      d[k] = a;
+    }
+#pragma unroll
+    for (int k = 0; k < CH; ++k) d[k] = wave_sum_fast(d[k]);
+    float sc = -INFINITY;
+#pragma unroll
+    for (int k = 0; k < CH; ++k) sc = lane == k ? d[k] : sc;
+    sc = live_key != 0 ? sc * scale : -INFINITY;
+    float tmax = sc;
+#pragma unroll
+    for (int off = 8; off > 0; off >>= 1) tmax = fmaxf(tmax, __shfl_xor(tmax, off));
+    tmax = __shfl(tmax, 0);
+    const float m_new = fmaxf(m_run, tmax);
+    const float alpha = m_new == -INFINITY ? 1.f : expf(m_run - m_new);
+    const float p = sc == -INFINITY ? 0.f : expf(sc - m_new);
+    float psum = p;
+#pragma unroll
+    for (int off = 8; off > 0; off >>= 1) psum += __shfl_xor(psum, off);
+    psum = __shfl(psum, 0);
+    l_run = l_run * alpha + psum;
+    m_run = m_new;
+    if (lane < CH) ps[lane * HEADS + h] = p;
+    if (lane == 0) alpha_s[h] = alpha;
+    __syncthreads();
+#pragma unroll
+    for (int q4 = 0; q4 < HEADS / 4; ++q4) {
+      const floatx4 a = *reinterpret_cast<const floatx4*>(alpha_s + 4 * q4);
+#pragma unroll
+      for (int e = 0; e < 4; ++e) zacc[4 * q4 + e] *= a[e];
+    }
+#pragma unroll
+    for (int k = 0; k < CH; ++k) {
+      const float xv = xs[k * H + t];
+#pragma unroll
+      for (int q4 = 0; q4 < HEADS / 4; ++q4) {
+        const floatx4 pp = *reinterpret_cast<const floatx4*>(ps + k * HEADS + 4 * q4);
+#pragma unroll
+        for (int e = 0; e < 4; ++e) zacc[4 * q4 + e] = fmaf(pp[e], xv, zacc[4 * q4 + e]);
+      }
+    }
+    __syncthreads();
+  }
+  if (lane == 0) l_s[h] = l_run;
+  __syncthreads();
+#pragma unroll
+  for (int hh = 0; hh < HEADS; ++hh) {
+    const float l = l_s[hh];
+    float v = l > 0.f ? zacc[hh] * (1.0f / l) : 0.f;
+    if constexpr (FOLD) v = l > 0.f ? fmaf(v, g[t], be[t]) : 0.f;
+    z[((int64_t)b * HEADS + hh) * H + t] = v;
+  }
+  if (t == 0) live[b] = l_s[0] > 0.f ? 1.f : 0.f;
+}
+
 }
 
 using namespace mq;
@@ -1665,6 +1883,10 @@
 #define MQ_LN_FOLD_DEFAULT 1
 #endif
 constexpr bool kLnFoldDefault = MQ_LN_FOLD_DEFAULT != 0;
+#ifndef MQ_CLS_KFREE_DEFAULT
+#define MQ_CLS_KFREE_DEFAULT 1
+#endif
+constexpr bool kClsKfreeDefault = MQ_CLS_KFREE_DEFAULT != 0;
 
 enum Stage { ST_EMBED = 0, ST_QKV, ST_ATTN, ST_OPROJ, ST_LN, ST_FFN_UP, ST_FFN_DOWN, ST_POOL, ST_N };
 
@@ -1709,6 +1931,9 @@
   bool ln_fold = kLnFoldDefault;
   Buf wfold3, wfoldf, sfold;
   bool rows_planes = false;
+  bool cls_kfree = kClsKfreeDefault;
+  Buf wkt;
+  Buf cls;
   bool use_graphs = false;
   uint64_t graph_clock = 0;
   hipStream_t cap_stream = nullptr;
@@ -1820,6 +2045,19 @@
   return MQ_OK;
 }
 
+int build_wkt(mq_encoder* e) {
+  const int H = e->cfg.hidden;
+  if (e->cfg.pooling != MQ_POOL_CLS || e->layers.empty()) return MQ_OK;
+  DeviceGuard dg(e->device);
+  int rc = e->wkt.ensure((size_t)H * H);
+  if (rc) return rc;
+  hipLaunchKernelGGL(transpose_kernel, dim3(H / 32, H / 32), dim3(256), 0, nullptr,
+                     e->layers.back().wqkv + (int64_t)H * H, H, H, e->wkt.p);
+  MQ_HIP(hipGetLastError());
+  MQ_HIP(hipStreamSynchronize(nullptr));
+  return MQ_OK;
+}
+
 template <int EPI>
 void gemm(mq_encoder* e, const GemmArgs& g, int stage, hipStream_t s) {
   e->tl.mark(s, stage);
@@ -1863,6 +2101,68 @@
   else
     hipLaunchKernelGGL((ln_kernel<VPL, 2>), dim3((unsigned)((g.M + 7) / 8)), dim3(256), 0, s, g.out, g.M, lng,
                        lnb, e->cfg.ln_eps, x);
+}
+
+struct ClsBufs {
+  float *xc, *q, *u, *z, *part, *live;
+  static size_t floats(int B, int H, int heads) {
+    return (size_t)B * ((2 + kClsCtxSplits) * H + 2 * (size_t)heads * H + 1);
+  }
+  ClsBufs(float* p, int B, int H, int heads)
+      : xc(p), q(xc + (size_t)B * H), u(q + (size_t)B * H), z(u + (size_t)B * heads * H),
+        part(z + (size_t)B * heads * H), live(part + (size_t)kClsCtxSplits * B * H) {}
+};
+
+void launch_cls_u(int B, int H, int heads, const float* q, const float* wkt, float* u, hipStream_t s) {
+  using T = F32Tile<1, 4, 1, 1>;
+  const int tiles = ((B + T::BM - 1) / T::BM) * ((H + T::BN - 1) / T::BN);
+  hipLaunchKernelGGL((gemm_heads_kernel<T>), dim3(tiles * heads), dim3(256), 0, s, q, H, kDh, wkt, H, kDh, nullptr,
+                     nullptr, B, H, kDh, u, heads * H, H, 1, (int64_t)0);
+}
+
+void launch_cls_ctx(int B, int L, int H, int heads, float scale, const float* x, const float* stats,
+                    const float* g, const float* be, float eps, const float* u, const int* mask, const float* wv,
+                    const float* bv, float* z, float* part, float* live, float* ctx, hipStream_t s) {
+  auto pass = [&](auto vpl) {
+    constexpr int VPL = decltype(vpl)::value;
+    if (stats)
+      hipLaunchKernelGGL((cls_pass_kernel<VPL, true>), dim3(B), dim3(256 * VPL), 0, s, x, stats, g, be, eps, u, mask, L,
+                         scale, z, live);
+    else
+      hipLaunchKernelGGL((cls_pass_kernel<VPL, false>), dim3(B), dim3(256 * VPL), 0, s, x, stats, g, be, eps, u, mask, L,
+                         scale, z, live);
+  };
+  if (H == 256)
+    pass(IC<1>{});
+  else if (H == 512)
+    pass(IC<2>{});
+  else
+    pass(IC<3>{});
+  using T = F32Tile<2, 2, 1, 1>;
+  const int tiles = (B + T::BM - 1) / T::BM;
+  hipLaunchKernelGGL((gemm_heads_kernel<T>), dim3(tiles * heads * kClsCtxSplits), dim3(256), 0, s, z, heads * H, H, wv, H,
+                     kDh * H, nullptr, nullptr, B, kDh, H, part, H, kDh, kClsCtxSplits, (int64_t)B * H);
+  hipLaunchKernelGGL(cls_ctx_reduce_kernel, dim3((unsigned)(((int64_t)B * H / 4 + 255) / 256)), dim3(256), 0, s, part, B,
+                     H, bv, live, ctx);
+}
+
+template <int VPL>
+void gemm_resid_ln_pool(mq_encoder* e, const GemmArgs& g, const float* lng, const float* lnb, const int* mask,
+                        float* out, int stage, hipStream_t s) {
+  const int H = VPL * 256;
+  const int S = splitk_factor(g, e->num_cus, e->splitk_max, e->splitk_tiles);
+  if (S && g.ldr == H && g.N == H) {
+    e->tl.mark(s, stage);
+    launch_splitk_gemm(g, S, s);
+    e->tl.mark(s, ST_POOL);
+    hipLaunchKernelGGL((splitk_reduce_ln_kernel<VPL, true>), dim3((unsigned)g.M), dim3(256), 0, s, g.slab, S, g.M,
+                       g.bias, g.resid, g.ldr, lng, lnb, e->cfg.ln_eps, out);
+    return;
+  }
+  gemm<EPI_RESID>(e, g, stage, s);
+  e->tl.mark(s, ST_POOL);
+  hipLaunchKernelGGL((ln_pool_kernel<VPL>), dim3((unsigned)((g.M + 3) / 4)), dim3(256), 0, s, g.out, 1, (int64_t)0, mask,
+                     g.M, 1, 1, MQ_POOL_CLS, lng, lnb, e->cfg.ln_eps, out);
 }
 
 template <int VPL>
@@ -1890,6 +2190,7 @@
   float* fst1 = e->lnst.p;
   float* fst2 = e->lnst.p + (size_t)2 * M * nt;
   bool raw = false;
+  bool pooled = false;
   auto fold_gemm = [&](auto epi, GemmArgs g, int stage) {
     e->tl.mark(s, stage);
     if (!e->x6_presplit) g.W3 = nullptr;
@@ -1917,7 +2218,11 @@
     const LayerW& w = e->layers[li];
     const bool cls_only = c.pooling == MQ_POOL_CLS && li + 1 == e->layers.size();
     const int rows = cls_only ? B : M;
-    const int stride = cls_only ? L * H : H;
+    int stride = cls_only ? L * H : H;
+    const float* resid = e->x.p;
+    int ldr = stride;
+    const bool kfree = cls_only && L > 1 && e->cls_kfree && VPL <= 3 && e->wkt.p != nullptr &&
+                       e->cls.n >= ClsBufs::floats(B, H, c.heads);
     const float* qkv_in = y_pending ? e->y.p : e->x.p;
     const int lnt = M <= 256 && (int)li >= e->resident_layers ? 1 : 0;
     const bool fold_layer = fold && !(cls_only && L > 1);
@@ -1940,7 +2245,26 @@
         gemm<EPI_BIAS>(e, g, ST_QKV, s);
       }
     };
-    if (cls_only && L > 1) {
+    if (kfree) {
+      const ClsBufs cb(e->cls.p, B, H, c.heads);
+      const float* xin = raw ? e->x.p : y_pending ? e->y.p : e->x.p;
+      const float* xst = raw ? fst2 : y_pending ? st2 : nullptr;
+      if (xst) {
+        e->tl.mark(s, ST_LN);
+        hipLaunchKernelGGL((ln_rows_kernel<VPL>), dim3((unsigned)((B + 3) / 4)), dim3(256), 0, s, xin, B, (int64_t)L * H,
+                           prev->ln2g, prev->ln2b, c.ln_eps, cb.xc);
+        resid = cb.xc;
+        ldr = H;
+      }
+      GemmArgs q{e->slab.p, e->slab.n, resid, ldr, w.wqkv, w.bqkv, nullptr, 0, cb.q, H, B, H, H, lnt};
+      q.W3 = w.wqkv3;
+      gemm<EPI_BIAS>(e, q, ST_QKV, s);
+      launch_cls_u(B, H, c.heads, cb.q, e->wkt.p, cb.u, s);
+      e->tl.mark(s, ST_ATTN);
+      launch_cls_ctx(B, L, H, c.heads, scale, xin, xst, xst ? prev->ln2g : nullptr, xst ? prev->ln2b : nullptr,
+                     c.ln_eps, cb.u, mask, w.wqkv + (int64_t)2 * H * H, w.bqkv + 2 * H, cb.z, cb.part, cb.live, e->ctx.p, s);
+      stride = H;
+    } else if (cls_only && L > 1) {
       GemmArgs kv{e->slab.p, e->slab.n, qkv_in, H, w.wqkv + (int64_t)H * H, w.bqkv + H, nullptr, 0, e->qkv.p + H,
                   3 * H, M, 2 * H, H};
       if (w.wqkv3) kv.W3 = w.wqkv3 + w3_row_offset(H, H);
@@ -1961,11 +2285,13 @@
     y_pending = false;
     const bool resid_raw = raw && fold_layer;
     raw = false;
-    e->tl.mark(s, ST_ATTN);
-    const int qt = cls_only ? 1 : q_tiles;
-    launch_attention(B, L, c.heads, qt, H, scale, e->qkv.p, mask, e->ctx.p, s);
+    if (!kfree) {
+      e->tl.mark(s, ST_ATTN);
+      const int qt = cls_only ? 1 : q_tiles;
+      launch_attention(B, L, c.heads, qt, H, scale, e->qkv.p, mask, e->ctx.p, s);
+    }
     const bool lnl_layer = lnl && !cls_only;
-    GemmArgs oproj{e->slab.p, e->slab.n, e->ctx.p, stride, w.wo, w.bo, e->x.p, stride, e->y.p, H, rows, H, H, lnt};
+    GemmArgs oproj{e->slab.p, e->slab.n, e->ctx.p, stride, w.wo, w.bo, resid, ldr, e->y.p, H, rows, H, H, lnt};
     oproj.W3 = w.wo3;
     if (fold_layer) {
       oproj.lf.stats_out = fst1;
@@ -2028,15 +2354,20 @@
       e->tl.mark(s, ST_FFN_DOWN);
       launch_gemm_stats(down, stats_out(st2), e->num_cus, s);
       y_pending = true;
+    } else if (kfree) {
+      gemm_resid_ln_pool<VPL>(e, down, w.ln2g, w.ln2b, mask, out, ST_FFN_DOWN, s);
+      pooled = true;
     } else {
       gemm_resid_ln<VPL>(e, down, w.ln2g, w.ln2b, e->x.p, ST_FFN_DOWN, s);
     }
     prev = &w;
   }
-  e->tl.mark(s, ST_POOL);
-  const bool pruned = c.pooling == MQ_POOL_CLS;
-  hipLaunchKernelGGL((pool_kernel<VPL>), dim3((B + 3) / 4), dim3(256), 0, s, e->x.p, mask, B,
-                     pruned ? 1 : L, c.pooling, out);
+  if (!pooled) {
+    e->tl.mark(s, ST_POOL);
+    const bool pruned = c.pooling == MQ_POOL_CLS;
+    hipLaunchKernelGGL((pool_kernel<VPL>), dim3((B + 3) / 4), dim3(256), 0, s, e->x.p, mask, B,
+                       pruned ? 1 : L, c.pooling, out);
+  }
   e->tl.close(s);
   MQ_HIP(hipGetLastError());
   return MQ_OK;
@@ -2294,7 +2625,8 @@
 int launch_graph(mq_encoder* e, int B, int L, hipStream_t s) {
   const std::vector<const void*> bufs = {e->weights.p, e->x.p,   e->y.p,      e->qkv.p,
                                          e->ctx.p,     e->ffn.p, e->slab.p,   e->io_out.p,
-                                         e->io_ids,    e->io_mask,  e->w3.p,   e->wfrag.p};
+                                         e->io_ids,    e->io_mask,  e->w3.p,   e->wfrag.p,
+                                         e->wkt.p,     e->cls.p};
   mq_encoder::Graph* hit = nullptr;
   for (auto& g : e->graphs)
     if (g.B == B && g.L == L && g.precision == e->precision && g.bufs == bufs) hit = &g;
@@ -2394,7 +2726,7 @@
   {
     DeviceGuard dg(e->device);
     for (Buf* b : {&e->weights, &e->x, &e->y, &e->qkv, &e->ctx, &e->ffn, &e->io_out, &e->slab, &e->w3, &e->wfrag,
-                   &e->lnst})
+                   &e->lnst, &e->wkt, &e->cls})
       b->release();
     if (e->io_ids) (void)hipFree(e->io_ids);
     if (e->io_mask) (void)hipFree(e->io_mask);
@@ -2452,6 +2784,8 @@
     rc = build_frag16(e);
     if (rc) return rc;
   }
+  rc = build_wkt(e);
+  if (rc) return rc;
   return build_w3(e);
 }
 
@@ -2577,6 +2911,33 @@
   (void)hipFree(scratch);
   if (err == hipSuccess) err = serr;
   if (err != hipSuccess) MQ_FAIL(MQ_EHIP, "fused attention + output projection failed: %s", hipGetErrorString(err));
+  return MQ_OK;
+}
+
+int mq_debug_cls_attention(const float* q, const float* x, const float* stats, const float* ln_g,
+                           const float* ln_b, float eps, const int* mask, int B, int L, int H, int heads,
+                           float scale, const float* Wk, const float* Wv, const float* bv, float* ctx,
+                           void* stream) {
+  clear_error();
+  MQ_CHECK_ARG(q && x && mask && Wk && Wv && bv && ctx, "NULL buffer");
+  MQ_CHECK_ARG(B > 0 && L > 0 && heads > 0 && H == heads * kDh, "bad shape B=%d L=%d H=%d heads=%d", B, L, H, heads);
+  MQ_CHECK_ARG(H == 256 || H == 512 || H == 768, "hidden must be 256 / 512 / 768 (got %d)", H);
+  MQ_CHECK_ARG(!stats || (ln_g && ln_b && H == kLnPartW * kLnMaxParts), "stats need ln_g, ln_b and H = %d",
+               kLnPartW * kLnMaxParts);
+  hipStream_t s = (hipStream_t)stream;
+  float* scratch = nullptr;
+  const size_t wkt_floats = (size_t)H * H;
+  if (hipMalloc((void**)&scratch, (wkt_floats + ClsBufs::floats(B, H, heads)) * 4) != hipSuccess)
+    MQ_FAIL(MQ_ENOMEM, "scratch allocation failed");
+  const ClsBufs cb(scratch + wkt_floats, B, H, heads);
+  hipLaunchKernelGGL(transpose_kernel, dim3(H / 32, H / 32), dim3(256), 0, s, Wk, H, H, scratch);
+  launch_cls_u(B, H, heads, q, scratch, cb.u, s);
+  launch_cls_ctx(B, L, H, heads, scale, x, stats, ln_g, ln_b, eps, cb.u, mask, Wv, bv, cb.z, cb.part, cb.live, ctx, s);
+  hipError_t err = hipGetLastError();
+  const hipError_t serr = hipStreamSynchronize(s);
+  (void)hipFree(scratch);
+  if (err == hipSuccess) err = serr;
+  if (err != hipSuccess) MQ_FAIL(MQ_EHIP, "CLS attention failed: %s", hipGetErrorString(err));
   return MQ_OK;
 }
 
@@ -2641,6 +3002,10 @@
       MQ_CHECK_ARG(value == 0 || value == 1, "ln_fold must be 0 or 1 (got %d)", value);
       e->ln_fold = value != 0;
       break;
+    case MQ_ENC_OPT_CLS_KFREE:
+      MQ_CHECK_ARG(value == 0 || value == 1, "cls_kfree must be 0 or 1 (got %d)", value);
+      e->cls_kfree = value != 0;
+      break;
     default:
       MQ_FAIL(MQ_EINVAL, "unknown encoder option %d", option);
   }
@@ -2665,6 +3030,7 @@
     case MQ_ENC_OPT_X6_PRESPLIT: *value = e->x6_presplit ? 1 : 0; break;
     case MQ_ENC_OPT_ROWS_PLANES: *value = e->rows_planes ? 1 : 0; break;
     case MQ_ENC_OPT_LN_FOLD: *value = e->ln_fold ? 1 : 0; break;
+    case MQ_ENC_OPT_CLS_KFREE: *value = e->cls_kfree ? 1 : 0; break;
     default: MQ_FAIL(MQ_EINVAL, "unknown encoder option %d", option);
   }
   return MQ_OK;
@@ -2711,9 +3077,11 @@
   rc = build_fold(e);
   if (rc) return rc;
   const size_t ln_parts = (e->ln_on_load || e->ln_fold) && M > 256 ? (size_t)4 * M * std::max(1, c.hidden / kLnPartW) : 0;
+  const size_t cls_floats = e->cls_kfree && c.pooling == MQ_POOL_CLS && L > 1 ? ClsBufs::floats(B, c.hidden, c.heads) : 0;
   for (auto bn : {std::make_pair(&e->x, M * c.hidden), std::make_pair(&e->y, (M <= (size_t)kRowsMax ? 4 : 1) * M * c.hidden),
                   std::make_pair(&e->ctx, M * c.hidden), std::make_pair(&e->qkv, M * 3 * c.hidden),
-                  std::make_pair(&e->ffn, (M + 15) / 16 * 16 * c.ffn), std::make_pair(&e->lnst, ln_parts)}) {
+                  std::make_pair(&e->ffn, (M + 15) / 16 * 16 * c.ffn), std::make_pair(&e->lnst, ln_parts),
+                  std::make_pair(&e->cls, cls_floats)}) {
     rc = bn.first->ensure(bn.second);
     if (rc) return rc;
   }
diff --git a/mediquery-rag_amd/mediquery_hip/_lib.py b/mediquery-rag_amd/mediquery_hip/_lib.py
--- a/mediquery-rag_amd/mediquery_hip/_lib.py
+++ b/mediquery-rag_amd/mediquery_hip/_lib.py
@@ -24,6 +24,7 @@
 MQ_ENC_OPT_X6_PRESPLIT = 9
 MQ_ENC_OPT_ROWS_PLANES = 10
 MQ_ENC_OPT_LN_FOLD = 11
+MQ_ENC_OPT_CLS_KFREE = 12
 
 
 class MQError(RuntimeError):
@@ -114,6 +115,8 @@
     "mq_debug_gemm_x6p_ln": (_I, [_P, _P, _P, _P, _P, _I, _I, _I, _I, _I, _P, _P, _P, _P, _P, ctypes.c_float, _P]),
     "mq_debug_ln_fold_weight": (_I, [_P, _P, _P, _P, _I, _I, _P, _P, _P, _P]),
     "mq_debug_attention": (_I, [_P, _P, _I, _I, _I, _I, ctypes.c_float, _I, _P, _P]),
+    "mq_debug_cls_attention": (_I, [_P, _P, _P, _P, _P, ctypes.c_float, _P, _I, _I, _I, _I, ctypes.c_float, _P, _P, _P,
+                                    _P, _P]),
     "mq_debug_attn_oproj": (_I, [_P, _P, _I, _I, _I, _I, ctypes.c_float, _P, _P, _P, _I, _I, _I, _I, _P, _P]),
     "mq_debug_int8_screen":(_I, [_P, _P, _I, _P, _P, _P]),
 }
diff --git a/mediquery-rag_amd/mediquery_hip/native.py b/mediquery-rag_amd/mediquery_hip/native.py
--- a/mediquery-rag_amd/mediquery_hip/native.py
+++ b/mediquery-rag_amd/mediquery_hip/native.py
@@ -258,7 +258,8 @@
                "fuse_attn_oproj": _lib.MQ_ENC_OPT_FUSE_ATTN_OPROJ, "fused_ln": _lib.MQ_ENC_OPT_FUSED_LN,
                "splitk_tiles": _lib.MQ_ENC_OPT_SPLITK_TILES, "ln_on_load": _lib.MQ_ENC_OPT_LN_ON_LOAD,
                "resident_layers": _lib.MQ_ENC_OPT_RESIDENT_LAYERS, "x6_presplit": _lib.MQ_ENC_OPT_X6_PRESPLIT,
-               "rows_planes": _lib.MQ_ENC_OPT_ROWS_PLANES, "ln_fold": _lib.MQ_ENC_OPT_LN_FOLD}
+               "rows_planes": _lib.MQ_ENC_OPT_ROWS_PLANES, "ln_fold": _lib.MQ_ENC_OPT_LN_FOLD,
+               "cls_kfree": _lib.MQ_ENC_OPT_CLS_KFREE}
 
     def set_option(self, name, value):
         _lib.call("mq_encoder_set_option", self._h, self.OPTIONS[name], int(value))
```

Result: faster. 38770 (median of 6 runs) (+1.3%).
